# cherise215/Cooperative_Training_and_Latent_Space_Data_Augmentation

Hardware: AMD Instinct MI355X
Metric: cooperative-training slices/sec (256x256, bs16 per GPU) (higher is better)
Workload: dtype f32 (bf16x3 split)

## Files before the change

### cooperative_training_and_latent_space_data_augmentation_amd/_ffi.py

```python
from __future__ import annotations

import ctypes as C
import os

import numpy as np

_HERE = os.path.dirname(os.path.abspath(__file__))
LIB_PATH = os.path.join(_HERE, "csrc", "libctl_hip.so")
ABI_VERSION = 11
RED_BLOCKS = 512

IN_PLAIN, IN_UP2, IN_ZINS2, IN_C4 = 0, 1, 2, 3
ACT_NONE, ACT_LEAKY, ACT_SIGMOID = 0, 1, 2
EPI_BIAS, EPI_ACCUM, EPI_RES, EPI_STATS, EPI_BNBWD, EPI_TAILBWD = 1, 2, 4, 8, 16, 32
(OP_CONV, OP_WGRAD, OP_WGRAD_REDUCE, OP_PACK, OP_BN_FINALIZE, OP_BN_EVAL, OP_BN_ACT, OP_BWD_REDUCE, OP_BN_BWD_FINALIZE,
 OP_BWD_APPLY, OP_CHAN_SUM_FINALIZE, OP_SUMPOOL2, OP_SIGMOID_BWD, OP_ZERO, OP_COPY, OP_PACK_BATCH, OP_WGRAD_REDUCE_BATCH, OP_DROPOUT2D, OP_BN_REPLAY,
 OP_WGRAD_GROUP) = range(1, 21)
WGRAD_GROUP_MAX = 8
OP_MAX_T = 14

CONV_DTYPE = np.dtype([
    ("n", "<i4"), ("hin", "<i4"), ("win", "<i4"), ("cin", "<i4"), ("hout", "<i4"), ("wout", "<i4"), ("cout", "<i4"),
    ("ks", "<i4"), ("stride", "<i4"), ("pad", "<i4"), ("in_mode", "<i4"), ("pro_affine", "<i4"), ("pro_slope", "<f4"),
    ("epi_flags", "<i4"), ("epi_act", "<i4"), ("epi_slope", "<f4"), ("out_h", "<i4"), ("out_w", "<i4"),
    ("out_sy", "<i4"), ("out_sx", "<i4"), ("nsub", "<i4"), ("out_sub", "<i4"), ("groups", "<i4"), ("dt", "<i4")])
DT_BF16, DT_X16, DT_Y16, DT_RES16, DT_X3 = 1, 2, 4, 8, 16
PACK_X3 = 16
LOSS_WCE, LOSS_FOCAL, LOSS_DICE, LOSS_FG_DICE = 0, 1, 2, 3
OP_DTYPE = np.dtype([("kind", "<i4"), ("i", "<i4", (27,)), ("f", "<f4", (4,)), ("slot", "<i4", (OP_MAX_T,)),
                     ("off", "<i8", (OP_MAX_T,)), ("l", "<i8", (4,))], align=True)


class CtlError(RuntimeError):
    pass


class _Lib:
    def __init__(self):
        self._lib = None

    def load(self):
        if self._lib is not None:
            return self._lib
        if not os.path.exists(LIB_PATH):
            raise CtlError(f"HIP extension not built: {LIB_PATH} is missing. Run `python -c 'import __graft_entry__ as g; "
                           "g.build()'` (or `make -C <package>/csrc`). There is no fallback path.")
        import torch
        lib = C.CDLL(LIB_PATH)
        lib.ctl_last_error.restype = C.c_char_p
        lib.ctl_version.restype = C.c_int
        lib.ctl_launch_count.restype = C.c_ulonglong
        for name in ("ctl_conv_wpack_floats", "ctl_conv_stats_floats", "ctl_wgrad_partial_floats",
                     "ctl_wgrad_bias_partial_floats", "ctl_latent_score_ws_floats", "ctl_latent_mask_apply_ws_floats",
                     "ctl_rescale_intensity_ws_floats", "ctl_sizeof_op", "ctl_sizeof_conv", "ctl_latent_mask_fused_ws_floats", "ctl_conv_wpack_floats_x3",
                     "ctl_surface_stats_ws_bytes", "ctl_surface_map_ws_bytes", "ctl_cc_ws_bytes", "ctl_aug_ws_bytes", "ctl_aug_warp_ws_bytes",
                     "ctl_surface_quantiles_ws_bytes",
                     "ctl_aug_spline_ws_bytes", "ctl_aug_warp_cubic_ws_bytes", "ctl_aug_bias_ws_bytes", "ctl_order_stats_ws_bytes", "ctl_corrupt_spike_ws_bytes",
                     "ctl_seg_loss_ws_doubles"):
            getattr(lib, name).restype = C.c_size_t
        p, i32, i64, f32, u64 = C.c_void_p, C.c_int32, C.c_int64, C.c_float, C.c_uint64
        sig = {
            "ctl_conv_wpack_floats": [i32, i32, i32],
            "ctl_conv_stats_floats": [p], "ctl_conv_stats_blocks": [p],
            "ctl_wgrad_splits": [p], "ctl_wgrad_partial_floats": [p], "ctl_wgrad_bias_partial_floats": [p],
            "ctl_pack_weights": [p, p, i32, i32, i32, i64, i64, i64, i64, i32, p],
            "ctl_conv_forward": [p] * 12, "ctl_conv_forward_ex": [p] * 16, "ctl_conv_pool_ok": [p],
            "ctl_conv_wgrad": [p] * 8, "ctl_conv_wgrad_ex": [p] * 10,
            "ctl_wgrad_group_class": [p, i32], "ctl_wgrad_group_plan": [p, i32, p], "ctl_conv_wgrad_group": [i32] + [p] * 11,
            "ctl_wgrad_reduce": [p, p, p, p, i64, i64, i64, i64, p, i32, p],
            "ctl_confusion_hist": [p, p, i64, i32, p, p],
            "ctl_rescale_intensity": [p, p, p, i32, i64, f32, f32, f32, p],
            "ctl_noise_clamp": [p, p, u64, f32, f32, f32, p, i64, p],
            "ctl_rescale_intensity_ws_floats": [i32],
            "ctl_crop_or_pad": [p, p, i32, i32, i32, i32, i32, i32, p],
            "ctl_bn_finalize": [p, i32, i32, i64, p, p, f32, f32, i32, p, p, p, p, p, p, p, i32, p],
            "ctl_bn_finalize_ex": [p, i32, i32, i64, p, p, f32, f32, i32, p, p, p, p, p, p, p, p, i32, p],
            "ctl_bn_replay_running": [p, p, p, p, i32, f32, p],
            "ctl_bn_eval_coeffs": [i32, p, p, p, p, f32, p, p, i32, p],
            "ctl_bn_act": [p, p, p, f32, p, i64, i32, i32, p],
            "ctl_bwd_reduce": [i32, p, p, p, p, p, f32, i64, i32, p, i32, p], "ctl_red_blocks": [],
            "ctl_bn_bwd_finalize": [p, i32, i64, p, p, p, p, p, p, i32, i32, i32, p],
            "ctl_bn_bwd_finalize_ex": [p, i32, i64, p, p, p, p, p, p, i32, i32, i32, C.c_uint32, p],
            "ctl_bwd_apply": [i32, p, p, p, p, p, f32, p, i64, i32, p, p, i32, p],
            "ctl_chan_sum_finalize": [p, i32, p, i32, p],
            "ctl_sumpool2": [p, p, i32, i32, i32, i32, i32, p],
            "ctl_sigmoid_bwd": [p, p, p, i64, p],
            "ctl_softmax_t_fwd": [p, f32, p, i64, i32, p],
            "ctl_softmax_t_bwd": [p, p, f32, p, i64, i32, p],
            "ctl_onehot": [p, p, i64, i32, p],
            "ctl_ce2d_fwd": [p, p, i64, i32, p, p, p],
            "ctl_ce2d_bwd": [p, p, p, i64, i32, p, p],
            "ctl_mse_fwd": [p, p, i64, f32, p, p, p],
            "ctl_mse_bwd": [p, p, p, i64, f32, p, p],
            "ctl_argmax_c": [p, p, i64, i32, p],
            "ctl_latent_score_ws_floats": [i32, i32, i32, i32],
            "ctl_latent_score": [i32, p, p, p, i32, i32, i32, p],
            "ctl_latent_mask_apply": [i32, p, p, p, i32, p, p, p, p, i32, i32, i32, p],
            "ctl_latent_mask_apply_ws_floats": [i32, i32, i32, i32],
            "ctl_latent_mask_fused_ws_floats": [i32, i32, i32, i32],
            "ctl_latent_mask_fused": [i32, p, p, p, i32, p, p, p, p, p, i32, i32, i32, p],
            "ctl_dropout2d": [p, p, u64, f32, p, p, i32, i32, i32, p],
            "ctl_uniform": [p, i64, u64, p],
            "ctl_step_tick": [p, p],
            "ctl_spin": [i32, p],
            "ctl_dropout2d_ex": [p, p, u64, p, f32, p, p, p, i32, i32, i32, p],
            "ctl_dropout2d_dt": [p, p, u64, p, f32, p, p, i32, i32, i32, C.c_uint32, p],
            "ctl_uniform_dev": [p, i64, u64, p, p],
            "ctl_adam_dev": [p, p, p, p, i64, f32, f32, f32, f32, p, f32, p],
            "ctl_adam": [p, p, p, p, i64, f32, f32, f32, f32, i32, f32, p],
            "ctl_accumulate": [p, p, i32, i64, p],
            "ctl_plan_run": [p, i32, p, i32, p],
            "ctl_prof_start": [C.c_char_p], "ctl_prof_start_sampled": [C.c_char_p, i32], "ctl_prof_stop": [p, C.c_size_t],
            "ctl_pack_weights_batched": [p, p, p, i32, i64, p], "ctl_wgrad_reduce_batched": [p, p, p, i32, i64, p],
            "ctl_pack_weights_bf16_batched": [p, p, p, i32, i64, p],
            "ctl_pack_weights_x3_batched": [p, p, p, i32, i64, p], "ctl_conv_wpack_floats_x3": [i32, i32, i32],
            "ctl_bwd_reduce_rows": [i32, i64, i32],
            "ctl_bn_act_dt": [p, p, p, f32, p, i64, i32, i32, C.c_uint32, p],
            "ctl_bwd_reduce_dt": [i32, p, p, p, p, p, f32, i64, i32, p, i32, C.c_uint32, p, p],
            "ctl_bwd_apply_dt": [i32, p, p, p, p, p, f32, p, i64, i32, p, p, i32, C.c_uint32, p],
            "ctl_sumpool2_dt": [p, p, i32, i32, i32, i32, i32, C.c_uint32, p],
            "ctl_surface_stats_rows": [i32, i32, i32, i32], "ctl_surface_stats_ws_bytes": [i32] * 6,
            "ctl_surface_stats": [p, p, i32, i32, i32, i32, i32, i32, i32, p, p, p, C.c_size_t, p],
            "ctl_surface_map_ws_bytes": [i32] * 4,
            "ctl_surface_quantiles_ws_bytes": [i32] * 7,
            "ctl_surface_quantiles": [p, p, i32, i32, i32, i32, i32, i32, i32, p, p, i32, p, p, p, C.c_size_t, p],
            "ctl_surface_map": [p, i32, i32, i32, i32, i32, p, p, p, p, C.c_size_t, p],
            "ctl_cc_ws_bytes": [i32] * 5, "ctl_cc_label": [p, i32, i32, i32, i32, i32, i32, p, p],
            "ctl_cc_keep_largest": [p, i32, i32, i32, i32, i32, i32, p, p, p, C.c_size_t, p],
            "ctl_aug_ws_bytes": [i32] * 3, "ctl_aug_warp_ws_bytes": [i32] * 5, "ctl_aug_field": [p, p, p, p, i32, i32, i32, p, p, C.c_size_t, p],
            "ctl_aug_warp": [p, p, p, p, p, i32, i32, i32, i32, i32, p, p, p, C.c_size_t, p],
            "ctl_aug_spline_ws_bytes": [i32] * 4, "ctl_aug_warp_cubic_ws_bytes": [i32] * 6,
            "ctl_aug_spline_coeffs": [p, p, p, i32, i32, i32, i32, p, p, C.c_size_t, p],
            "ctl_aug_warp_cubic": [p, p, p, p, p, i32, i32, i32, i32, i32, i32, p, p, p, C.c_size_t, p],
            "ctl_aug_bias_ws_bytes": [i32] * 3, "ctl_aug_bias": [p, p, p, p, i32, i32, i32, p, p, C.c_size_t, p],
            "ctl_aug_coarse_field": [p, i32, i32, i32, p, p],
            "ctl_order_stats_ws_bytes": [i32, i32], "ctl_order_stats": [p, i32, i64, p, i32, p, p, C.c_size_t, p],
            "ctl_percentile_apply": [p, p, i32, i64, C.c_double, C.c_double, i32, f32, f32, p, p, p],
            "ctl_resample_inplane": [p, p, i32, i32, i32, i32, i32, i32, C.c_double, C.c_double, p, p, p],
            "ctl_restore_scores": [p, i32, i32, i32, i32, i32, i32, i32, i32, i32, i32, C.c_double, C.c_double, i32, p, p, p],
            "ctl_restore_labels": [p, i32, i32, i32, i32, i32, i32, i32, i32, i32, C.c_double, C.c_double, p, p],
            "ctl_corrupt_bias": [p, p, i32, i32, i32, p, p], "ctl_corrupt_spike_ws_bytes": [i32] * 4,
            "ctl_corrupt_spike": [p, i32, i32, i32, p, p, i32, C.c_double, p, p, C.c_size_t, p],
            "ctl_corrupt_rigid3d": [p, i32, i32, i32, p, i32, p, p], "ctl_axis_operator": [p, p, i32, i32, i32, i32, i32, p, p, p],
            "ctl_slice_foreground": [p, p, i32, i64, p, p],
            "ctl_batch_gather": [p, p, p, i32, i64, p, i32, p, i32, i32, p, p, i32, i32, p, p, p],
            "ctl_seg_loss_blocks": [i32, i64], "ctl_seg_loss_ws_doubles": [i32, i32, i64, i32],
            "ctl_seg_loss_fwd": [i32, p, p, p, f32, i32, i64, i32, p, p, p],
            "ctl_seg_loss_bwd": [i32, p, p, p, f32, p, p, i32, i64, i32, p, p],
        }
        for name, args in sig.items():
            getattr(lib, name).argtypes = args
        if lib.ctl_version() != ABI_VERSION or lib.ctl_sizeof_op() != OP_DTYPE.itemsize or lib.ctl_sizeof_conv() != CONV_DTYPE.itemsize:
            raise CtlError(f"ABI mismatch: library version {lib.ctl_version()} vs binding {ABI_VERSION}, sizeof(ctl_op)={lib.ctl_sizeof_op()} "
                           f"vs {OP_DTYPE.itemsize}, sizeof(ctl_conv)={lib.ctl_sizeof_conv()} vs {CONV_DTYPE.itemsize}")
        if lib.ctl_red_blocks() != RED_BLOCKS:
            raise CtlError(f"ABI mismatch: the library was built with CTL_RED_BLOCKS={lib.ctl_red_blocks()}, this binding sizes scratch for {RED_BLOCKS}")
        self._lib = lib
        return lib

    def __getattr__(self, name):
        return getattr(self.load(), name)


lib = _Lib()

EXPORTED = ["ctl_version", "ctl_last_error", "ctl_conv_wpack_floats", "ctl_conv_stats_floats", "ctl_conv_stats_blocks",
            "ctl_pack_weights", "ctl_conv_forward", "ctl_conv_forward_ex", "ctl_conv_pool_ok", "ctl_wgrad_splits", "ctl_wgrad_partial_floats",
            "ctl_wgrad_bias_partial_floats", "ctl_conv_wgrad", "ctl_conv_wgrad_ex", "ctl_wgrad_reduce", "ctl_bn_finalize", "ctl_bn_finalize_ex", "ctl_bn_replay_running", "ctl_bn_eval_coeffs",
            "ctl_bn_act", "ctl_bwd_reduce", "ctl_bn_bwd_finalize", "ctl_bn_bwd_finalize_ex", "ctl_bwd_apply", "ctl_chan_sum_finalize", "ctl_sumpool2",
            "ctl_sigmoid_bwd", "ctl_softmax_t_fwd", "ctl_softmax_t_bwd", "ctl_onehot", "ctl_ce2d_fwd", "ctl_ce2d_bwd",
            "ctl_mse_fwd", "ctl_mse_bwd", "ctl_argmax_c", "ctl_latent_score_ws_floats", "ctl_latent_score",
            "ctl_latent_mask_apply", "ctl_latent_mask_apply_ws_floats", "ctl_dropout2d", "ctl_uniform", "ctl_adam", "ctl_plan_run", "ctl_sizeof_op",
            "ctl_sizeof_conv", "ctl_prof_start", "ctl_prof_start_sampled", "ctl_prof_stop", "ctl_pack_weights_batched",
            "ctl_wgrad_reduce_batched", "ctl_confusion_hist", "ctl_rescale_intensity_ws_floats", "ctl_rescale_intensity",
            "ctl_noise_clamp", "ctl_crop_or_pad", "ctl_step_tick", "ctl_spin", "ctl_dropout2d_ex", "ctl_dropout2d_dt", "ctl_uniform_dev", "ctl_adam_dev",
            "ctl_latent_mask_fused_ws_floats", "ctl_latent_mask_fused", "ctl_accumulate", "ctl_pack_weights_bf16_batched",
            "ctl_bn_act_dt", "ctl_bwd_reduce_dt", "ctl_bwd_apply_dt", "ctl_sumpool2_dt", "ctl_bwd_reduce_rows", "ctl_red_blocks",
            "ctl_launch_count", "ctl_conv_wpack_floats_x3", "ctl_pack_weights_x3_batched", "ctl_wgrad_group_class", "ctl_wgrad_group_plan",
            "ctl_conv_wgrad_group", "ctl_surface_stats_rows", "ctl_surface_stats_ws_bytes", "ctl_surface_stats", "ctl_surface_map_ws_bytes",
            "ctl_surface_map", "ctl_cc_ws_bytes", "ctl_cc_label", "ctl_cc_keep_largest", "ctl_aug_ws_bytes", "ctl_aug_warp_ws_bytes", "ctl_aug_field",
            "ctl_aug_warp", "ctl_aug_spline_ws_bytes", "ctl_aug_warp_cubic_ws_bytes", "ctl_aug_spline_coeffs", "ctl_aug_warp_cubic",
            "ctl_aug_bias_ws_bytes", "ctl_aug_bias", "ctl_aug_coarse_field", "ctl_order_stats_ws_bytes", "ctl_order_stats",
            "ctl_percentile_apply", "ctl_resample_inplane", "ctl_corrupt_bias", "ctl_corrupt_spike_ws_bytes", "ctl_corrupt_spike",
            "ctl_corrupt_rigid3d", "ctl_axis_operator", "ctl_slice_foreground", "ctl_batch_gather", "ctl_surface_quantiles_ws_bytes",
            "ctl_surface_quantiles", "ctl_restore_scores", "ctl_restore_labels", "ctl_seg_loss_blocks", "ctl_seg_loss_ws_doubles",
            "ctl_seg_loss_fwd", "ctl_seg_loss_bwd"]


def prof_start(kernel_filter: str = "", every: int = 1) -> None:
    check(lib.ctl_prof_start_sampled(kernel_filter.encode(), int(every)), "ctl_prof_start_sampled")


def prof_stop() -> dict:
    buf = C.create_string_buffer(1 << 18)
    check(lib.ctl_prof_stop(buf, len(buf)), "ctl_prof_stop")
    out = {}
    for line in buf.value.decode().splitlines():
        parts = line.split()
        out[parts[0]] = {k: float(v) for k, v in (kv.split("=") for kv in parts[1:])}
    return out


def check(rc: int, what: str = "") -> None:
    if rc != 0:
        msg = lib.ctl_last_error()
        raise CtlError(f"{what} failed (rc={rc}): {msg.decode() if msg else ''}")


def conv_desc(**kw) -> np.ndarray:
    d = np.zeros((), dtype=CONV_DTYPE)
    d["pad"] = 1 if kw.get("ks", 3) in (3, 4) else 0
    d["stride"] = 1
    d["nsub"] = 1
    d["groups"] = 1
    d["out_sy"] = d["out_sx"] = 1
    for k, v in kw.items():
        d[k] = v
    if "out_h" not in kw:
        d["out_h"] = d["hout"]
    if "out_w" not in kw:
        d["out_w"] = d["wout"]
    return d


def desc_ptr(d: np.ndarray) -> int:
    return d.ctypes.data
```

### cooperative_training_and_latent_space_data_augmentation_amd/csrc/ctl_common.h

```cpp
#pragma once
#include <hip/hip_runtime.h>
#include <stdint.h>
#include <stdio.h>
#include "ctl_hip.h"

void ctl_set_error(const char* fmt, ...);

#define CTL_FAIL(code, ...)            \
    do {                               \
        ctl_set_error(__VA_ARGS__);    \
        return (code);                 \
    } while (0)

#define CTL_REQUIRE(cond, ...)                        \
    do {                                              \
        if (!(cond)) CTL_FAIL(CTL_EINVAL, __VA_ARGS__); \
    } while (0)

void ctl_count_launches(int n);
#define CTL_LAUNCH_CHECK(name)                                                         \
    do {                                                                               \
        ctl_count_launches(1);                                                         \
        hipError_t e__ = hipGetLastError();                                            \
        if (e__ != hipSuccess) CTL_FAIL(CTL_ELAUNCH, "%s: %s", name, hipGetErrorString(e__)); \
    } while (0)

__host__ __device__ static inline int ctl_cdiv(int a, int b) { return (a + b - 1) / b; }
__host__ __device__ static inline int64_t ctl_cdiv64(int64_t a, int64_t b) { return (a + b - 1) / b; }

typedef float f32x4 __attribute__((ext_vector_type(4)));

__device__ __forceinline__ float ctl_leaky(float v, float slope) { return v > 0.f ? v : v * slope; }
__device__ __forceinline__ float ctl_leaky_grad(float out, float slope) { return out > 0.f ? 1.f : slope; }

__device__ __forceinline__ void ctl_barrier_lds_reads_done() { asm volatile("s_barrier" ::: "memory"); }
__device__ __forceinline__ void ctl_barrier_lds_writes_done() { asm volatile("s_waitcnt lgkmcnt(0)\n\ts_barrier" ::: "memory"); }

#ifdef CTL_TUNING
#include <stdlib.h>
static inline int ctl_tune_int(const char* name, int dflt) { const char* e = getenv(name); return e ? atoi(e) : dflt; }
static inline const char* ctl_tune_str(const char* name) { return getenv(name); }
#else
static inline constexpr int ctl_tune_int(const char*, int dflt) { return dflt; }
static inline constexpr const char* ctl_tune_str(const char*) { return nullptr; }
#endif

typedef unsigned int u32x2e __attribute__((ext_vector_type(2)));
typedef __bf16 bf16x2e __attribute__((ext_vector_type(2)));
typedef float f32x2e __attribute__((ext_vector_type(2)));
__device__ __forceinline__ f32x4 ldq(const void* __restrict__ p, int64_t i, bool b16) {
    if (b16) {
        const u32x2e u = reinterpret_cast<const u32x2e*>(p)[i];
        return f32x4{__builtin_bit_cast(float, u.x << 16), __builtin_bit_cast(float, u.x & 0xffff0000u),
                     __builtin_bit_cast(float, u.y << 16), __builtin_bit_cast(float, u.y & 0xffff0000u)};
    }
    return reinterpret_cast<const f32x4*>(p)[i];
}
#ifndef CTL_ELEM_NT
#define CTL_ELEM_NT 0
#endif
__device__ __forceinline__ void stq(void* __restrict__ p, int64_t i, f32x4 v, bool b16) {
    if (b16) {
        const u32x2e pk = u32x2e{__builtin_bit_cast(unsigned, __builtin_convertvector(f32x2e{v.x, v.y}, bf16x2e)),
                                 __builtin_bit_cast(unsigned, __builtin_convertvector(f32x2e{v.z, v.w}, bf16x2e))};
        if (CTL_ELEM_NT) __builtin_nontemporal_store(pk, reinterpret_cast<u32x2e*>(p) + i); else reinterpret_cast<u32x2e*>(p)[i] = pk;
    } else {
        if (CTL_ELEM_NT) __builtin_nontemporal_store(v, reinterpret_cast<f32x4*>(p) + i); else reinterpret_cast<f32x4*>(p)[i] = v;
    }
}

__device__ __forceinline__ double wave_sum_double(double v) {
    for (int o = 32; o > 0; o >>= 1) v += __shfl_xor(v, o);
    return v;
}

struct ctl_bn_chan { float gamma, beta, rm, rv; };
__device__ __forceinline__ ctl_bn_chan ctl_bn_chan_load(int ch, const float* __restrict__ gamma, const float* __restrict__ beta,
                                                        int update_running, const float* __restrict__ running_mean,
                                                        const float* __restrict__ running_var) {
    ctl_bn_chan p;
    p.gamma = gamma[ch]; p.beta = beta[ch];
    p.rm = update_running ? running_mean[ch] : 0.f;
    p.rv = update_running ? running_var[ch] : 0.f;
    return p;
}
__device__ __forceinline__ void ctl_bn_coefs(double s1, double s2, double count, int c, int g, int ch, ctl_bn_chan& p, float eps,
                                             float momentum, int update_running, float* __restrict__ running_mean,
                                             float* __restrict__ running_var, float* __restrict__ scale, float* __restrict__ shift,
                                             float* __restrict__ save_mean, float* __restrict__ save_invstd,
                                             float* __restrict__ save_uvar = nullptr) {
    const double mean = s1 / count;
    double var = s2 / count - mean * mean;
    if (var < 0.0) var = 0.0;
    const float invstd = (float)(1.0 / sqrt(var + (double)eps));
    const float sc = p.gamma * invstd;
    scale[g * c + ch] = sc;
    shift[g * c + ch] = p.beta - (float)mean * sc;
    if (save_mean) save_mean[g * c + ch] = (float)mean;
    if (save_invstd) save_invstd[g * c + ch] = invstd;
    if (update_running) {
        const double unbiased = count > 1.0 ? var * count / (count - 1.0) : var;
        if (save_uvar) save_uvar[g * c + ch] = (float)unbiased;
        p.rm = (1.f - momentum) * p.rm + momentum * (float)mean;
        p.rv = (1.f - momentum) * p.rv + momentum * (float)unbiased;
        running_mean[ch] = p.rm;
        running_var[ch] = p.rv;
    }
}
struct ctl_conv_cfg {
    int mt, tw, nt;
    int th;
    int tiles_h, tiles_w;
    int g;
    int cot;
    int pc;
};
int ctl_conv_pick_cfg(const ctl_conv* d, ctl_conv_cfg* c, int for_wgrad);
int ctl_conv_grid_x(int ntiles, int other, int occ);
static inline int ctl_num_cus() { static const int n = ctl_tune_int("CTL_NUM_CUS", 256); return n; }

int ctl_conv_forward_bf16(const ctl_conv* d, const void* x, const void* x2, const void* wpack, const float* bias, const float* pro_scale,
                          const float* pro_shift, const void* res, const float* res_scale, const float* res_shift, const void* res2, void* y,
                          float* stats_partial, void* pool, void* xout, ctl_stream stream);
int ctl_conv_bf16_stats_blocks(const ctl_conv* d);
int ctl_wgrad_bf16_splits(const ctl_conv* d);
int ctl_conv_wgrad_bf16(const ctl_conv* d, const void* x, const float* pro_scale, const float* pro_shift, const void* dy, const void* dy2,
                        const float* dy_coef, float* w_partial, float* b_partial, ctl_stream stream);

int ctl_wgrad_bf16_group_class(const ctl_conv* d, int has_dy2);
int ctl_wgrad_bf16_group_plan(const ctl_conv* descs, int n, int32_t* splits);
int ctl_conv_wgrad_bf16_group(int n, const ctl_conv* descs, const int32_t* splits, const void* const* x, const float* const* pro_scale,
                              const float* const* pro_shift, const void* const* dy, const void* const* dy2, const float* const* dy_coef,
                              float* const* w_partial, float* const* b_partial, ctl_stream stream);

int ctl_conv_x3_ok(const ctl_conv* d);
int ctl_conv_x3_stats_blocks(const ctl_conv* d);
int ctl_conv_forward_x3(const ctl_conv* d, const float* x, const float* wpack, const float* bias, const float* pro_scale, const float* pro_shift,
                        const float* res, const float* res_scale, const float* res_shift, const float* res2, const float* x2, float* y,
                        float* stats_partial, float* pool, float* xout, ctl_stream stream);

int ctl_wgrad_x3_ok(const ctl_conv* d);
int ctl_wgrad_x3_splits(const ctl_conv* d);
int ctl_conv_wgrad_x3(const ctl_conv* d, const float* x, const float* pro_scale, const float* pro_shift, const float* dy, const float* dy2,
                      const float* dy_coef, float* w_partial, float* b_partial, ctl_stream stream);

int ctl_prof_begin(const char* kind, const ctl_conv* d, const ctl_conv_cfg* c, int nt, hipStream_t stream, bool dy2 = false);
void ctl_prof_end(int token, hipStream_t stream);
int ctl_prof_begin_raw(const char* id, double flops, double bytes, hipStream_t stream);
```

### cooperative_training_and_latent_space_data_augmentation_amd/csrc/ctl_conv.hip

```cpp
#include <stdlib.h>

#include <type_traits>

#include "ctl_common.h"

#include "ctl_conv_common.h"

#ifdef CTL_TIMING
#define CTL_TM_WAVES 65536
__device__ unsigned long long ctl_tm[CTL_TM_WAVES][10];
#define TM_DECL unsigned long long tm_prev = __builtin_amdgcn_s_memtime(), tm_acc[10] = {0, 0, 0, 0, 0, 0, 0, 0, 0, 0}; \
                const unsigned long long tm_t0 = tm_prev, tm_r0 = __builtin_amdgcn_s_memrealtime();
#define TM(i) { const unsigned long long tm_now = __builtin_amdgcn_s_memtime(); tm_acc[i] += tm_now - tm_prev; tm_prev = tm_now; }
#define TM_COUNT(i) { tm_acc[i] += 1; }
#define TM_FLUSH { const unsigned w_ = ((blockIdx.x + gridDim.x * (blockIdx.y + gridDim.y * blockIdx.z)) * 4 + (threadIdx.x >> 6)) % CTL_TM_WAVES; \
                   tm_acc[8] = __builtin_amdgcn_s_memtime() - tm_t0; tm_acc[9] = __builtin_amdgcn_s_memrealtime() - tm_r0; \
                   if ((threadIdx.x & 63) == 0) { _Pragma("unroll") for (int i_ = 0; i_ < 10; ++i_) ctl_tm[w_][i_] += tm_acc[i_]; } }
extern "C" int ctl_debug_timing(unsigned long long* out8) {
    static unsigned long long host[CTL_TM_WAVES][10];
    if (hipMemcpyFromSymbol(host, HIP_SYMBOL(ctl_tm), sizeof(host)) != hipSuccess) return -1;
    for (int i = 0; i < 12; ++i) out8[i] = 0;
    for (int w = 0; w < CTL_TM_WAVES; ++w) {
        for (int i = 0; i < 10; ++i) out8[i] += host[w][i];
        if (host[w][8] > out8[10]) out8[10] = host[w][8];
        if (host[w][8]) out8[11] += 1;
    }
    for (int w = 0; w < CTL_TM_WAVES; ++w) for (int i = 0; i < 10; ++i) host[w][i] = 0;
    return hipMemcpyToSymbol(HIP_SYMBOL(ctl_tm), host, sizeof(host)) == hipSuccess ? 0 : -1;
}
#else
#define TM_DECL
#define TM(i)
#define TM_COUNT(i)
#define TM_FLUSH
#endif
#include "ctl_conv_igemm.h"


#ifndef CTL_WGRAD_PIPE_ASM_MFMA
#define CTL_WGRAD_PIPE_ASM_MFMA 0
#endif
#ifndef CTL_WGRAD_PIPE_ABLATE
#define CTL_WGRAD_PIPE_ABLATE 0
#endif
#ifndef CTL_WGRAD_PIPE_LAG
#define CTL_WGRAD_PIPE_LAG 2
#endif
template <int K, int N, class F>
__device__ __forceinline__ void ctl_unroll(F&& f) {
    if constexpr (K < N) {
        f(std::integral_constant<int, K>{});
        ctl_unroll<K + 1, N>(f);
    }
}

template <int KS, int S, int MODE, int MT, int TW, int NTW, bool DY2 = false, bool PIPE = false>
__global__ __launch_bounds__(256) void conv_wgrad_kernel(const ctl_conv d, const float* __restrict__ x,
                                                          const float* __restrict__ pro_scale,
                                                          const float* __restrict__ pro_shift,
                                                          const float* __restrict__ dy, float* __restrict__ w_partial,
                                                          float* __restrict__ b_partial, int tiles_h, int tiles_w,
                                                          int ntiles, int cin_p, int cout_p, const float* __restrict__ dy2,
                                                          const float* __restrict__ dy_coef) {
    using G = Geom<KS, S, MT, TW>;
    constexpr int TAPS = KS * KS;
    constexpr int DYT_FLOATS = NTW * G::TP * 16;
    constexpr int RED_FLOATS = 4 * NTW * 256;
    constexpr int BUF_FLOATS = G::XT_FLOATS + DYT_FLOATS;
    constexpr int IMG_FLOATS = (PIPE ? 2 : 1) * BUF_FLOATS;
    constexpr int LDS_FLOATS = (IMG_FLOATS > RED_FLOATS) ? IMG_FLOATS : RED_FLOATS;
    static_assert(!PIPE || (KS == 3 && S == 1 && MODE != CTL_IN_C4), "pipelined weight gradient: 3x3 stride-1 layers");
    __shared__ __attribute__((aligned(16))) float lds[LDS_FLOATS + (DY2 ? 5 : 2) * CTL_PRO_MAX];
    float* xt = lds;
    float* dyt = lds + G::XT_FLOATS;
    float* cf_scale = lds + LDS_FLOATS;
    float* cf_shift = cf_scale + CTL_PRO_MAX;
    float* cd = cf_shift + CTL_PRO_MAX;

    const int tid = threadIdx.x;
    const int lane = tid & 63;
    const int wave = __builtin_amdgcn_readfirstlane(tid >> 6);
    const int p = lane & 15, q = lane >> 4;
    const int g = blockIdx.y;
    const int cot0 = blockIdx.z * NTW;
    const int group_n = d.n / (d.groups > 1 ? d.groups : 1);

    constexpr bool C4 = (MODE == CTL_IN_C4);
    static_assert(!C4 || (KS == 3 && S == 1), "row-packed taps: 3x3 stride-1 only");
    constexpr int NACC = C4 ? 3 : TAPS;
    f32x4 acc[NACC][NTW];
#pragma unroll
    for (int a = 0; a < NACC; ++a)
#pragma unroll
        for (int t = 0; t < NTW; ++t) acc[a][t] = f32x4{0.f, 0.f, 0.f, 0.f};
    int c4off[3];
#pragma unroll
    for (int j = 0; j < 3; ++j) {
        const int tp = (4 * j + (p >> 2) < 9) ? 4 * j + (p >> 2) : 8;
        c4off[j] = ((tp / 3) * G::IWP + tp % 3) * 4 + (p & 3);
    }
    float bsum[NTW];
#pragma unroll
    for (int t = 0; t < NTW; ++t) bsum[t] = 0.f;

    constexpr int DU = G::TP * NTW * 4, ND = DU / 256;
    const __amdgpu_buffer_rsrc_t rx = ctl_rsrc(x, (int64_t)d.n * d.hin * d.win * d.cin * 4);
    const __amdgpu_buffer_rsrc_t rdy = ctl_rsrc(dy, (int64_t)d.n * d.hout * d.wout * d.cout * 4);
    const __amdgpu_buffer_rsrc_t rdy2 = DY2 ? ctl_rsrc(dy2, (int64_t)d.n * d.hout * d.wout * d.cout * 4) : rdy;
    XStage<KS, S, MODE, MT, TW> xs;
    xs.init(d);
    f32x4 dv[ND];
    f32x4 dv2[DY2 ? ND : 1];
    unsigned dmask = 0;
    bool dwhole = false;
    int dco = 0;
    int drel[ND], drc[ND], dlds[ND];
#pragma unroll
    for (int i = 0; i < ND; ++i) {
        const int u = tid + i * 256;
        const int pix = u / (NTW * 4);
        const int q4 = u - pix * (NTW * 4);
        const int t = q4 >> 2, cq = q4 & 3;
        const int pr = pix / TW, pc = pix % TW;
        const int co = (cot0 + t) * 16 + cq * 4;
        drc[i] = (co < d.cout) ? (pr | (pc << 16)) : 0x7fff7fff;
        drel[i] = (co < d.cout) ? ((pr * d.wout + pc) * d.cout + co) * 4 : CTL_OOB;
        dlds[i] = (t * G::TP + pix) * 16 + cq * 4;
        if (i == 0) dco = co < d.cout ? co : 0;
    }
    auto dyload = [&](int n, int ho0, int wo0) {
        const int tb = ((n * d.hout + ho0) * d.wout + wo0) * d.cout * 4;
        dwhole = ho0 + G::TH <= d.hout && wo0 + TW <= d.wout && d.cout >= 4;
        if (dwhole) {
#pragma unroll
            for (int i = 0; i < ND; ++i) dv[i] = ctl_bload4s(rdy, drel[i], tb);
            if constexpr (DY2) {
#pragma unroll
                for (int i = 0; i < ND; ++i) dv2[i] = ctl_bload4s(rdy2, drel[i], tb);
            }
            return;
        }
        dmask = 0;
#pragma unroll
        for (int i = 0; i < ND; ++i) {
            const bool ok = (unsigned)(ho0 + (drc[i] & 0xffff)) < (unsigned)d.hout && (unsigned)(wo0 + (drc[i] >> 16)) < (unsigned)d.wout;
            const int vo = ok ? (tb + drel[i]) : CTL_OOB;
            if constexpr (DY2) {
                dv[i] = ctl_bload4(rdy, vo); dv2[i] = ctl_bload4(rdy2, vo);
                dmask |= (ok && drel[i] != CTL_OOB) ? (1u << i) : 0u;
                continue;
            }
            if (d.cout >= 4) dv[i] = ctl_bload4(rdy, vo);
            else dv[i] = f32x4{ctl_bload1(rdy, vo), 0.f, 0.f, 0.f};
        }
    };
    auto dystore = [&](int goff) {
        if constexpr (DY2) {
            const float* cc = cd + goff + dco;
            const f32x4 ca = *reinterpret_cast<const f32x4*>(cc), cb = *reinterpret_cast<const f32x4*>(cc + CTL_PRO_MAX);
            const f32x4 c3 = *reinterpret_cast<const f32x4*>(cc + 2 * CTL_PRO_MAX);
            const f32x4 zero = {0.f, 0.f, 0.f, 0.f};
#pragma unroll
            for (int i = 0; i < ND; ++i) {
                const f32x4 r = ca * dv[i] + cb * dv2[i] + c3;
                *reinterpret_cast<f32x4*>(dyt + dlds[i]) = (dwhole || ((dmask >> i) & 1u)) ? r : zero;
            }
            return;
        }
#pragma unroll
        for (int i = 0; i < ND; ++i) *reinterpret_cast<f32x4*>(dyt + dlds[i]) = dv[i];
    };
    TileWalk cur;
    cur.init(blockIdx.x, gridDim.x, tiles_h, tiles_w);
    TM_DECL
    if constexpr (PIPE) {
        using XS = XStage<KS, S, MODE, MT, TW>;
        constexpr int NU = XS::NU, NITEM = NU + ND, NSLOT = MT * 4;
        constexpr bool PLAIN = CTL_MODE_IS_PLAIN(MODE);
        static_assert(TW == 16, "pipelined weight gradient: 16-pixel-wide tiles");
        const float *xl = x, *dyl = dy, *dy2l = DY2 ? dy2 : dy;
        asm volatile("" : "+s"(xl), "+s"(dyl), "+s"(dy2l));
        const __amdgpu_buffer_rsrc_t rx = ctl_rsrc(xl, (int64_t)d.n * d.hin * d.win * d.cin * 4);
        const __amdgpu_buffer_rsrc_t rdy = ctl_rsrc(dyl, (int64_t)d.n * d.hout * d.wout * d.cout * 4);
        const __amdgpu_buffer_rsrc_t rdy2 = ctl_rsrc(dy2l, (int64_t)d.n * d.hout * d.wout * d.cout * 4);
        const int ngrp = d.groups > 1 ? d.groups : 1;
        if (d.pro_affine)
            for (int i = tid; i < ngrp * d.cin; i += 256) { cf_scale[i] = pro_scale[i]; cf_shift[i] = pro_shift[i]; }
        if constexpr (DY2) {
            for (int i = tid; i < ngrp * d.cout; i += 256) {
                const int gi = i / d.cout, ch = i - gi * d.cout;
                cd[i] = dy_coef[(gi * 3 + 0) * d.cout + ch]; cd[CTL_PRO_MAX + i] = dy_coef[(gi * 3 + 1) * d.cout + ch];
                cd[2 * CTL_PRO_MAX + i] = dy_coef[(gi * 3 + 2) * d.cout + ch];
            }
        }
        const bool pro = d.pro_affine != 0;
        const float slope = d.pro_slope;
        const unsigned hv = PLAIN ? d.hin : 2 * d.hin, wv = PLAIN ? d.win : 2 * d.win;
        const bool chan_ok = g * 16 + (tid & 3) * 4 < d.cin;
        const bool chan_all = g * 16 + 16 <= d.cin;
        const int xcb = chan_ok ? g * 16 + (tid & 3) * 4 : 0;
        int L_tb = 0, L_vh0 = 0, L_vw0 = 0, L_dtb = 0, L_ho0 = 0, L_wo0 = 0, L_n = 0, R_n = 0;
        bool L_live = false, L_xall = false, L_dall = false, R_xall = false, R_dall = false;
        int L_oh = 0, L_ow = 0;
        auto L_set_a = [&](bool live) {
            const int ho0 = cur.th * G::TH, wo0 = cur.tw * TW;
            L_live = live; L_n = live ? cur.n : 0; L_ho0 = ho0; L_wo0 = wo0;
            L_vh0 = ho0 - G::PAD; L_vw0 = wo0 - G::PAD;
            L_oh = PLAIN ? L_vh0 : ((ho0 >> 1) - XS::PADH); L_ow = PLAIN ? L_vw0 : ((wo0 >> 1) - XS::PADH);
        };
        auto L_set_b = [&]() {
            L_tb = (((cur.n * d.hin + L_oh) * d.win + L_ow) * d.cin + g * 16) * 4;
            L_dtb = ((cur.n * d.hout + L_ho0) * d.wout + L_wo0) * d.cout * 4;
        };
        auto L_set_c = [&]() {
            L_xall = L_live && chan_all && L_vh0 >= 0 && L_vw0 >= 0 && L_vh0 + G::IH <= (int)hv && L_vw0 + G::IW <= (int)wv;
            L_dall = L_live && L_ho0 + G::TH <= d.hout && L_wo0 + TW <= d.wout;
        };
        auto L_set = [&](bool live) { L_set_a(live); L_set_b(); L_set_c(); };
        auto x_addr = [&](auto I) -> int {
            constexpr int i = decltype(I)::value;
            int vo = L_tb + xs.rel[i];
            if (__builtin_expect(!L_xall, 0)) {
                const int vh = L_vh0 + (xs.rc[i] & 0xffff), vw = L_vw0 + (xs.rc[i] >> 16);
                const bool ok = (L_live & chan_ok) & ((unsigned)vh < hv) & ((unsigned)vw < wv);
                vo = ok ? vo : CTL_OOB;
                xs.vmask = (xs.vmask & ~(1u << i)) | (ok ? (1u << i) : 0u);
            }
            return vo;
        };
        auto x_value = [&](auto I, f32x4 sc, f32x4 sh) -> f32x4 {
            constexpr int i = decltype(I)::value;
            f32x4 t = xs.v[i];
            if (pro) {
                t = ctl_leaky01(t * sc + sh, slope);
                if (__builtin_expect(!R_xall, 0)) {
                    const f32x4 zero = {0.f, 0.f, 0.f, 0.f};
                    t = ((xs.vmask >> i) & 1u) ? t : zero;
                }
            }
            return t;
        };
        auto dy_addr = [&](auto I) -> int {
            constexpr int i = decltype(I)::value;
            int vo = L_dtb + drel[i];
            if (__builtin_expect(!L_dall, 0)) {
                const bool ok = L_live & ((unsigned)(L_ho0 + (drc[i] & 0xffff)) < (unsigned)d.hout) & ((unsigned)(L_wo0 + (drc[i] >> 16)) < (unsigned)d.wout);
                vo = ok ? vo : CTL_OOB;
                if constexpr (DY2) dmask = (dmask & ~(1u << i)) | ((ok & (drel[i] != CTL_OOB)) ? (1u << i) : 0u);
            }
            return vo;
        };
        auto dy_value = [&](auto I, f32x4 ca, f32x4 cb, f32x4 c3) -> f32x4 {
            constexpr int i = decltype(I)::value;
            f32x4 r = dv[i];
            if constexpr (DY2) {
                r = ca * dv[i] + cb * dv2[i] + c3;
                if (__builtin_expect(!(R_dall && d.cout % 16 == 0), 0)) {
                    const f32x4 zero = {0.f, 0.f, 0.f, 0.f};
                    r = ((dmask >> i) & 1u) ? r : zero;
                }
            }
            return r;
        };
        auto u_value = [&](auto K, f32x4 sc, f32x4 sh, f32x4 ca, f32x4 cb, f32x4 c3) -> f32x4 {
            constexpr int k = decltype(K)::value;
            if constexpr (k < NU) return x_value(std::integral_constant<int, k>{}, sc, sh);
            else return dy_value(std::integral_constant<int, k - NU>{}, ca, cb, c3);
        };
        auto u_write = [&](auto K, float* img_w, f32x4 v) {
            constexpr int k = decltype(K)::value;
            if constexpr (k < NU) *reinterpret_cast<f32x4*>(img_w + xs.lds[k]) = v;
            else *reinterpret_cast<f32x4*>(img_w + G::XT_FLOATS + dlds[k - NU]) = v;
        };
        auto u_addr = [&](auto K) -> int {
            constexpr int k = decltype(K)::value;
            if constexpr (k < NU) return x_addr(std::integral_constant<int, k>{});
            else return dy_addr(std::integral_constant<int, k - NU>{});
        };
        auto u_load = [&](auto K, int vo) {
            constexpr int k = decltype(K)::value;
            if constexpr (k < NU) xs.v[k] = ctl_bload4(rx, vo);
            else {
                dv[k - NU] = ctl_bload4(rdy, vo);
                if constexpr (DY2) dv2[k - NU] = ctl_bload4(rdy2, vo);
            }
        };
        f32x4 sc = {1.f, 1.f, 1.f, 1.f}, sh = {0.f, 0.f, 0.f, 0.f}, ca = sh, cb = sh, c3 = sh;
        auto coefs = [&](int n) {
            const int gi = ngrp > 1 ? n / group_n : 0;
            if (pro) {
                sc = *reinterpret_cast<const f32x4*>(cf_scale + gi * d.cin + xcb); sh = *reinterpret_cast<const f32x4*>(cf_shift + gi * d.cin + xcb);
            }
            if constexpr (DY2) {
                const float* cc = cd + gi * d.cout + dco;
                ca = *reinterpret_cast<const f32x4*>(cc); cb = *reinterpret_cast<const f32x4*>(cc + CTL_PRO_MAX);
                c3 = *reinterpret_cast<const f32x4*>(cc + 2 * CTL_PRO_MAX);
            }
        };
        auto all_units = [&](auto&& f) { ctl_unroll<0, NITEM>(f); };
        L_set((int)blockIdx.x < ntiles);
        all_units([&](auto K) { u_load(K, u_addr(K)); });
        __syncthreads();
        R_xall = L_xall; R_dall = L_dall;
        coefs(L_n);
        all_units([&](auto K) { u_write(K, lds, u_value(K, sc, sh, ca, cb, c3)); });
// ... 191 lines not shown
        for (int tp = 0; tp < TPR; ++tp) {
            const int tap = tap0 + tp;
            if (tap < NACC) {
#pragma unroll
                for (int t = 0; t < NTW; ++t) {
                    float* r0 = red + tp * TAP_FLOATS + ((wave * NTW + t) * 4) * 64 + lane;
                    r0[0] = acc[tap][t].x; r0[64] = acc[tap][t].y; r0[128] = acc[tap][t].z; r0[192] = acc[tap][t].w;
                }
            }
        }
        ctl_barrier_lds_writes_done();
#pragma unroll
        for (int tp = 0; tp < TPR; ++tp) {
            const int tap = tap0 + tp;
            if (tap < NACC) {
#pragma unroll
                for (int e0 = 0; e0 < NTW * 256; e0 += 256) {
                    const int e = e0 + tid;
                    const int t = e >> 8, r = (e >> 6) & 3, l = e & 63;
                    float v = 0.f;
#pragma unroll
                    for (int w = 0; w < 4; ++w) v += red[tp * TAP_FLOATS + ((w * NTW + t) * 4 + r) * 64 + l];
                    const int co = (cot0 + t) * 16 + (l & 15);
                    if (C4) {
                        const int wtap = 4 * tap + (l >> 4);
                        if (wtap < TAPS && co < cout_p) w_partial[split_base + ((int64_t)wtap * cin_p + r) * cout_p + co] = v;
                    } else {
                        const int ci = g * 16 + (l >> 4) * 4 + r;
                        if (co < cout_p) w_partial[split_base + ((int64_t)tap * cin_p + ci) * cout_p + co] = v;
                    }
                }
            }
        }
    }
    if (g == 0 && b_partial != nullptr) {
        ctl_barrier_lds_reads_done();
#pragma unroll
        for (int t = 0; t < NTW; ++t) {
            float v = bsum[t];
            v += __shfl_xor(v, 16);
            v += __shfl_xor(v, 32);
            if (q == 0) red[(wave * NTW + t) * 16 + p] = v;
        }
        ctl_barrier_lds_writes_done();
        if (tid < NTW * 16) {
            float v = 0.f;
#pragma unroll
            for (int w = 0; w < 4; ++w) v += red[w * NTW * 16 + tid];
            const int co = cot0 * 16 + tid;
            if (co < cout_p) b_partial[(int64_t)blockIdx.x * cout_p + co] = v;
        }
    }
#ifdef CTL_TIMING_WGRAD
    tm_acc[5] += __builtin_amdgcn_s_memtime() - tm_loop_end;
    TM_FLUSH
#endif
}

__global__ __launch_bounds__(256) void wgrad_reduce_kernel(const float* __restrict__ w_partial,
                                                            const float* __restrict__ b_partial, int splits, int taps,
                                                            int ks, int cin, int cout, int cin_p, int cout_p,
                                                            float* __restrict__ dw, int64_t s_co, int64_t s_ci,
                                                            int64_t s_kh, int64_t s_kw, float* __restrict__ dbias,
                                                            int accumulate) {
    __shared__ float sm[8][32];
    const int e = threadIdx.x & 31, sl = threadIdx.x >> 5;
    const int64_t total = (int64_t)taps * cin * cout;
    const int64_t idx = (int64_t)blockIdx.x * 32 + e;
    const bool is_w = idx < total;
    const bool is_b = !is_w && dbias != nullptr && idx < total + cout;
    float v = 0.f;
    int co = 0, ci = 0, tap = 0;
    if (is_w) {
        co = idx % cout;
        ci = (idx / cout) % cin;
        tap = idx / ((int64_t)cout * cin);
        const int64_t stride = (int64_t)taps * cin_p * cout_p;
        const float* src = w_partial + ((int64_t)tap * cin_p + ci) * cout_p + co;
        for (int s = sl; s < splits; s += 8) v += src[s * stride];
    } else if (is_b) {
        co = idx - total;
        for (int s = sl; s < splits; s += 8) v += b_partial[(int64_t)s * cout_p + co];
    }
    sm[sl][e] = v;
    __syncthreads();
    if (sl == 0 && (is_w || is_b)) {
        float t = 0.f;
#pragma unroll
        for (int k = 0; k < 8; ++k) t += sm[k][e];
        float* dst = is_w ? dw + co * s_co + ci * s_ci + (tap / ks) * s_kh + (tap % ks) * s_kw : dbias + co;
        *dst = accumulate ? (*dst + t) : t;
    }
}

__global__ void pack_weights_kernel(const float* __restrict__ src, float* __restrict__ dst, int cout, int cin, int ks,
                                    int g_chunks, int64_t total, int64_t s_co, int64_t s_ci, int64_t s_kh,
                                    int64_t s_kw, int flip) {
    const int64_t idx = (int64_t)blockIdx.x * blockDim.x + threadIdx.x;
    if (idx >= total) return;
    const int j = idx & 3, lane = (idx >> 2) & 63;
    int64_t rest = idx >> 8;
    const int g = rest % g_chunks;
    rest /= g_chunks;
    const int taps = ks * ks;
    const int tap = rest % taps;
    const int cot = rest / taps;
    const int co = cot * 16 + (lane & 15);
    const int ci = g * 16 + (lane >> 4) * 4 + j;
    int kh = tap / ks, kw = tap % ks;
    if (flip) { kh = ks - 1 - kh; kw = ks - 1 - kw; }
    float v = 0.f;
    if (co < cout && ci < cin) v = src[co * s_co + ci * s_ci + kh * s_kh + kw * s_kw];
    dst[idx] = v;
}

__global__ void pack_weights_batched_kernel(const float* __restrict__ params, float* __restrict__ wpack,
                                            const int64_t* __restrict__ table) {
    const int64_t* r = table + (int64_t)blockIdx.y * 12;
    const int64_t total = r[10];
    const int64_t idx = (int64_t)blockIdx.x * blockDim.x + threadIdx.x;
    if (idx >= total || (r[11] & CTL_PACK_X3)) return;
    const float* src = params + r[0];
    float* dst = wpack + r[1];
    const int cout = (int)r[2], cin = (int)r[3], ks = (int)r[4], flip = (int)r[5];
    const int g_chunks = (cin + 15) / 16;
    const int j = idx & 3, lane = (idx >> 2) & 63;
    int64_t rest = idx >> 8;
    const int g = rest % g_chunks;
    rest /= g_chunks;
    const int taps = ks * ks;
    const int tap = rest % taps;
    const int cot = rest / taps;
    const int co = cot * 16 + (lane & 15);
    const int ci = g * 16 + (lane >> 4) * 4 + j;
    int kh = tap / ks, kw = tap % ks;
    float v = 0.f;
    if (r[11] == 4) {
        const int c = j, quad = (int)((idx >> 8) % 3), cot4 = (int)((idx >> 8) / 3);
        const int co4 = cot4 * 16 + (lane & 15), tp = 4 * quad + (lane >> 4);
        if (co4 < cout && c < cin && tp < 9) v = src[co4 * r[6] + c * r[7] + (tp / 3) * r[8] + (tp % 3) * r[9]];
        dst[idx] = v;
        return;
    }
    if (r[11] == 1) {
        if (co < cout && ci < cin) {
            for (int a = 0; a < 2; ++a) {
                const int sh = a + 2 - kh;
                if (sh < 0 || sh > 2) continue;
                for (int b = 0; b < 2; ++b) {
                    const int sw = b + 2 - kw;
                    if (sw < 0 || sw > 2) continue;
                    v += src[co * r[6] + ci * r[7] + sh * r[8] + sw * r[9]];
                }
            }
        }
    } else if (r[11] == 2) {
        if (co < cout && ci < cin) {
            const int a = flip >> 1, b = flip & 1;
            const int h0 = (kh == 0) ? 0 : (a ? 2 : 1), h1 = (kh == 0) ? (a ? 1 : 0) : 2;
            const int w0 = (kw == 0) ? 0 : (b ? 2 : 1), w1 = (kw == 0) ? (b ? 1 : 0) : 2;
            for (int sh = h0; sh <= h1; ++sh)
                for (int sw = w0; sw <= w1; ++sw) v += src[co * r[6] + ci * r[7] + sh * r[8] + sw * r[9]];
        }
    } else if (r[11] == 3) {
        if (co < cout && ci < cin) {
            const int a = flip >> 1, b = flip & 1;
            const int sh = a ? (kh == 0 ? 2 : 0) : (kh == 0 ? 1 : -1);
            const int sw = b ? (kw == 0 ? 2 : 0) : (kw == 0 ? 1 : -1);
            if (sh >= 0 && sw >= 0) v = src[co * r[6] + ci * r[7] + sh * r[8] + sw * r[9]];
        }
    } else {
        if (flip) { kh = ks - 1 - kh; kw = ks - 1 - kw; }
        if (co < cout && ci < cin) v = src[co * r[6] + ci * r[7] + kh * r[8] + kw * r[9]];
    }
    dst[idx] = v;
}

__global__ __launch_bounds__(256) void wgrad_reduce_batched_kernel(const float* __restrict__ scratch, float* __restrict__ grad,
                                                                    const int64_t* __restrict__ table) {
    __shared__ float sm[32][65];
    const int64_t* r = table + (int64_t)blockIdx.y * 16;
    const int splits = (int)r[4], taps = (int)(r[5] & 0xff), ks = (int)(r[5] >> 8), cin = (int)r[6], cout = (int)r[7];
    const int cin_p = (int)r[8], cout_p = (int)r[9];
    const int64_t total = (int64_t)taps * cin * cout;
    const bool has_b = r[1] >= 0 && r[3] >= 0;
    const bool wide = splits <= 64;
    const int EW = wide ? 64 : 8, SLN = wide ? 4 : 32;
    if ((int64_t)blockIdx.x * EW >= total + (has_b ? cout : 0)) return;
    const int e = wide ? (threadIdx.x & 63) : (threadIdx.x & 7), sl = wide ? (threadIdx.x >> 6) : (threadIdx.x >> 3);
    const int64_t idx = (int64_t)blockIdx.x * EW + e;
    const bool is_w = idx < total, is_b = !is_w && has_b && idx < total + cout;
    float v = 0.f;
    int co = 0, ci = 0, tap = 0;
    if (is_w) {
        co = idx % cout;
        ci = (idx / cout) % cin;
        tap = idx / ((int64_t)cout * cin);
        const int64_t stride = (int64_t)taps * cin_p * cout_p;
        const float* src = scratch + r[0] + ((int64_t)tap * cin_p + ci) * cout_p + co;
        for (int s0 = sl; s0 < splits; s0 += 8 * SLN) {
            float t8[8];
#pragma unroll
            for (int u = 0; u < 8; ++u) { const int s = s0 + u * SLN; t8[u] = s < splits ? src[s * stride] : 0.f; }
#pragma unroll
            for (int u = 0; u < 8; ++u) v += t8[u];
        }
    } else if (is_b) {
        co = idx - total;
        const float* src = scratch + r[1] + co;
        for (int s = sl; s < splits; s += SLN) v += src[(int64_t)s * cout_p];
    }
    sm[sl][e] = v;
    __syncthreads();
    if (sl == 0 && (is_w || is_b)) {
        float t = 0.f;
        for (int k = 0; k < SLN; ++k) t += sm[k][e];
        float* dst = is_w ? grad + r[2] + co * r[10] + ci * r[11] + (tap / ks) * r[12] + (tap % ks) * r[13] : grad + r[3] + co;
        *dst = r[14] ? (*dst + t) : t;
    }
}

extern "C" int ctl_pack_weights_batched(const float* params, float* wpack, const int64_t* table, int32_t n_rec,
                                        int64_t max_total, ctl_stream stream) {
    CTL_REQUIRE(params && wpack && table && n_rec > 0 && max_total > 0, "pack_weights_batched: bad arguments");
    pack_weights_batched_kernel<<<dim3((unsigned)ctl_cdiv64(max_total, 256), (unsigned)n_rec), dim3(256), 0, (hipStream_t)stream>>>(
        params, wpack, table);
    CTL_LAUNCH_CHECK("pack_weights_batched");
    return CTL_OK;
}
extern "C" int ctl_wgrad_reduce_batched(const float* scratch, float* grad, const int64_t* table, int32_t n_rec,
                                        int64_t max_elems, ctl_stream stream) {
    CTL_REQUIRE(scratch && grad && table && n_rec > 0 && max_elems > 0, "wgrad_reduce_batched: bad arguments");
    wgrad_reduce_batched_kernel<<<dim3((unsigned)max_elems, (unsigned)n_rec), dim3(256), 0, (hipStream_t)stream>>>(
        scratch, grad, table);
    CTL_LAUNCH_CHECK("wgrad_reduce_batched");
    return CTL_OK;
}

extern "C" size_t ctl_conv_wpack_floats(int32_t cin, int32_t cout, int32_t ks) {
    return (size_t)ctl_cdiv(cout, 16) * ks * ks * ctl_cdiv(cin, 16) * 256;
}

static bool conv_combo_ok(const ctl_conv* d) {
    const int k = d->ks, s = d->stride, m = d->in_mode, pd = d->pad;
    if (k == 3 && s == 1 && pd == 1 && m != CTL_IN_C4) return true;
    if (k == 3 && s == 1 && pd == 1 && m == CTL_IN_C4 && d->cin <= 4 && d->nsub == 1) return true;
    if (k == 3 && s == 2 && pd == 1 && m == CTL_IN_PLAIN) return true;
    if (k == 1 && s == 1 && pd == 0 && m != CTL_IN_ZINS2) return true;
    if (k == 2 && s == 2 && pd == 0 && m == CTL_IN_PLAIN) return true;
    if (k == 4 && s == 2 && pd == 1 && m == CTL_IN_PLAIN) return true;
    if (k == 2 && s == 1 && (pd == 0 || pd == 2) && m == CTL_IN_PLAIN && d->nsub == 4) return true;
    return false;
}

int ctl_conv_pick_cfg(const ctl_conv* d, ctl_conv_cfg* c, int for_wgrad) {
    CTL_REQUIRE(conv_combo_ok(d), "conv: unsupported ks/stride/pad/in_mode %d/%d/%d/%d", d->ks, d->stride, d->pad,
                d->in_mode);
    CTL_REQUIRE(d->cin == 1 || d->cin % 4 == 0, "conv: cin must be 1 or a multiple of 4 (got %d)", d->cin);
    CTL_REQUIRE(d->cout == 1 || d->cout % 4 == 0, "conv: cout must be 1 or a multiple of 4 (got %d)", d->cout);
    CTL_REQUIRE(d->cin < 16 ? (d->cin == 1 || d->cin == 4 || d->cin == 8 || d->cin == 12) : d->cin % 16 == 0,
                "conv: cin >= 16 must be a multiple of 16 (got %d)", d->cin);
    CTL_REQUIRE(d->nsub == 1 || d->nsub == 4, "conv: nsub must be 1 or 4");
    c->cot = ctl_cdiv(d->cout, 16);
    c->g = ctl_cdiv(d->cin, 16);
    c->nt = (c->cot % 2 == 0) ? 2 : 1;
    auto blocks = [&](int mt, int tw) {
        const int th = 4 * mt * 16 / tw;
        return (int64_t)d->n * ctl_cdiv(d->hout, th) * ctl_cdiv(d->wout, tw) * (c->cot / c->nt) * d->nsub;
    };
    int mt, tw;
    if (for_wgrad) {
        if (d->hout >= 8) { mt = 2; tw = 16; }
        else { mt = 1; tw = 16; }
    } else if (d->stride == 2) {
        if (blocks(2, 16) >= 384) { mt = 2; tw = 16; } else { mt = 1; tw = 16; }
        if (d->ks == 4 && c->nt == 2) { mt = 1; tw = 16; }
    } else if (d->wout >= 32 && blocks(4, 32) >= 512 && !(c->nt == 2 && blocks(4, 32) > 768)) {
        mt = 4; tw = 32;
    } else if (blocks(2, 16) >= 384) {
        mt = 2; tw = 16;
    } else {
        mt = 1; tw = 16;
    }
    {
        static int fm = 0, ft = 0, fn = 0;
        static const bool forced = [] {
            const char* f = ctl_tune_str("CTL_FORCE_CFG");
            return f && sscanf(f, "%d,%d,%d", &fm, &ft, &fn) == 3;
        }();
        if (forced) {
            const bool tile_ok = (fm == 4 && ft == 32 && d->stride == 1 && !for_wgrad) || (fm == 2 && ft == 16) || (fm == 1 && ft == 16);
            if (tile_ok) { mt = fm; tw = ft; }
            if ((fn == 1 || fn == 2) && c->cot % fn == 0) c->nt = fn;
            if (d->ks == 4 && c->nt == 2) { mt = 1; tw = 16; }
        }
    }
    c->pc = 0;
    c->mt = mt; c->tw = tw; c->th = 4 * mt * 16 / tw;
    c->tiles_h = ctl_cdiv(d->hout, c->th);
    c->tiles_w = ctl_cdiv(d->wout, c->tw);
    return CTL_OK;
}

int ctl_conv_grid_x(int ntiles, int other, int occ) {
    static int per_cu = -1;
    if (per_cu < 0) {
        per_cu = ctl_tune_int("CTL_PERSIST", 4);
        if (per_cu < 1) per_cu = 1;
    }
    const int resident = occ < per_cu ? occ : per_cu;
    int cap = (ctl_num_cus() * resident) / other;
    if (other > 1 && cap >= 8) cap -= cap % 8;
    if (cap < 1) cap = 1;
    return ntiles < cap ? ntiles : cap;
}

extern "C" int ctl_pack_weights(const float* src, float* dst, int32_t cout, int32_t cin, int32_t ks, int64_t s_co,
                                int64_t s_ci, int64_t s_kh, int64_t s_kw, int32_t flip, ctl_stream stream) {
    CTL_REQUIRE(src && dst && cout > 0 && cin > 0 && ks >= 1 && ks <= 4, "pack_weights: bad arguments");
    const int64_t total = (int64_t)ctl_conv_wpack_floats(cin, cout, ks);
    pack_weights_kernel<<<dim3((unsigned)ctl_cdiv64(total, 256)), dim3(256), 0, (hipStream_t)stream>>>(
        src, dst, cout, cin, ks, ctl_cdiv(cin, 16), total, s_co, s_ci, s_kh, s_kw, flip);
    CTL_LAUNCH_CHECK("pack_weights");
    return CTL_OK;
}

struct conv_call {
    const ctl_conv* d; ctl_conv_cfg c;
    const float *x, *wpack, *bias, *pro_scale, *pro_shift, *res, *res_scale, *res_shift, *res2, *x2;
    float *y, *stats_partial, *pool, *xout;
    hipStream_t stream;
    bool query;
    int grid_x;
};

template <int KS, int S, int MODE, int MT, int TW, int NT, int EPI, bool X2 = false>
static void conv_go(conv_call& a) {
    if constexpr (!X2 && ((KS == 3 && S == 1 && MODE == CTL_IN_PLAIN) || (KS == 4 && S == 2)) && EPI != 2) {
        if (a.d->pro_affine == 2) { conv_go<KS, S, MODE, MT, TW, NT, EPI, true>(a); return; }
    }
    static int occ = 0;
    if (!occ) {
        int n = 0;
        if (hipOccupancyMaxActiveBlocksPerMultiprocessor(&n, conv_igemm_kernel<KS, S, MODE, MT, TW, NT, EPI, X2>, 256, 0) != hipSuccess || n < 1) {
            (void)hipGetLastError();
            n = 2;
        }
        occ = n;
    }
    const ctl_conv* d = a.d;
    const int ntiles = d->n * a.c.tiles_h * a.c.tiles_w;
    a.grid_x = ctl_conv_grid_x(ntiles, (a.c.cot / NT) * d->nsub, occ);
    if (a.query) return;
    const dim3 grid((unsigned)a.grid_x, (unsigned)(a.c.cot / NT), (unsigned)d->nsub);
    conv_igemm_kernel<KS, S, MODE, MT, TW, NT, EPI, X2><<<grid, dim3(256), 0, a.stream>>>(
        *d, a.x, a.wpack, a.bias, a.pro_scale, a.pro_shift, a.res, a.res_scale, a.res_shift, a.y, a.stats_partial, a.c.tiles_h,
        a.c.tiles_w, a.c.g, (int64_t)ctl_conv_wpack_floats(d->cin, d->cout, d->ks), ntiles, a.res2, a.x2, a.pool, a.xout);
}
template <int KS, int S, int MODE>
constexpr bool conv_tail_ok() { return (KS == 1 && MODE == CTL_IN_PLAIN) || KS == 2 || (KS == 3 && S == 1 && MODE == CTL_IN_ZINS2); }
template <int KS, int S, int MODE, int MT, int TW>
static void conv_go_nt(conv_call& a) {
    const bool epi = (a.d->epi_flags & (CTL_EPI_RES | CTL_EPI_ACCUM | CTL_EPI_BNBWD)) != 0;
    if constexpr (conv_tail_ok<KS, S, MODE>()) {
        if (a.d->epi_flags & CTL_EPI_TAILBWD) {
            if (a.c.nt == 2) conv_go<KS, S, MODE, MT, TW, 2, 2>(a); else conv_go<KS, S, MODE, MT, TW, 1, 2>(a);
            return;
        }
    }
    if constexpr (KS == 3 && S == 1 && MODE == CTL_IN_PLAIN) {
        if ((a.d->epi_flags & (CTL_EPI_RES | CTL_EPI_ACCUM | CTL_EPI_BNBWD)) == CTL_EPI_BNBWD && a.d->cout % 16 == 0 && a.d->epi_act == CTL_ACT_NONE) {
            if (a.c.nt == 2) conv_go<KS, S, MODE, MT, TW, 2, 3>(a); else conv_go<KS, S, MODE, MT, TW, 1, 3>(a);
            return;
        }
    }
    if (a.c.nt == 2) { if (epi) conv_go<KS, S, MODE, MT, TW, 2, 1>(a); else conv_go<KS, S, MODE, MT, TW, 2, 0>(a); }
    else { if (epi) conv_go<KS, S, MODE, MT, TW, 1, 1>(a); else conv_go<KS, S, MODE, MT, TW, 1, 0>(a); }
}
template <int KS, int S, int MODE>
static void conv_go_tile(conv_call& a) {
    if (S == 1 && a.c.mt == 4 && a.c.tw == 32) conv_go_nt<KS, S, MODE, (S == 1 ? 4 : 2), (S == 1 ? 32 : 16)>(a);
    else if (a.c.mt == 2) conv_go_nt<KS, S, MODE, 2, 16>(a);
    else conv_go_nt<KS, S, MODE, 1, 16>(a);
}
static int conv_dispatch(conv_call& a) {
    const int k = a.d->ks, s = a.d->stride, m = a.d->in_mode;
    if (k == 3 && s == 1 && m == CTL_IN_PLAIN) conv_go_tile<3, 1, CTL_IN_PLAIN>(a);
    else if (k == 3 && s == 1 && m == CTL_IN_UP2) conv_go_tile<3, 1, CTL_IN_UP2>(a);
    else if (k == 3 && s == 1 && m == CTL_IN_ZINS2) conv_go_tile<3, 1, CTL_IN_ZINS2>(a);
    else if (k == 3 && s == 1 && m == CTL_IN_C4) conv_go_tile<3, 1, CTL_IN_C4>(a);
    else if (k == 3 && s == 2) conv_go_tile<3, 2, CTL_IN_PLAIN>(a);
    else if (k == 1 && m == CTL_IN_PLAIN) conv_go_tile<1, 1, CTL_IN_PLAIN>(a);
    else if (k == 1 && m == CTL_IN_UP2) conv_go_tile<1, 1, CTL_IN_UP2>(a);
    else if (k == 2 && s == 2) conv_go_tile<2, 2, CTL_IN_PLAIN>(a);
    else if (k == 2 && s == 1) conv_go_tile<2, 1, CTL_IN_PLAIN>(a);
    else if (k == 4 && s == 2) {
        const bool epi = (a.d->epi_flags & (CTL_EPI_RES | CTL_EPI_ACCUM | CTL_EPI_BNBWD)) != 0;
        if (a.c.mt == 2 && a.c.nt == 1) { if (epi) conv_go<4, 2, CTL_IN_PLAIN, 2, 16, 1, 1>(a); else conv_go<4, 2, CTL_IN_PLAIN, 2, 16, 1, 0>(a); }
        else if (a.c.nt == 2) { if (epi) conv_go<4, 2, CTL_IN_PLAIN, 1, 16, 2, 1>(a); else conv_go<4, 2, CTL_IN_PLAIN, 1, 16, 2, 0>(a); }
        else { if (epi) conv_go<4, 2, CTL_IN_PLAIN, 1, 16, 1, 1>(a); else conv_go<4, 2, CTL_IN_PLAIN, 1, 16, 1, 0>(a); }
    }
    else CTL_FAIL(CTL_EUNSUPPORTED, "conv_forward: no kernel for this combination");
    return CTL_OK;
}

extern "C" int ctl_conv_stats_blocks(const ctl_conv* d) {
    if (d->dt & CTL_DT_BF16) return ctl_conv_bf16_stats_blocks(d);
    if (d->dt & CTL_DT_X3) return ctl_conv_x3_stats_blocks(d);
    conv_call a = {};
    a.d = d;
    if (ctl_conv_pick_cfg(d, &a.c, 0) != CTL_OK) return -1;
    a.query = true;
    if (conv_dispatch(a) != CTL_OK) return -1;
    return a.grid_x * d->nsub;
}
extern "C" size_t ctl_conv_stats_floats(const ctl_conv* d) {
    const int b = ctl_conv_stats_blocks(d);
    return b < 0 ? 0 : (size_t)(d->groups > 1 ? d->groups : 1) * b * 2 * d->cout;
}

extern "C" int ctl_conv_forward(const ctl_conv* d, const float* x, const float* wpack, const float* bias,
                                const float* pro_scale, const float* pro_shift, const float* res,
                                const float* res_scale, const float* res_shift, float* y, float* stats_partial,
                                ctl_stream stream) {
    return ctl_conv_forward_ex(d, x, wpack, bias, pro_scale, pro_shift, res, res_scale, res_shift, nullptr, nullptr, y, stats_partial, nullptr, nullptr, stream);
}
extern "C" int ctl_conv_pool_ok(const ctl_conv* d) {
    ctl_conv_cfg c;
    if (!d) return 0;
    if (!(d->epi_flags & CTL_EPI_TAILBWD) || d->ks != 1 || d->stride != 1 || d->in_mode != CTL_IN_PLAIN || d->nsub != 1 || (d->out_h & 1) || (d->out_w & 1) ||
        d->out_h != d->hout || d->out_w != d->wout || d->cout % 16 != 0)
        return 0;
    if (ctl_conv_pick_cfg(d, &c, 0) != CTL_OK) return 0;
    return (c.mt == 4 && c.tw == 32) || (c.mt == 2 && c.tw == 16);
}
extern "C" int ctl_conv_forward_ex(const ctl_conv* d, const float* x, const float* wpack, const float* bias,
                                   const float* pro_scale, const float* pro_shift, const float* res,
                                   const float* res_scale, const float* res_shift, const float* res2, const float* x2, float* y,
                                   float* stats_partial, float* pool, float* xout, ctl_stream stream) {
    CTL_REQUIRE(d && x && wpack && y, "conv_forward: null argument");
    CTL_REQUIRE(!xout || d->pro_affine == 2, "conv_forward: `xout` (the virtual input written out) goes with the BatchNorm-backward prologue (pro_affine 2)");
    CTL_REQUIRE(!pool || ctl_conv_pool_ok(d), "conv_forward: `pool` needs a CTL_EPI_TAILBWD 1x1 conv with even output sizes whose tile configuration gives every wave a row pair (ctl_conv_pool_ok)");
    CTL_REQUIRE((d->dt & CTL_DT_BF16) || !(d->dt & (CTL_DT_X16 | CTL_DT_Y16 | CTL_DT_RES16)), "conv_forward: bf16-stored tensors need CTL_DT_BF16");
    conv_call a = {};
    a.d = d;
    int rc = ctl_conv_pick_cfg(d, &a.c, 0);
    if (rc != CTL_OK) return rc;
    CTL_REQUIRE(!(d->epi_flags & CTL_EPI_BIAS) || bias, "conv_forward: CTL_EPI_BIAS without bias");
    CTL_REQUIRE(!(d->epi_flags & CTL_EPI_RES) || (res && res_scale && res_shift), "conv_forward: CTL_EPI_RES without res");
    CTL_REQUIRE(!(d->epi_flags & CTL_EPI_STATS) || stats_partial, "conv_forward: CTL_EPI_STATS without a partial buffer");
    CTL_REQUIRE(!(d->epi_flags & CTL_EPI_BNBWD) || ((d->epi_flags & CTL_EPI_STATS) && res && res_scale && res_shift &&
                                                    !(d->epi_flags & (CTL_EPI_RES | CTL_EPI_ACCUM | CTL_EPI_BIAS)) && d->epi_act == CTL_ACT_NONE),
                "conv_forward: CTL_EPI_BNBWD needs CTL_EPI_STATS + res (= u) + res_scale/res_shift (BatchNorm coefficients) and nothing else");
    if (d->epi_flags & CTL_EPI_TAILBWD) {
        const int k = d->ks, s = d->stride, m = d->in_mode;
        CTL_REQUIRE((d->epi_flags & CTL_EPI_STATS) && res && res2 && !(d->epi_flags & (CTL_EPI_RES | CTL_EPI_BNBWD | CTL_EPI_BIAS)) &&
                    d->epi_act == CTL_ACT_NONE && d->cout % 16 == 0,
                    "conv_forward: CTL_EPI_TAILBWD needs CTL_EPI_STATS + res (= the block output) + res2 (= the BatchNorm input), cout %% 16 == 0, nothing else but CTL_EPI_ACCUM (got cout %d)", d->cout);
        CTL_REQUIRE((k == 1 && m == CTL_IN_PLAIN) || k == 2 || (k == 3 && s == 1 && m == CTL_IN_ZINS2),
                    "conv_forward: CTL_EPI_TAILBWD is built for the launches that write a block's output gradient (1x1, 2x2, zero-insert 3x3)");
        CTL_REQUIRE(d->epi_slope >= 0.f && d->epi_slope <= 1.f, "conv_forward: LeakyReLU slope must be in [0, 1]");
    }
    CTL_REQUIRE(d->pro_affine >= 0 && d->pro_affine <= 2, "conv_forward: pro_affine must be 0, 1 or 2");
    CTL_REQUIRE(d->pro_affine != 1 || (pro_scale && pro_shift), "conv_forward: prologue without scale/shift");
    CTL_REQUIRE(d->pro_affine != 2 || (x2 && pro_scale && d->cin % 16 == 0 && d->in_mode == CTL_IN_PLAIN &&
                                       ((d->ks == 3 && d->stride == 1) || (d->ks == 4 && d->stride == 2)) && !(d->epi_flags & CTL_EPI_TAILBWD)),
                "conv_forward: the BatchNorm-backward prologue (pro_affine 2) needs x2 + coefficients, cin %% 16 == 0 and a plain 3x3 stride-1 or 4x4 stride-2 conv (got cin %d)", d->cin);
    CTL_REQUIRE(!d->pro_affine || (d->groups > 1 ? d->groups : 1) * d->cin <= CTL_PRO_MAX, "conv_forward: groups * cin = %d prologue coefficients exceed %d", (d->groups > 1 ? d->groups : 1) * d->cin, CTL_PRO_MAX);
    CTL_REQUIRE(d->pro_affine != 1 || (d->pro_slope >= 0.f && d->pro_slope <= 1.f), "conv_forward: prologue slope must be in [0, 1]");
    CTL_REQUIRE(d->epi_act != CTL_ACT_LEAKY || (d->epi_slope >= 0.f && d->epi_slope <= 1.f), "conv_forward: LeakyReLU slope must be in [0, 1]");
    CTL_REQUIRE(d->n > 0 && d->hout > 0 && d->wout > 0, "conv_forward: empty problem");
    CTL_REQUIRE(d->groups >= 0 && (d->groups <= 1 || d->n % d->groups == 0), "conv_forward: n=%d is not divisible into %d groups", d->n, d->groups);
    CTL_REQUIRE((int64_t)d->n * d->hin * d->win * d->cin * 4 < (1ll << 31) &&
                (int64_t)d->n * d->out_h * d->out_w * d->cout * 4 < (1ll << 31),
                "conv_forward: tensors must stay below 2 GiB (32-bit buffer offsets)");
    if (d->dt & CTL_DT_X3)
        return ctl_conv_forward_x3(d, x, wpack, bias, pro_scale, pro_shift, res, res_scale, res_shift, res2, x2, y, stats_partial, pool, xout, stream);
    if (d->dt & CTL_DT_BF16) {
        const int ptok16 = ctl_prof_begin("conv_igemm_bf16", d, &a.c, a.c.nt, (hipStream_t)stream);
        rc = ctl_conv_forward_bf16(d, x, x2, wpack, bias, pro_scale, pro_shift, res, res_scale, res_shift, res2, y, stats_partial, pool, xout, stream);
        ctl_prof_end(ptok16, (hipStream_t)stream);
        return rc;
    }
    a.x = x; a.wpack = wpack; a.bias = bias; a.pro_scale = pro_scale; a.pro_shift = pro_shift; a.res = res;
    a.res_scale = res_scale; a.res_shift = res_shift; a.res2 = res2; a.x2 = x2; a.y = y; a.stats_partial = stats_partial; a.pool = pool; a.xout = xout;
    a.stream = (hipStream_t)stream;
    const int ptok = ctl_prof_begin("conv_igemm", d, &a.c, a.c.nt, a.stream);
    rc = conv_dispatch(a);
    if (rc != CTL_OK) return rc;
    ctl_prof_end(ptok, a.stream);
    CTL_LAUNCH_CHECK("conv_forward");
    return CTL_OK;
}

#ifndef CTL_WGRAD_PIPE
#define CTL_WGRAD_PIPE 1
#endif
struct wgrad_cfg { ctl_conv_cfg c; int ntw, splits, ntiles, cin_p, cout_p; };

struct wgrad_call {
    const ctl_conv* d; wgrad_cfg* w;
    const float *x, *pro_scale, *pro_shift, *dy, *dy2, *dy_coef;
    float *w_partial, *b_partial;
    hipStream_t stream;
    bool query;
};

template <int KS, int S, int MODE, int MT, int TW, int NTW>
static void wgrad_go(wgrad_call& a) {
    static int occ = 0;
    if (!occ) {
        int n = 0;
        if (hipOccupancyMaxActiveBlocksPerMultiprocessor(&n, conv_wgrad_kernel<KS, S, MODE, MT, TW, NTW>, 256, 0) != hipSuccess || n < 1) {
            (void)hipGetLastError();
            n = 2;
        }
        occ = n;
    }
    wgrad_cfg& w = *a.w;
    static int per_cu = -1;
    if (per_cu < 0) {
        per_cu = ctl_tune_int("CTL_WGRAD_PERSIST", 1);
        if (per_cu < 1) per_cu = 1;
    }
    const int par = w.c.g * (w.c.cot / NTW);
    static const int slots = ctl_tune_int("CTL_WGRAD_SLOTS", 0);
    static const int narrow_cu = ctl_tune_int("CTL_WGRAD_NARROW_PERSIST", 2);
    const int cu_blocks = (KS == 1 || MODE == CTL_IN_C4) ? narrow_cu : per_cu;
    int splits = (slots > 0 ? slots : ctl_num_cus() * (occ < cu_blocks ? occ : cu_blocks)) / par;
    if (splits > 512) splits = 512;
    if (splits > w.ntiles) splits = w.ntiles;
    if (splits < 1) splits = 1;
    w.splits = splits;
    if (a.query) return;
    const dim3 grid((unsigned)splits, (unsigned)w.c.g, (unsigned)(w.c.cot / NTW));
    if constexpr (KS == 3 && S == 1 && MODE != CTL_IN_C4) {
        static const int pipe = ctl_tune_int("CTL_WGRAD_PIPE", CTL_WGRAD_PIPE);
        const bool pipe_on = pipe >= 2 || (pipe == 1 && a.dy2 && w.ntiles >= 8 * splits);
        if (pipe_on && a.d->cin % 4 == 0 && a.d->cout % 4 == 0 && a.d->cin <= CTL_PRO_MAX) {
            if (a.dy2)
                conv_wgrad_kernel<KS, S, MODE, MT, TW, NTW, true, true><<<grid, dim3(256), 0, a.stream>>>(
                    *a.d, a.x, a.pro_scale, a.pro_shift, a.dy, a.w_partial, a.b_partial, w.c.tiles_h, w.c.tiles_w, w.ntiles, w.cin_p, w.cout_p, a.dy2, a.dy_coef);
            else
                conv_wgrad_kernel<KS, S, MODE, MT, TW, NTW, false, true><<<grid, dim3(256), 0, a.stream>>>(
                    *a.d, a.x, a.pro_scale, a.pro_shift, a.dy, a.w_partial, a.b_partial, w.c.tiles_h, w.c.tiles_w, w.ntiles, w.cin_p, w.cout_p, nullptr, nullptr);
            return;
        }
    }
    if constexpr (KS == 3 && S == 1) {
        if (a.dy2) {
            conv_wgrad_kernel<KS, S, MODE, MT, TW, NTW, true><<<grid, dim3(256), 0, a.stream>>>(
                *a.d, a.x, a.pro_scale, a.pro_shift, a.dy, a.w_partial, a.b_partial, w.c.tiles_h, w.c.tiles_w, w.ntiles, w.cin_p, w.cout_p, a.dy2, a.dy_coef);
            return;
        }
    }
    conv_wgrad_kernel<KS, S, MODE, MT, TW, NTW><<<grid, dim3(256), 0, a.stream>>>(
        *a.d, a.x, a.pro_scale, a.pro_shift, a.dy, a.w_partial, a.b_partial, w.c.tiles_h, w.c.tiles_w, w.ntiles, w.cin_p, w.cout_p, nullptr, nullptr);
}
template <int KS, int S, int MODE>
static void wgrad_go_tile(wgrad_call& a) {
    const wgrad_cfg& w = *a.w;
    if (w.c.mt == 2) { if (w.ntw == 2) wgrad_go<KS, S, MODE, 2, 16, 2>(a); else wgrad_go<KS, S, MODE, 2, 16, 1>(a); }
    else { if (w.ntw == 2) wgrad_go<KS, S, MODE, 1, 16, 2>(a); else wgrad_go<KS, S, MODE, 1, 16, 1>(a); }
}
static int wgrad_dispatch(wgrad_call& a) {
    const int k = a.d->ks, s = a.d->stride, m = a.d->in_mode;
    if (k == 3 && s == 1 && m == CTL_IN_PLAIN) wgrad_go_tile<3, 1, CTL_IN_PLAIN>(a);
    else if (k == 3 && s == 1 && m == CTL_IN_UP2) wgrad_go_tile<3, 1, CTL_IN_UP2>(a);
    else if (k == 3 && s == 1 && m == CTL_IN_C4) wgrad_go_tile<3, 1, CTL_IN_C4>(a);
    else if (k == 3 && s == 2) wgrad_go_tile<3, 2, CTL_IN_PLAIN>(a);
    else if (k == 1 && m == CTL_IN_PLAIN) wgrad_go_tile<1, 1, CTL_IN_PLAIN>(a);
    else if (k == 1 && m == CTL_IN_UP2) wgrad_go_tile<1, 1, CTL_IN_UP2>(a);
    else if (k == 2 && s == 2) wgrad_go_tile<2, 2, CTL_IN_PLAIN>(a);
    else CTL_FAIL(CTL_EUNSUPPORTED, "conv_wgrad: no kernel for this combination");
    return CTL_OK;
}

static int wgrad_pick(const ctl_conv* d, wgrad_cfg* w) {
    CTL_REQUIRE(d->nsub == 1, "wgrad: nsub must be 1");
    CTL_REQUIRE(d->in_mode != CTL_IN_ZINS2, "wgrad: zero-insert input is not a forward mode");
    int rc = ctl_conv_pick_cfg(d, &w->c, 1);
    if (rc != CTL_OK) return rc;
    w->ntw = (w->c.cot >= 2 && w->c.cot % 2 == 0) ? 2 : 1;
    w->ntiles = d->n * w->c.tiles_h * w->c.tiles_w;
    w->cin_p = w->c.g * 16;
    w->cout_p = w->c.cot * 16;
    if (d->dt & CTL_DT_BF16) {
        w->splits = ctl_wgrad_bf16_splits(d);
        return w->splits > 0 ? CTL_OK : CTL_EUNSUPPORTED;
    }
    if (d->dt & CTL_DT_X3) {
        w->splits = ctl_wgrad_x3_splits(d);
        return w->splits > 0 ? CTL_OK : CTL_EUNSUPPORTED;
    }
    wgrad_call a = {};
    a.d = d; a.w = w; a.query = true;
    return wgrad_dispatch(a);
}

extern "C" int ctl_wgrad_splits(const ctl_conv* d) {
    wgrad_cfg w;
    return wgrad_pick(d, &w) == CTL_OK ? w.splits : -1;
}
extern "C" size_t ctl_wgrad_partial_floats(const ctl_conv* d) {
    wgrad_cfg w;
    if (wgrad_pick(d, &w) != CTL_OK) return 0;
    return (size_t)w.splits * d->ks * d->ks * w.cin_p * w.cout_p;
}
extern "C" size_t ctl_wgrad_bias_partial_floats(const ctl_conv* d) {
    wgrad_cfg w;
    if (wgrad_pick(d, &w) != CTL_OK) return 0;
    return (size_t)w.splits * w.cout_p;
}

extern "C" int ctl_conv_wgrad(const ctl_conv* d, const float* x, const float* pro_scale, const float* pro_shift,
                              const float* dy, float* w_partial, float* b_partial, ctl_stream stream) {
    return ctl_conv_wgrad_ex(d, x, pro_scale, pro_shift, dy, nullptr, nullptr, w_partial, b_partial, stream);
}
extern "C" int ctl_conv_wgrad_ex(const ctl_conv* d, const float* x, const float* pro_scale, const float* pro_shift,
                                 const float* dy, const float* dy2, const float* dy_coef, float* w_partial, float* b_partial,
                                 ctl_stream stream) {
    CTL_REQUIRE(d && x && dy && w_partial, "conv_wgrad: null argument");
    CTL_REQUIRE(d->pro_affine == 0 || d->pro_affine == 1, "conv_wgrad: pro_affine must be 0 or 1");
    CTL_REQUIRE(!dy2 || (dy_coef && d->ks == 3 && d->stride == 1 && d->cout % 16 == 0 &&
                         (d->groups > 1 ? d->groups : 1) * d->cout <= CTL_PRO_MAX),
                "conv_wgrad: the two-tensor output gradient needs coefficients, a 3x3 stride-1 conv, cout %% 16 == 0 and groups * cout <= %d (got cout %d)", CTL_PRO_MAX, d->cout);
    CTL_REQUIRE(!d->pro_affine || (pro_scale && pro_shift), "conv_wgrad: prologue without scale/shift");
    CTL_REQUIRE(!d->pro_affine || (d->groups > 1 ? d->groups : 1) * d->cin <= CTL_PRO_MAX, "conv_wgrad: groups * cin = %d prologue coefficients exceed %d", (d->groups > 1 ? d->groups : 1) * d->cin, CTL_PRO_MAX);
    CTL_REQUIRE(!d->pro_affine || (d->pro_slope >= 0.f && d->pro_slope <= 1.f), "conv_wgrad: prologue slope must be in [0, 1]");
    CTL_REQUIRE((int64_t)d->n * d->hin * d->win * d->cin * 4 < (1ll << 31) &&
                (int64_t)d->n * d->hout * d->wout * d->cout * 4 < (1ll << 31),
                "conv_wgrad: tensors must stay below 2 GiB (32-bit buffer offsets)");
    wgrad_cfg w;
    int rc = wgrad_pick(d, &w);
    if (rc != CTL_OK) return rc;
    if (d->dt & CTL_DT_X3) return ctl_conv_wgrad_x3(d, x, pro_scale, pro_shift, dy, dy2, dy_coef, w_partial, b_partial, stream);
    if (d->dt & CTL_DT_BF16) {
        const int ptok16 = ctl_prof_begin("conv_wgrad_bf16", d, &w.c, w.ntw, (hipStream_t)stream, dy2 != nullptr);
        rc = ctl_conv_wgrad_bf16(d, x, pro_scale, pro_shift, dy, dy2, dy_coef, w_partial, b_partial, stream);
        ctl_prof_end(ptok16, (hipStream_t)stream);
        return rc;
    }
    wgrad_call a = {};
    a.d = d; a.w = &w; a.x = x; a.pro_scale = pro_scale; a.pro_shift = pro_shift; a.dy = dy; a.dy2 = dy2; a.dy_coef = dy_coef; a.w_partial = w_partial;
    a.b_partial = b_partial; a.stream = (hipStream_t)stream;
    const int ptok = ctl_prof_begin("conv_wgrad", d, &w.c, w.ntw, a.stream, dy2 != nullptr);
    rc = wgrad_dispatch(a);
    if (rc != CTL_OK) return rc;
    ctl_prof_end(ptok, a.stream);
    CTL_LAUNCH_CHECK("conv_wgrad");
    return CTL_OK;
}

extern "C" int ctl_wgrad_reduce(const ctl_conv* d, const float* w_partial, const float* b_partial, float* dw,
                                int64_t s_co, int64_t s_ci, int64_t s_kh, int64_t s_kw, float* dbias,
                                int32_t accumulate, ctl_stream stream) {
    CTL_REQUIRE(d && w_partial && dw, "wgrad_reduce: null argument");
    CTL_REQUIRE(!dbias || b_partial, "wgrad_reduce: dbias without b_partial");
    wgrad_cfg w;
    int rc = wgrad_pick(d, &w);
    if (rc != CTL_OK) return rc;
    const int taps = d->ks * d->ks;
    const int64_t total = (int64_t)taps * d->cin * d->cout + (dbias ? d->cout : 0);
    wgrad_reduce_kernel<<<dim3((unsigned)ctl_cdiv64(total, 32)), dim3(256), 0, (hipStream_t)stream>>>(
        w_partial, b_partial, w.splits, taps, d->ks, d->cin, d->cout, w.cin_p, w.cout_p, dw, s_co, s_ci, s_kh, s_kw,
        dbias, accumulate);
    CTL_LAUNCH_CHECK("wgrad_reduce");
    return CTL_OK;
}
```

### cooperative_training_and_latent_space_data_augmentation_amd/csrc/ctl_conv_igemm.h

```cpp
#pragma once
#include <stdlib.h>

#include <type_traits>

#include "ctl_common.h"

#include "ctl_conv_common.h"
#include "ctl_conv_x3_stage.h"

#ifndef TM_DECL
#define TM_DECL
#define TM(i)
#define TM_COUNT(i)
#define TM_FLUSH
#endif

#define CTL_MODE_IS_PLAIN(M) ((M) == CTL_IN_PLAIN || (M) == CTL_IN_C4)

template <int KS, int S, int MODE, int MT, int TW, bool X2 = false>
struct XStage {
    using G = Geom<KS, S, MT, TW>;
    static constexpr bool C4M = (MODE == CTL_IN_C4);
    static constexpr int UNITS = G::IH * G::IW * (C4M ? 1 : 4);
    static constexpr int NU = (UNITS + 255) / 256;
    static constexpr int PADH = (G::PAD + 1) >> 1;
    int rel[NU];
    int rc[NU];
    int lds[NU];
    f32x4 v[NU];
    f32x4 v2[X2 ? NU : 1];
    unsigned vmask;
    int pad_h, pad_w;
    bool all_in;
    int tb_last;

    __device__ __forceinline__ void init(const ctl_conv& d) {
        const int tid = threadIdx.x, cq = C4M ? 0 : (tid & 3);
#pragma unroll
        for (int i = 0; i < NU; ++i) {
            const int u = tid + i * 256;
            const int pix = C4M ? u : (u >> 2);
            const int r = pix / G::IW;
            const int c = pix - r * G::IW;
            const bool in = u < UNITS;
            const int rr = CTL_MODE_IS_PLAIN(MODE) ? r : (((r - G::PAD) >> 1) + PADH);
            const int cc = CTL_MODE_IS_PLAIN(MODE) ? c : (((c - G::PAD) >> 1) + PADH);
            rel[i] = in ? ((rr * d.win + cc) * d.cin + cq * 4) * 4 : CTL_OOB;
            rc[i] = in ? (r | (c << 16)) : 0x7fff7fff;
            lds[i] = in ? (C4M ? (r * G::IWP + c) * 4 : ((r * G::IWP + G::ldscol(c)) * 16 + cq * 4)) : G::XT_IMAGE;
        }
        vmask = 0;
        all_in = false;
        pad_h = pad_w = G::PAD;
    }

    __device__ __forceinline__ void load(__amdgpu_buffer_rsrc_t rx, const ctl_conv& d, int n, int ho0, int wo0, int g) { load(rx, rx, d, n, ho0, wo0, g); }
    __device__ __forceinline__ void load(__amdgpu_buffer_rsrc_t rx, __amdgpu_buffer_rsrc_t rx2, const ctl_conv& d, int n, int ho0, int wo0, int g) {
        const int vh0 = ho0 * S - pad_h, vw0 = wo0 * S - pad_w;
        const unsigned hv = CTL_MODE_IS_PLAIN(MODE) ? d.hin : 2 * d.hin;
        const unsigned wv = CTL_MODE_IS_PLAIN(MODE) ? d.win : 2 * d.win;
        const int oh = CTL_MODE_IS_PLAIN(MODE) ? vh0 : ((ho0 >> 1) - PADH);
        const int ow = CTL_MODE_IS_PLAIN(MODE) ? vw0 : ((wo0 >> 1) - PADH);
        const int tb = (((n * d.hin + oh) * d.win + ow) * d.cin + g * 16) * 4;
        tb_last = tb;
#ifdef CTL_NO_INTERIOR
        all_in = false;
#else
        all_in = MODE != CTL_IN_ZINS2 && vh0 >= 0 && vw0 >= 0 && vh0 + G::IH <= (int)hv && vw0 + G::IW <= (int)wv &&
                 g * 16 + 16 <= d.cin;
#endif
        if (all_in) {
#pragma unroll
            for (int i = 0; i < NU; ++i) v[i] = ctl_bload4s(rx, rel[i], tb);
            if constexpr (X2) {
#pragma unroll
                for (int i = 0; i < NU; ++i) v2[i] = ctl_bload4s(rx2, rel[i], tb);
            }
            return;
        }
        const bool chan_ok = C4M || g * 16 + (threadIdx.x & 3) * 4 < d.cin;
        unsigned m = 0;
        int vo[NU];
#pragma unroll
        for (int i = 0; i < NU; ++i) {
            const int vh = vh0 + (rc[i] & 0xffff), vw = vw0 + (rc[i] >> 16);
            bool ok = chan_ok && (unsigned)vh < hv && (unsigned)vw < wv;
            if (MODE == CTL_IN_ZINS2) ok = ok && (((vh | vw) & 1) == 0);
            vo[i] = ok ? (tb + rel[i]) : CTL_OOB;
            m |= ok ? (1u << i) : 0u;
        }
        vmask = m;
        if constexpr (X2) {
#pragma unroll
            for (int i = 0; i < NU; ++i) { v[i] = ctl_bload4(rx, vo[i]); v2[i] = ctl_bload4(rx2, vo[i]); }
        } else if (d.cin >= 4) {
#pragma unroll
            for (int i = 0; i < NU; ++i) v[i] = ctl_bload4(rx, vo[i]);
        } else {
#pragma unroll
            for (int i = 0; i < NU; ++i) v[i] = f32x4{ctl_bload1(rx, vo[i]), 0.f, 0.f, 0.f};
        }
    }

    __device__ __forceinline__ void store(float* __restrict__ xt, const ctl_conv& d, int g,
                                          const float* pro_scale, const float* pro_shift, int goff, const float* pro_c = nullptr) {
        store(xt, d, g, pro_scale, pro_shift, goff, pro_c, ctl_rsrc((const void*)nullptr, 0), false);
    }
    __device__ __forceinline__ void store(float* __restrict__ xt, const ctl_conv& d, int g,
                                          const float* pro_scale, const float* pro_shift, int goff, const float* pro_c,
                                          __amdgpu_buffer_rsrc_t rxout, bool xout_on) {
        if constexpr (X2) {
            const int cb = g * 16 + (threadIdx.x & 3) * 4;
            const f32x4 ca = *reinterpret_cast<const f32x4*>(pro_scale + goff + cb), cbb = *reinterpret_cast<const f32x4*>(pro_shift + goff + cb);
            const f32x4 cc = *reinterpret_cast<const f32x4*>(pro_c + goff + cb);
            const f32x4 zero = {0.f, 0.f, 0.f, 0.f};
#pragma unroll
            for (int i = 0; i < NU; ++i) {
                const bool in = all_in || ((vmask >> i) & 1u);
                const f32x4 r = in ? (ca * v[i] + cbb * v2[i] + cc) : zero;
                *reinterpret_cast<f32x4*>(xt + lds[i]) = r;
                if (xout_on) {
                    const unsigned tr = (unsigned)((rc[i] & 0xffff) - pad_h), tc = (unsigned)((rc[i] >> 16) - pad_w);
                    const bool own = in && tr < (unsigned)(G::TH * S) && tc < (unsigned)(TW * S);
                    ctl_bstore4(rxout, own ? (tb_last + rel[i]) : CTL_OOB, r);
                }
            }
            return;
        }
        if (!d.pro_affine) {
#pragma unroll
            for (int i = 0; i < NU; ++i) *reinterpret_cast<f32x4*>(xt + lds[i]) = v[i];
            return;
        }
        const int cb = C4M ? 0 : g * 16 + (threadIdx.x & 3) * 4;
        f32x4 sc = {1.f, 1.f, 1.f, 1.f}, sh = {0.f, 0.f, 0.f, 0.f};
        if (cb < d.cin) {
            if (d.cin >= 4) {
                sc = *reinterpret_cast<const f32x4*>(pro_scale + goff + cb);
                sh = *reinterpret_cast<const f32x4*>(pro_shift + goff + cb);
            } else {
                sc.x = pro_scale[goff];
                sh.x = pro_shift[goff];
            }
        }
        const float slope = d.pro_slope;
        if (all_in) {
#pragma unroll
            for (int i = 0; i < NU; ++i) *reinterpret_cast<f32x4*>(xt + lds[i]) = ctl_leaky01(v[i] * sc + sh, slope);
            return;
        }
        const f32x4 zero = {0.f, 0.f, 0.f, 0.f};
#pragma unroll
        for (int i = 0; i < NU; ++i) {
            const f32x4 t = ctl_leaky01(v[i] * sc + sh, slope);
            *reinterpret_cast<f32x4*>(xt + lds[i]) = ((vmask >> i) & 1u) ? t : zero;
        }
    }
};


#ifndef CTL_LB_MID
#define CTL_LB_MID 3
#endif
#ifndef CTL_LB_SMALL
#define CTL_LB_SMALL 3
#endif
#ifndef CTL_PC_SETS
#define CTL_PC_SETS 3
#endif
#ifndef CTL_PC_SETS_X2
#define CTL_PC_SETS_X2 2
#endif
template <int KS, int S, int MODE, int MT, int TW, int NT, int EPI, bool X2 = false, bool X3 = false, bool PC = false>
#ifndef CTL_LB_X2EPI
#define CTL_LB_X2EPI 2
#endif
#ifndef CTL_LB_X2
#define CTL_LB_X2 2
#endif
#ifndef CTL_LB_SMALL_X2EPI
#define CTL_LB_SMALL_X2EPI CTL_LB_SMALL
#endif
#ifndef CTL_LB_X3
#define CTL_LB_X3(MT, NT, X2) (((NT) == 1 && (MT) >= 2 && !(X2)) ? 3 : 2)
#endif
__global__ __launch_bounds__(PC ? 512 : 256, PC ? 2 : X3 ? CTL_LB_X3(MT, NT, X2) : (MT * NT >= 8 || KS == 4) ? 2 : ((MT * NT >= 4) ? (X2 ? (EPI ? CTL_LB_X2EPI : CTL_LB_X2) : CTL_LB_MID)
                                                                                    : ((X2 && EPI) ? CTL_LB_SMALL_X2EPI : CTL_LB_SMALL))) void conv_igemm_kernel(const ctl_conv d, const float* __restrict__ x,
                                                          const float* __restrict__ wpack,
                                                          const float* __restrict__ bias,
                                                          const float* __restrict__ pro_scale,
                                                          const float* __restrict__ pro_shift,
                                                          const float* __restrict__ res,
                                                          const float* __restrict__ res_scale,
                                                          const float* __restrict__ res_shift, float* __restrict__ y,
                                                          float* __restrict__ stats_partial, int tiles_h, int tiles_w,
                                                          int G_chunks, int64_t wpack_sub_stride, int ntiles,
                                                          const float* __restrict__ res2, const float* __restrict__ x2,
                                                          float* __restrict__ pool, float* __restrict__ xout) {
    using G = Geom<KS, S, MT, TW>;
    constexpr int TAPS = KS * KS;
    constexpr bool C4 = (MODE == CTL_IN_C4);
    static_assert(!C4 || (KS == 3 && S == 1), "K-packed taps: 3x3 stride-1 only");
    static_assert(!X3 || !C4, "X3: whole 16-channel chunks");
    static_assert(!PC || X3, "the producer / consumer form exists for the X3 launches");
    constexpr int NIMG = PC ? 2 : 1;
    using XS3 = XStage3<KS, S, C4 ? CTL_IN_PLAIN : MODE, MT, TW, X2>;
    constexpr int NFRAG = X3 ? (TAPS + 1) / 2 : (C4 ? 3 : TAPS);
    constexpr int WSPL = X3 ? 3 : 1;
    constexpr int RED_FLOATS = 4 * NT * 16 * 2;
    constexpr int WT_FLOATS = NFRAG * NT * WSPL * 256;
    constexpr int XT_ALLOC = X3 ? XS3::XT_BYTES / 4 : G::XT_FLOATS;
    static_assert((NIMG * (XT_ALLOC + WT_FLOATS) + RED_FLOATS + (X2 ? 3 : 2) * CTL_PRO_MAX) * 4 <= 160 * 1024, "LDS budget of one CU");
    __shared__ __attribute__((aligned(16))) float xt[NIMG * (XT_ALLOC + WT_FLOATS) + RED_FLOATS + (X2 ? 3 : 2) * CTL_PRO_MAX];
    float* wt = xt + NIMG * XT_ALLOC;
    float* sred = wt + NIMG * WT_FLOATS;
    float* cf_scale = sred + RED_FLOATS;
    float* cf_shift = cf_scale + CTL_PRO_MAX;
    float* cf_c = cf_shift + (X2 ? CTL_PRO_MAX : 0);
    constexpr int WU = NFRAG * NT * WSPL * 64, NW = (WU + 255) / 256;

    const int tid = threadIdx.x;
    const int lane = tid & 63;
    const int wave_all = __builtin_amdgcn_readfirstlane(tid >> 6);
    const int wave = PC ? (wave_all & 3) : wave_all;
    const bool consumer = PC && wave_all >= 4;
    const int p = lane & 15, q = lane >> 4;
    const int P = gridDim.x < 8 ? (int)gridDim.x : 8;
    const int xcd = blockIdx.x % P, jblk = blockIdx.x / P;
    const int nb = ((int)gridDim.x - xcd + P - 1) / P;
    const int t_lo = (int)(((int64_t)ntiles * xcd) / P), t_hi = (int)(((int64_t)ntiles * (xcd + 1)) / P);
    const int bid0 = t_lo + jblk;
    const int z = blockIdx.z;
    const int cot0 = blockIdx.y * NT;
    const float* wp = wpack + (int64_t)z * wpack_sub_stride;
    const int my_tiles = (bid0 < t_hi) ? (t_hi - bid0 + nb - 1) / nb : 0;
    const int total_it = my_tiles * G_chunks;
    const int flags = d.epi_flags;
    const int ngroups = d.groups > 1 ? d.groups : 1;
    const int group_n = d.n / ngroups;
    const int oy0 = (z >> 1) * d.out_sub, ox0 = (z & 1) * d.out_sub;
    const __amdgpu_buffer_rsrc_t rx = ctl_rsrc(x, (int64_t)d.n * d.hin * d.win * d.cin * 4);
    const __amdgpu_buffer_rsrc_t rx2 = X2 ? ctl_rsrc(x2, (int64_t)d.n * d.hin * d.win * d.cin * 4) : rx;
    const bool xout_on = X2 && xout != nullptr && blockIdx.y == 0 && blockIdx.z == 0;
    const __amdgpu_buffer_rsrc_t rxout = xout_on ? ctl_rsrc(xout, (int64_t)d.n * d.hin * d.win * d.cin * 4) : rx;
    const int64_t ybytes = (int64_t)d.n * d.out_h * d.out_w * d.cout * 4;
    const __amdgpu_buffer_rsrc_t ry = ctl_rsrc(y, ybytes);
    const __amdgpu_buffer_rsrc_t rres = ctl_rsrc(EPI ? (const void*)res : (const void*)y, ybytes);
    constexpr bool TAIL = (EPI == 2);
    const __amdgpu_buffer_rsrc_t rres2 = ctl_rsrc(TAIL ? (const void*)res2 : (const void*)y, ybytes);
    constexpr bool CAN_POOL = TAIL && KS == 1 && S == 1 && MODE == CTL_IN_PLAIN && (MT / (TW / 16)) == 2;
    const __amdgpu_buffer_rsrc_t rpool = ctl_rsrc(CAN_POOL && pool ? (const void*)pool : (const void*)y, CAN_POOL && pool ? ybytes / 4 : ybytes);

    f32x4 ssum[NT], ssq[NT];
#pragma unroll
    for (int t = 0; t < NT; ++t) ssum[t] = ssq[t] = f32x4{0.f, 0.f, 0.f, 0.f};

    constexpr int TWT = TW / 16;
    static_assert(MT % TWT == 0, "a wave's M-tiles must cover whole tile rows");
    const int wrow = wave * (MT / TWT);
    int yrel[MT];
#pragma unroll
    for (int m = 0; m < MT; ++m)
        yrel[m] = (((wrow + m / TWT) * d.out_sy * d.out_w + ((m % TWT) * 16 + p) * d.out_sx) * d.cout + q * 4) * 4;
    const float* xrd = xt + ((wrow * S) * G::IWP + p) * 16 + q * 4;
    const float* wrd = wt + lane * 4;
    const float* xrd4[3];
#pragma unroll
    for (int j = 0; j < 3; ++j) {
        const int tp = (4 * j + q < 9) ? 4 * j + q : 8;
        xrd4[j] = xt + ((wrow + tp / 3) * G::IWP + p + tp % 3) * 4;
    }
    int xoff3[X3 ? NFRAG : 1];
    if constexpr (X3) {
#pragma unroll
        for (int f = 0; f < NFRAG; ++f) {
            int tap = 2 * f + (q >> 1);
            tap = tap < TAPS ? tap : TAPS - 1;
            const int kh = tap / KS, kw = tap % KS;
            const int kcol = (S == 2) ? ((kw & 1) * G::IWH + (kw >> 1)) : kw;
            xoff3[f] = (((wrow * S + kh) * G::IWP + p + kcol) * 16) + (q & 1) * XS3::PLANE;
        }
    }
    const unsigned char* xt8 = reinterpret_cast<const unsigned char*>(xt);
    const unsigned char* wrd8 = reinterpret_cast<const unsigned char*>(wt) + lane * 16;

    std::conditional_t<X3, XS3, XStage<KS, S, MODE, MT, TW, X2>> xs;
    xs.init(d);
    if (KS == 2 && S == 1) {
        xs.pad_h = d.pad == 2 ? 1 - (z >> 1) : 0;
        xs.pad_w = d.pad == 2 ? 1 - (z & 1) : 0;
    }
    const __amdgpu_buffer_rsrc_t rw = ctl_rsrc(wp, (int64_t)ctl_cdiv(d.cout, 16) * NFRAG * G_chunks * WSPL * 1024);
    f32x4 wv[NW];
    int wrel[NW];
#pragma unroll
    for (int i = 0; i < NW; ++i) {
        const int u = tid + i * 256;
        const int tt = u >> 6, l = u & 63;
        const int sp = X3 ? tt % WSPL : 0, tq = tt / WSPL;
        const int tap = tq / NT, t = tq - tap * NT;
        wrel[i] = (u < WU) ? (((((cot0 + t) * NFRAG + tap) * G_chunks) * WSPL + sp) * 64 + l) * 16 : CTL_OOB;
    }
    auto wload = [&](int g) {
#pragma unroll
        for (int i = 0; i < NW; ++i) wv[i] = ctl_bload4s(rw, wrel[i], g * WSPL * 1024);
    };
    auto wstore = [&](int img = 0) {
#pragma unroll
        for (int i = 0; i < NW; ++i) {
            const int u = tid + i * 256;
            if (u < WU) *reinterpret_cast<f32x4*>(wt + img * WT_FLOATS + u * 4) = wv[i];
        }
    };

    TileWalk cur, nxt;
    cur.init(bid0, nb, tiles_h, tiles_w);
    nxt = cur;
    TM_DECL
    if (!PC && total_it > 0) {
        xs.load(rx, rx2, d, cur.n, cur.th * G::TH, cur.tw * TW, 0);
        wload(0);
    }
    f32x4 bias4[NT];
    float bv[NT][4];
    {
        const bool has_bias = (flags & CTL_EPI_BIAS) != 0;
        const float* bp = has_bias ? bias : wpack;
#pragma unroll
        for (int t = 0; t < NT; ++t) {
            const int co0 = (cot0 + t) * 16 + q * 4;
#pragma unroll
            for (int k = 0; k < 4; ++k) bv[t][k] = bp[has_bias ? (co0 + k < d.cout ? co0 + k : d.cout - 1) : k];
        }
    }
    {
        const int ncf = ngroups * d.cin;
        const bool pro_on = X2 || d.pro_affine != 0;
        const bool con = pro_on && tid < ncf;
        const int ci = con ? tid : 0;
        float c0, c1, c2 = 0.f;
        if constexpr (X2) {
            const int gi = ci / d.cin, ch = ci - gi * d.cin;
            c0 = pro_scale[(gi * 3 + 0) * d.cin + ch]; c1 = pro_scale[(gi * 3 + 1) * d.cin + ch]; c2 = pro_scale[(gi * 3 + 2) * d.cin + ch];
        } else {
            const float* ps = pro_on ? pro_scale : wpack;
            const float* ph = pro_on ? pro_shift : wpack;
            c0 = ps[ci]; c1 = ph[ci];
        }
        static_assert(NT == 1 || NT == 2, "bias hand-over written for one or two cout tiles per block");
        if constexpr (NT == 1)
            asm volatile("" : "+v"(c0), "+v"(c1), "+v"(c2), "+v"(bv[0][0]), "+v"(bv[0][1]), "+v"(bv[0][2]), "+v"(bv[0][3]));
        else
            asm volatile("" : "+v"(c0), "+v"(c1), "+v"(c2), "+v"(bv[0][0]), "+v"(bv[0][1]), "+v"(bv[0][2]), "+v"(bv[0][3]),
                              "+v"(bv[NT - 1][0]), "+v"(bv[NT - 1][1]), "+v"(bv[NT - 1][2]), "+v"(bv[NT - 1][3]));
        const bool hb = (flags & CTL_EPI_BIAS) != 0;
#pragma unroll
        for (int t = 0; t < NT; ++t) {
            const int co0 = (cot0 + t) * 16 + q * 4;
            bias4[t] = f32x4{(hb && co0 + 0 < d.cout) ? bv[t][0] : 0.f, (hb && co0 + 1 < d.cout) ? bv[t][1] : 0.f,
                             (hb && co0 + 2 < d.cout) ? bv[t][2] : 0.f, (hb && co0 + 3 < d.cout) ? bv[t][3] : 0.f};
            asm volatile("" ::"v"(bias4[t]));
        }
        if (pro_on) {
            if (con) {
                cf_scale[tid] = c0; cf_shift[tid] = c1;
                if constexpr (X2) cf_c[tid] = c2;
            }
            __syncthreads();
        }
    }
    if constexpr (!PC) {
        if (total_it > 0) {
            xs.store(xt, d, 0, cf_scale, cf_shift, (cur.n / group_n) * d.cin, cf_c, rxout, xout_on);
            wstore();
        }
        __syncthreads();
    }

    constexpr bool WREG3 = X3 && !PC && MT == 1 && (NFRAG * NT * 3 <= 15);
    const bool wreg_on = WREG3 && G_chunks == 1;
    x3_bf16x8 wreg[WREG3 ? NFRAG : 1][WREG3 ? 3 : 1][WREG3 ? NT : 1];
    if constexpr (WREG3) {
        if (wreg_on) {
#pragma unroll
            for (int f = 0; f < NFRAG; ++f)
#pragma unroll
                for (int sp = 0; sp < 3; ++sp)
#pragma unroll
                    for (int t = 0; t < NT; ++t) wreg[f][sp][t] = *reinterpret_cast<const x3_bf16x8*>(wrd8 + ((f * NT + t) * 3 + sp) * 1024);
        }
    }

    const int srows = gridDim.x * gridDim.z * (PC ? 4 : 1), srow = (z * gridDim.x + blockIdx.x) * (PC ? 4 : 1) + (PC ? wave : 0);
    auto flush_stats = [&](int grp) {
#pragma unroll
        for (int t = 0; t < NT; ++t) {
            float a[8] = {ssum[t].x, ssum[t].y, ssum[t].z, ssum[t].w, ssq[t].x, ssq[t].y, ssq[t].z, ssq[t].w};
#pragma unroll
            for (int i = 0; i < 8; ++i) {
                float v = a[i];
                v += __shfl_xor(v, 1); v += __shfl_xor(v, 2); v += __shfl_xor(v, 4); v += __shfl_xor(v, 8);
                a[i] = v;
            }
            if constexpr (PC) {
                if (p == 0) {
#pragma unroll
                    for (int r = 0; r < 4; ++r) {
                        const int co = (cot0 + t) * 16 + q * 4 + r;
                        if (co < d.cout) {
                            stats_partial[(((int64_t)grp * srows + srow) * 2 + 0) * d.cout + co] = a[r];
                            stats_partial[(((int64_t)grp * srows + srow) * 2 + 1) * d.cout + co] = a[4 + r];
                        }
                    }
                }
                ssum[t] = ssq[t] = f32x4{0.f, 0.f, 0.f, 0.f};
                continue;
            }
            if (p == 0) {
#pragma unroll
                for (int r = 0; r < 4; ++r) {
                    sred[((wave * NT + t) * 16 + q * 4 + r) * 2 + 0] = a[r];
                    sred[((wave * NT + t) * 16 + q * 4 + r) * 2 + 1] = a[4 + r];
                }
            }
            ssum[t] = ssq[t] = f32x4{0.f, 0.f, 0.f, 0.f};
        }
        if constexpr (PC) return;
        __syncthreads();
        if (tid < NT * 16 * 2) {
            const int stat = tid / (NT * 16), cl = tid % (NT * 16);
            float v = 0.f;
#pragma unroll
            for (int w = 0; w < 4; ++w) v += sred[((w * NT * 16) + cl) * 2 + stat];
            const int co = cot0 * 16 + cl;
            if (co < d.cout) stats_partial[(((int64_t)grp * srows + srow) * 2 + stat) * d.cout + co] = v;
        }
        __syncthreads();
    };
    int cur_grp = (my_tiles > 0) ? cur.n / group_n : 0;
    if constexpr (PC) {
        if ((flags & CTL_EPI_STATS) && ngroups > 1 && consumer && p == 0) {
            for (int gi = 0; gi < ngroups; ++gi)
#pragma unroll
                for (int t = 0; t < NT; ++t)
#pragma unroll
                    for (int r = 0; r < 4; ++r) {
                        const int co = (cot0 + t) * 16 + q * 4 + r;
                        if (co < d.cout) {
                            stats_partial[(((int64_t)gi * srows + srow) * 2 + 0) * d.cout + co] = 0.f;
                            stats_partial[(((int64_t)gi * srows + srow) * 2 + 1) * d.cout + co] = 0.f;
                        }
                    }
        }
    } else if ((flags & CTL_EPI_STATS) && ngroups > 1 && tid < NT * 16 * 2) {
        const int stat = tid / (NT * 16), co = cot0 * 16 + tid % (NT * 16);
        if (co < d.cout)
            for (int gi = 0; gi < ngroups; ++gi) stats_partial[(((int64_t)gi * srows + srow) * 2 + stat) * d.cout + co] = 0.f;
    }

    TM(7)
    f32x4 acc[MT][NT];
#ifndef CTL_X3_ABLATE
#define CTL_X3_ABLATE 0
#endif

    auto mfma_phase3 = [&](auto wreg_tag, const unsigned char* xb, const unsigned char* wb) {
        constexpr bool WR = decltype(wreg_tag)::value;
#ifndef CTL_X3_MS
#define CTL_X3_MS(MT, NT, X2) ((CTL_LB_X3(MT, NT, X2) == 3 || (MT) < 2) ? 1 : 2)
#endif
        constexpr int MS = PC ? (MT >= 2 ? 2 : 1) : CTL_X3_MS(MT, NT, X2);
        constexpr int NSTEP = NFRAG * (MT / MS);
        x3_bf16x8 xf[2][MS][3], wf[2][WR ? 1 : 3][WR ? 1 : NT];
        auto xread = [&](int st, int b) {
            const int f = st / (MT / MS), m0 = (st % (MT / MS)) * MS;
#pragma unroll
            for (int mi = 0; mi < MS; ++mi)
#pragma unroll
                for (int sp = 0; sp < 3; ++sp)
                    xf[b][mi][sp] = *reinterpret_cast<const x3_bf16x8*>(xb + xoff3[f] + ((((m0 + mi) / TWT) * S) * G::IWP + ((m0 + mi) % TWT) * 16) * 16 + 2 * sp * XS3::PLANE);
        };
        auto wread = [&](int f, int b) {
            if constexpr (!WR) {
#pragma unroll
                for (int sp = 0; sp < 3; ++sp)
#pragma unroll
                    for (int t = 0; t < NT; ++t) wf[b][sp][t] = *reinterpret_cast<const x3_bf16x8*>(wb + ((f * NT + t) * 3 + sp) * 1024);
            }
        };
        xread(0, 0);
        wread(0, 0);
#pragma unroll
        for (int st = 0; st < NSTEP; ++st) {
            const int f = st / (MT / MS), m0 = (st % (MT / MS)) * MS, b = st & 1;
            if (st + 1 < NSTEP) {
                xread(st + 1, b ^ 1);
                if ((st + 1) % (MT / MS) == 0) wread(f + 1, (f + 1) & 1);
            }
#pragma unroll
            for (int mi = 0; mi < MS; ++mi) asm volatile("" : "+v"(xf[b][mi][0]), "+v"(xf[b][mi][1]), "+v"(xf[b][mi][2]) : : "memory");
#pragma unroll
            for (int t = 0; t < NT; ++t) {
                x3_bf16x8 ah, am, al;
                if constexpr (WR) { ah = wreg[WREG3 ? f : 0][0][WREG3 ? t : 0]; am = wreg[WREG3 ? f : 0][WREG3 ? 1 : 0][WREG3 ? t : 0]; al = wreg[WREG3 ? f : 0][WREG3 ? 2 : 0][WREG3 ? t : 0]; }
                else { ah = wf[f & 1][0][t]; am = wf[f & 1][WR ? 0 : 1][t]; al = wf[f & 1][WR ? 0 : 2][t]; }
#define CTL_X3_MFMA(A, SP) _Pragma("unroll") for (int mi = 0; mi < MS; ++mi) \
                    acc[m0 + mi][t] = __builtin_amdgcn_mfma_f32_16x16x32_bf16(A, xf[b][mi][SP], acc[m0 + mi][t], 0, 0, 0);
                CTL_X3_MFMA(al, 0)
                CTL_X3_MFMA(ah, 2)
                CTL_X3_MFMA(am, 1)
                CTL_X3_MFMA(am, 0)
                CTL_X3_MFMA(ah, 1)
                CTL_X3_MFMA(ah, 0)
#undef CTL_X3_MFMA
            }
        }
    };

    constexpr bool BNB = (EPI == 3), HAS_OV = (EPI == 1 || EPI == 2);
    f32x4 rv[EPI ? MT : 1][EPI ? NT : 1], ov[HAS_OV ? MT : 1][HAS_OV ? NT : 1], r2[TAIL ? MT : 1][TAIL ? NT : 1];
    f32x4 e_rs[EPI ? NT : 1] = {}, e_rh[EPI ? NT : 1] = {};
    auto tile_full = [&](int ho0, int wo0) {
#ifdef CTL_NO_FULL_EPI
        return false;
#else
        return ho0 + G::TH <= d.hout && wo0 + TW <= d.wout && (cot0 + NT) * 16 <= d.cout;
#endif
    };
    auto tile_ybase = [&](int n, int ho0, int wo0) {
        return (((n * d.out_h + ho0 * d.out_sy + oy0) * d.out_w + wo0 * d.out_sx + ox0) * d.cout + cot0 * 16) * 4;
    };
    auto epi_load = [&](auto full_tag, int n, int ho0, int wo0) {
        constexpr bool FULL = decltype(full_tag)::value;
        if constexpr (EPI != 0) {
            const int grp = n / group_n;
            const int ybase = tile_ybase(n, ho0, wo0);
#pragma unroll
            for (int t = 0; t < NT; ++t) {
                const bool cok = FULL || (cot0 + t) * 16 + q * 4 < d.cout;
#pragma unroll
                for (int m = 0; m < MT; ++m) {
                    const bool pvm = FULL || ((ho0 + wrow + m / TWT < d.hout) && (wo0 + (m % TWT) * 16 + p < d.wout));
                    const int vo = FULL ? (yrel[m] + t * 64) : ((pvm && cok) ? (ybase + yrel[m] + t * 64) : CTL_OOB);
                    const int so = FULL ? ybase : 0;
                    rv[m][t] = f32x4{0.f, 0.f, 0.f, 0.f};
                    if constexpr (HAS_OV) ov[m][t] = f32x4{0.f, 0.f, 0.f, 0.f};
                    if constexpr (BNB) {
                        rv[m][t] = ctl_bload4s(rres, vo, so);
                    } else if constexpr (TAIL) {
                        rv[m][t] = ctl_bload4s(rres, vo, so);
                        r2[m][t] = ctl_bload4s(rres2, vo, so);
                        if (flags & CTL_EPI_ACCUM) ov[m][t] = ctl_bload4s(ry, vo, so);
                    } else if (d.cout >= 4) {
                        if (flags & (CTL_EPI_RES | CTL_EPI_BNBWD)) rv[m][t] = ctl_bload4s(rres, vo, so);
                        if (flags & CTL_EPI_ACCUM) ov[m][t] = ctl_bload4s(ry, vo, so);
                    } else {
                        if (flags & (CTL_EPI_RES | CTL_EPI_BNBWD)) rv[m][t].x = ctl_bload1(rres, vo);
                        if (flags & CTL_EPI_ACCUM) ov[m][t].x = ctl_bload1(ry, vo);
                    }
                }
                const int co0 = (cot0 + t) * 16 + q * 4;
                const int cc = cok ? co0 : 0;
                f32x4 rs = {0.f, 0.f, 0.f, 0.f}, rh = {0.f, 0.f, 0.f, 0.f};
                if (!TAIL && (BNB || (flags & (CTL_EPI_RES | CTL_EPI_BNBWD)))) {
                    if (d.cout >= 4) {
                        rs = *reinterpret_cast<const f32x4*>(res_scale + grp * d.cout + cc);
                        rh = *reinterpret_cast<const f32x4*>(res_shift + grp * d.cout + cc);
                    } else { rs.x = res_scale[grp]; rh.x = res_shift[grp]; }
                }
                e_rs[t] = rs; e_rh[t] = rh;
            }
        }
    };
    auto epi_finish = [&](auto full_tag, int n, int ho0, int wo0) {
        constexpr bool FULL = decltype(full_tag)::value;
        const int ybase = tile_ybase(n, ho0, wo0);
#ifndef CTL_NO_FAST_EPI
        if constexpr (!EPI && FULL) {
            if (d.epi_act == CTL_ACT_NONE) {
                if (flags & CTL_EPI_STATS) {
                    asm volatile("" ::: "memory");
#pragma unroll
                    for (int t = 0; t < NT; ++t)
#pragma unroll
                        for (int m = 0; m < MT; ++m) { ssum[t] += acc[m][t]; ssq[t] += acc[m][t] * acc[m][t]; }
                }
#pragma unroll
                for (int t = 0; t < NT; ++t)
#pragma unroll
                    for (int m = 0; m < MT; ++m) ctl_bstore4(ry, ybase + yrel[m] + t * 64, acc[m][t]);
                return;
            }
        }
#endif
        bool pv[MT];
#pragma unroll
        for (int m = 0; m < MT; ++m)
            pv[m] = FULL || ((ho0 + wrow + m / TWT < d.hout) && (wo0 + (m % TWT) * 16 + p < d.wout));
#pragma unroll
        for (int t = 0; t < NT; ++t) {
            const int co0 = (cot0 + t) * 16 + q * 4;
            const bool cok = FULL || co0 < d.cout;
            const f32x4 rs = e_rs[EPI ? t : 0], rh = e_rh[EPI ? t : 0];
#pragma unroll
            for (int m = 0; m < MT; ++m) {
                f32x4 v = acc[m][t];
                if constexpr (TAIL) {
                    v += ov[m][t];
                    const f32x4 o = rv[m][t];
                    const float sl = d.epi_slope;
                    v.x *= o.x > 0.f ? 1.f : sl; v.y *= o.y > 0.f ? 1.f : sl;
                    v.z *= o.z > 0.f ? 1.f : sl; v.w *= o.w > 0.f ? 1.f : sl;
                    if (FULL || pv[m]) { ssum[t] += v; ssq[t] += v * r2[m][t]; }
                    if (FULL) ctl_bstore4(ry, ybase + yrel[m] + t * 64, v);
                    else ctl_bstore4(ry, (pv[m] && cok) ? (ybase + yrel[m] + t * 64) : CTL_OOB, v);
                    if constexpr (CAN_POOL) {
                        if (pool) {
                            f32x4 hs;
                            hs.x = v.x + __shfl_xor(v.x, 1); hs.y = v.y + __shfl_xor(v.y, 1);
                            hs.z = v.z + __shfl_xor(v.z, 1); hs.w = v.w + __shfl_xor(v.w, 1);
                            if (m < TWT) ov[m][t] = hs;
                            else {
                                const f32x4 top = ov[m - TWT][t];
                                const f32x4 pl = {top.x + hs.x, top.y + hs.y, top.z + hs.z, top.w + hs.w};
                                const int lo = ((((n * (d.out_h >> 1) + ((ho0 + wrow) >> 1)) * (d.out_w >> 1) + ((wo0 + (m % TWT) * 16 + p) >> 1)) * d.cout) + co0) * 4;
                                ctl_bstore4(rpool, ((p & 1) == 0 && (FULL || (pv[m] && cok))) ? lo : CTL_OOB, pl);
                            }
                        }
                    }
                    continue;
                }
                if (BNB || (EPI == 1 && (flags & CTL_EPI_BNBWD))) {
                    const f32x4 u = rv[m][t], sa = u * rs + rh;
                    const float sl = d.epi_slope;
                    v.x *= sa.x > 0.f ? 1.f : sl; v.y *= sa.y > 0.f ? 1.f : sl;
                    v.z *= sa.z > 0.f ? 1.f : sl; v.w *= sa.w > 0.f ? 1.f : sl;
                    if (FULL || pv[m]) { ssum[t] += v; ssq[t] += v * u; }
                } else {
                    if (EPI) v += rv[m][t] * rs + rh;
                    if (flags & CTL_EPI_STATS) {
                        if (FULL) { ssum[t] += v; ssq[t] += v * v; }
                        else if (pv[m]) { ssum[t] += v; ssq[t] += v * v; }
                    }
                }
                if (d.epi_act == CTL_ACT_LEAKY) {
                    v = ctl_leaky01(v, d.epi_slope);
                } else if (d.epi_act == CTL_ACT_SIGMOID) {
                    v.x = 1.f / (1.f + expf(-v.x)); v.y = 1.f / (1.f + expf(-v.y));
                    v.z = 1.f / (1.f + expf(-v.z)); v.w = 1.f / (1.f + expf(-v.w));
                }
                if constexpr (HAS_OV) v += ov[m][t];
                if (FULL) {
                    ctl_bstore4(ry, ybase + yrel[m] + t * 64, v);
                } else {
                    const int vo = (pv[m] && cok) ? (ybase + yrel[m] + t * 64) : CTL_OOB;
                    if (d.cout >= 4) ctl_bstore4(ry, vo, v);
                    else ctl_bstore1(ry, vo, v.x);
                }
            }
        }
    };

    if constexpr (PC) {
        const bool wdouble = G_chunks > 1;
        if (!consumer) {
            constexpr int R = X2 ? CTL_PC_SETS_X2 : CTL_PC_SETS;
            typename XS3::Pay P[R];
            int s_n[R], s_g[R];
            TileWalk lw = cur;
            int lg = 0, lit = 0;
            auto load_step = [&](typename XS3::Pay& pay, int& sn, int& sg) {
                xs.template load<true>(pay, rx, rx2, d, lw.n, lw.th * G::TH, lw.tw * TW, lg, lit < total_it);
                sn = lw.n; sg = lg;
                ++lit;
                if (++lg == G_chunks) { lg = 0; lw.next(); }
            };
#pragma unroll
            for (int r = 0; r < R - 1; ++r) load_step(P[r], s_n[r], s_g[r]);
            wload(0);
            load_step(P[R - 1], s_n[R - 1], s_g[R - 1]);
            auto run = [&](auto wd_tag) {
                constexpr bool WD = decltype(wd_tag)::value;
                int wg = 0;
                auto step = [&](int it, typename XS3::Pay& pay, int& sn, int& sg, bool more) {
                    const int img = it & 1;
#ifdef CTL_TIMING_X3_VMCNT
                    asm volatile("s_waitcnt vmcnt(%0)" :: "n"((R - 1) * XS3::NU * (X2 ? 4 : 2)) : "memory");
                    TM(9)
#endif
                    xs.template store<true>(pay, xt + img * XT_ALLOC, d, sg, cf_scale, cf_shift, (sn / group_n) * d.cin, cf_c, rxout, xout_on);
                    if constexpr (WD) wstore(img);
                    else if (it == 0) wstore(0);
                    TM(3)
                    if (more) {
                        if constexpr (WD) { wg = (wg + 1 == G_chunks) ? 0 : wg + 1; wload(wg); }
                        load_step(pay, sn, sg);
                    }
                    TM(0)
                    ctl_barrier_lds_writes_done();
                    TM(4)
                };
                const int full = (total_it / R) * R;
                for (int it0 = 0; it0 < full; it0 += R) {
#pragma unroll
                    for (int r = 0; r < R; ++r) step(it0 + r, P[r], s_n[r], s_g[r], true);
                }
#pragma unroll
                for (int r = 0; r < R - 1; ++r)
                    if (full + r < total_it) {
                        step(full + r, P[r], s_n[r], s_g[r], false);
                        if constexpr (WD) { if (full + r + 1 < total_it) { wg = (wg + 1 == G_chunks) ? 0 : wg + 1; wload(wg); } }
                    }
            };
            if (wdouble) run(std::true_type{}); else run(std::false_type{});
            TM_FLUSH
            return;
        }
#ifndef CTL_PC_PRIO
#define CTL_PC_PRIO 2
#endif
        __builtin_amdgcn_s_setprio(CTL_PC_PRIO);
        TileWalk cw = cur;
        int g = 0;
        for (int it = 0; it < total_it; ++it) {
            const int n = cw.n, ho0 = cw.th * G::TH, wo0 = cw.tw * TW;
            const bool last = (g == G_chunks - 1);
            const bool full = tile_full(ho0, wo0);
            if (last) {
                const int grp = n / group_n;
                if ((flags & CTL_EPI_STATS) && grp != cur_grp) { flush_stats(cur_grp); cur_grp = grp; }
                if (full) epi_load(std::true_type{}, n, ho0, wo0); else epi_load(std::false_type{}, n, ho0, wo0);
            }
            TM(7)
            ctl_barrier_lds_reads_done();
            TM(2)
            TM_COUNT(6)
            if (g == 0) {
#pragma unroll
                for (int m = 0; m < MT; ++m)
#pragma unroll
                    for (int t = 0; t < NT; ++t) acc[m][t] = bias4[t];
            }
            const int img = it & 1;
            mfma_phase3(std::false_type{}, xt8 + img * (XT_ALLOC * 4), wrd8 + (wdouble ? img : 0) * (WT_FLOATS * 4));
            TM(1)
            if (last) {
                if (full) epi_finish(std::true_type{}, n, ho0, wo0); else epi_finish(std::false_type{}, n, ho0, wo0);
            }
            TM(5)
            if (++g == G_chunks) { g = 0; cw.next(); }
        }
        if (flags & CTL_EPI_STATS) flush_stats(cur_grp);
        TM_FLUSH
        return;
    } else {
    for (int it = 0, g = 0; it < total_it; ++it) {
        TM_COUNT(6)
        const int n = cur.n, ho0 = cur.th * G::TH, wo0 = cur.tw * TW;
        const bool has_next = it + 1 < total_it;
        const int g2 = (g + 1 == G_chunks) ? 0 : g + 1;
        const bool new_w = has_next && G_chunks > 1;
        if (g2 == 0) nxt.next();
        if (has_next && !(X3 && (CTL_X3_ABLATE & 2))) {
            xs.load(rx, rx2, d, nxt.n, nxt.th * G::TH, nxt.tw * TW, g2);
            if (new_w) wload(g2);
        }
        TM(0)
        if (g == 0) {
#pragma unroll
            for (int m = 0; m < MT; ++m)
#pragma unroll
                for (int t = 0; t < NT; ++t) acc[m][t] = bias4[t];
        }
        if constexpr (X3 && (CTL_X3_ABLATE & 4)) {
        } else if constexpr (X3) {
            if constexpr (WREG3) {
                if (wreg_on) mfma_phase3(std::true_type{}, xt8, wrd8);
                else mfma_phase3(std::false_type{}, xt8, wrd8);
            } else {
                mfma_phase3(std::false_type{}, xt8, wrd8);
            }
        } else
        {
            f32x4 wf[2][NT], xf[2][MT];
            auto lds_operands = [&](int tap, int b) {
                const int kh = tap / KS, kw = tap % KS;
                const int kcol = (S == 2) ? ((kw & 1) * G::IWH + (kw >> 1)) : kw;
#pragma unroll
                for (int t = 0; t < NT; ++t) wf[b][t] = *reinterpret_cast<const f32x4*>(wrd + (tap * NT + t) * 256);
#pragma unroll
                for (int m = 0; m < MT; ++m) {
                    if (C4) xf[b][m] = *reinterpret_cast<const f32x4*>(xrd4[tap] + ((m / TWT) * G::IWP + (m % TWT) * 16) * 4);
                    else xf[b][m] = *reinterpret_cast<const f32x4*>(xrd + (((m / TWT) * S + kh) * G::IWP + (m % TWT) * 16 + kcol) * 16);
                }
            };
            lds_operands(0, 0);
#pragma unroll
            for (int tap = 0; tap < NFRAG; ++tap) {
                const int b = tap & 1;
                if (tap + 1 < NFRAG) lds_operands(tap + 1, b ^ 1);
#ifdef CTL_PIN_READ_AHEAD
                __builtin_amdgcn_sched_barrier(0);
#endif
#pragma unroll
                for (int m = 0; m < MT; ++m) {
#pragma unroll
                    for (int t = 0; t < NT; ++t) {
                        acc[m][t] = __builtin_amdgcn_mfma_f32_16x16x4f32(wf[b][t].x, xf[b][m].x, acc[m][t], 0, 0, 0);
                        acc[m][t] = __builtin_amdgcn_mfma_f32_16x16x4f32(wf[b][t].y, xf[b][m].y, acc[m][t], 0, 0, 0);
                        acc[m][t] = __builtin_amdgcn_mfma_f32_16x16x4f32(wf[b][t].z, xf[b][m].z, acc[m][t], 0, 0, 0);
                        acc[m][t] = __builtin_amdgcn_mfma_f32_16x16x4f32(wf[b][t].w, xf[b][m].w, acc[m][t], 0, 0, 0);
                    }
                }
#ifdef CTL_PIN_READ_AHEAD
                __builtin_amdgcn_sched_barrier(0);
#endif
            }
        }

        TM(1)
        ctl_barrier_lds_reads_done();
        TM(2)
#ifdef CTL_TIMING_X3_VMCNT
        asm volatile("s_waitcnt vmcnt(0)" ::: "memory");
        TM(9)
#endif
        if (has_next) {
            xs.store(xt, d, g2, cf_scale, cf_shift, (nxt.n / group_n) * d.cin, cf_c, rxout, xout_on);
            if (new_w) wstore();
        }
        TM(3)
        ctl_barrier_lds_writes_done();
        TM(4)

        if (g == G_chunks - 1 && !(X3 && (CTL_X3_ABLATE & 8))) {
            const int grp = n / group_n;
            if ((flags & CTL_EPI_STATS) && grp != cur_grp) {
                flush_stats(cur_grp);
                cur_grp = grp;
            }
            if (tile_full(ho0, wo0)) { epi_load(std::true_type{}, n, ho0, wo0); epi_finish(std::true_type{}, n, ho0, wo0); }
            else { epi_load(std::false_type{}, n, ho0, wo0); epi_finish(std::false_type{}, n, ho0, wo0); }
        }
        TM(5)
        if (g2 == 0) cur = nxt;
        g = g2;
    }
    }
#ifndef CTL_TIMING_WGRAD
#ifdef CTL_TIMING_DOMINANT_ONLY
    if (KS == 3 && S == 1 && MODE == 0 && MT == 4 && TW == 32 && NT == 1 && EPI == 0)
#endif
    TM_FLUSH
#endif

    if (flags & CTL_EPI_STATS) flush_stats(cur_grp);
}
```

### cooperative_training_and_latent_space_data_augmentation_amd/csrc/ctl_conv_x3.hip

```cpp
#include "ctl_common.h"
#ifdef CTL_TIMING_X3
#define CTL_TM_WAVES 65536
__device__ unsigned long long ctl_tm3[CTL_TM_WAVES][10];
#define TM_DECL unsigned long long tm_prev = __builtin_amdgcn_s_memtime(), tm_acc[10] = {0, 0, 0, 0, 0, 0, 0, 0, 0, 0}; \
                const unsigned long long tm_t0 = tm_prev, tm_r0 = __builtin_amdgcn_s_memrealtime();
#define TM(i) { const unsigned long long tm_now = __builtin_amdgcn_s_memtime(); tm_acc[i] += tm_now - tm_prev; tm_prev = tm_now; }
#define TM_COUNT(i) { tm_acc[i] += 1; }
#ifdef CTL_TIMING_X3_VMCNT
#define CTL_TM3_REAL
#else
#define CTL_TM3_REAL tm_acc[9] = __builtin_amdgcn_s_memrealtime() - tm_r0;
#endif
#define TM_FLUSH { const unsigned w_ = ((blockIdx.x + gridDim.x * (blockIdx.y + gridDim.y * blockIdx.z)) * 8 + (threadIdx.x >> 6)) % CTL_TM_WAVES; \
                   tm_acc[8] = __builtin_amdgcn_s_memtime() - tm_t0; CTL_TM3_REAL \
                   if ((threadIdx.x & 63) == 0) { _Pragma("unroll") for (int i_ = 0; i_ < 10; ++i_) ctl_tm3[w_][i_] += tm_acc[i_]; } }
extern "C" int ctl_debug_timing_x3(unsigned long long* out12) {
    static unsigned long long host[CTL_TM_WAVES][10];
    if (hipMemcpyFromSymbol(host, HIP_SYMBOL(ctl_tm3), sizeof(host)) != hipSuccess) return -1;
    for (int i = 0; i < 12; ++i) out12[i] = 0;
    for (int w = 0; w < CTL_TM_WAVES; ++w) {
        for (int i = 0; i < 10; ++i) out12[i] += host[w][i];
        if (host[w][8] > out12[10]) out12[10] = host[w][8];
        if (host[w][8]) out12[11] += 1;
    }
    for (int w = 0; w < CTL_TM_WAVES; ++w) for (int i = 0; i < 10; ++i) host[w][i] = 0;
    return hipMemcpyToSymbol(HIP_SYMBOL(ctl_tm3), host, sizeof(host)) == hipSuccess ? 0 : -1;
}
#endif
#include "ctl_conv_igemm.h"

__device__ static float x3_pack_value(const float* __restrict__ src, const int64_t* __restrict__ r, int mode, int co, int ci, int kh, int kw) {
    const int cout = (int)r[2], cin = (int)r[3], ks = (int)r[4], flip = (int)r[5];
    if (co >= cout || ci >= cin) return 0.f;
    float v = 0.f;
    if (mode == 1) {
        for (int a = 0; a < 2; ++a) {
            const int sh = a + 2 - kh;
            if (sh < 0 || sh > 2) continue;
            for (int b = 0; b < 2; ++b) {
                const int sw = b + 2 - kw;
                if (sw < 0 || sw > 2) continue;
                v += src[co * r[6] + ci * r[7] + sh * r[8] + sw * r[9]];
            }
        }
    } else if (mode == 2) {
        const int a = flip >> 1, b = flip & 1;
        const int h0 = (kh == 0) ? 0 : (a ? 2 : 1), h1 = (kh == 0) ? (a ? 1 : 0) : 2;
        const int w0 = (kw == 0) ? 0 : (b ? 2 : 1), w1 = (kw == 0) ? (b ? 1 : 0) : 2;
        for (int sh = h0; sh <= h1; ++sh)
            for (int sw = w0; sw <= w1; ++sw) v += src[co * r[6] + ci * r[7] + sh * r[8] + sw * r[9]];
    } else if (mode == 3) {
        const int a = flip >> 1, b = flip & 1;
        const int sh = a ? (kh == 0 ? 2 : 0) : (kh == 0 ? 1 : -1);
        const int sw = b ? (kw == 0 ? 2 : 0) : (kw == 0 ? 1 : -1);
        if (sh >= 0 && sw >= 0) v = src[co * r[6] + ci * r[7] + sh * r[8] + sw * r[9]];
    } else {
        if (flip) { kh = ks - 1 - kh; kw = ks - 1 - kw; }
        v = src[co * r[6] + ci * r[7] + kh * r[8] + kw * r[9]];
    }
    return v;
}
__global__ void pack_weights_x3_batched_kernel(const float* __restrict__ params, float* __restrict__ wpack, const int64_t* __restrict__ table) {
    const int64_t* r = table + (int64_t)blockIdx.y * 12;
    if (!(r[11] & CTL_PACK_X3)) return;
    const int mode = (int)(r[11] & ~(int64_t)CTL_PACK_X3);
    const int cout = (int)r[2], cin = (int)r[3], ks = (int)r[4];
    const int g_chunks = (cin + 15) / 16, taps = ks * ks, nfrag = (taps + 1) / 2;
    const int64_t total = (int64_t)((cout + 15) / 16) * nfrag * g_chunks * 64 * 4;
    const int64_t idx = (int64_t)blockIdx.x * blockDim.x + threadIdx.x;
    if (idx >= total) return;
    const float* src = params + r[0];
    unsigned* dst = reinterpret_cast<unsigned*>(wpack + r[1]);
    const int jp = idx & 3, lane = (idx >> 2) & 63;
    int64_t rest = idx >> 8;
    const int g = rest % g_chunks;
    rest /= g_chunks;
    const int f = rest % nfrag;
    const int cot = rest / nfrag;
    const int co = cot * 16 + (lane & 15), q = lane >> 4;
    const int tap = 2 * f + (q >> 1);
    float a = 0.f, b = 0.f;
    if (tap < taps) {
        const int ci = g * 16 + (q & 1) * 8 + jp * 2;
        a = x3_pack_value(src, r, mode, co, ci, tap / ks, tap % ks);
        b = x3_pack_value(src, r, mode, co, ci + 1, tap / ks, tap % ks);
    }
    const int64_t base = ((((int64_t)cot * nfrag + f) * g_chunks + g) * 3) * 256 + lane * 4 + jp;
#pragma unroll
    for (int sp = 0; sp < 3; ++sp) dst[base + sp * 256] = x3_pack2(x3_part(a, sp), x3_part(b, sp));
}
extern "C" size_t ctl_conv_wpack_floats_x3(int32_t cin, int32_t cout, int32_t ks) {
    return (size_t)ctl_cdiv(cout, 16) * ((ks * ks + 1) / 2) * ctl_cdiv(cin, 16) * 3 * 256;
}
extern "C" int ctl_pack_weights_x3_batched(const float* params, float* wpack, const int64_t* table, int32_t n_rec, int64_t max_total, ctl_stream stream) {
    CTL_REQUIRE(params && wpack && table && n_rec > 0 && max_total > 0, "pack_weights_x3_batched: bad arguments");
    pack_weights_x3_batched_kernel<<<dim3((unsigned)ctl_cdiv64(max_total, 3 * 256) + 1, (unsigned)n_rec), dim3(256), 0, (hipStream_t)stream>>>(params, wpack, table);
    CTL_LAUNCH_CHECK("pack_weights_x3_batched");
    return CTL_OK;
}

struct conv3_call {
    const ctl_conv* d; ctl_conv_cfg c;
    const float *x, *wpack, *bias, *pro_scale, *pro_shift, *res, *res_scale, *res_shift, *res2, *x2;
    float *y, *stats_partial, *pool, *xout;
    hipStream_t stream;
    bool query;
    int grid_x;
    int stat_rows_per_block;
};

#ifndef CTL_X3_PC_DEFAULT
#define CTL_X3_PC_DEFAULT 1
#endif
#ifndef CTL_X3_PC_MIN_STEPS
#define CTL_X3_PC_MIN_STEPS 4
#endif
static bool conv3_pc_shape_ok(const ctl_conv* d) {
    const int f = d->epi_flags & (CTL_EPI_RES | CTL_EPI_ACCUM | CTL_EPI_BNBWD | CTL_EPI_TAILBWD);
    const bool epi_ok = f == 0 || (f == CTL_EPI_BNBWD && d->cout % 16 == 0 && d->epi_act == CTL_ACT_NONE);
    return d->ks == 3 && d->stride == 1 && d->in_mode == CTL_IN_PLAIN && d->nsub == 1 && epi_ok;
}
template <int KS, int S, int MODE, int MT, int TW, int NT, int EPI, bool X2>
constexpr bool conv3_pc_ok() { return S == 1 && KS == 3 && MODE == CTL_IN_PLAIN && (EPI == 0 || EPI == 3); }
template <int KS, int S, int MODE, int MT, int TW, int NT, int EPI, bool X2>
static bool conv3_go_pc(conv3_call& a) {
    if constexpr (conv3_pc_ok<KS, S, MODE, MT, TW, NT, EPI, X2>()) {
        if (!a.c.pc) return false;
        const ctl_conv* d = a.d;
        const int ntiles = d->n * a.c.tiles_h * a.c.tiles_w;
        const int grid_x = ctl_conv_grid_x(ntiles, (a.c.cot / NT) * d->nsub, 1);
        a.grid_x = grid_x;
        a.stat_rows_per_block = 4;
        if (a.query) return true;
        const dim3 grid((unsigned)grid_x, (unsigned)(a.c.cot / NT), (unsigned)d->nsub);
        conv_igemm_kernel<KS, S, MODE, MT, TW, NT, EPI, X2, true, true><<<grid, dim3(512), 0, a.stream>>>(
            *d, a.x, a.wpack, a.bias, a.pro_scale, a.pro_shift, a.res, a.res_scale, a.res_shift, a.y, a.stats_partial, a.c.tiles_h,
            a.c.tiles_w, a.c.g, (int64_t)ctl_conv_wpack_floats_x3(d->cin, d->cout, d->ks), ntiles, a.res2, a.x2, a.pool, a.xout);
        return true;
    }
    return false;
}
template <int KS, int S, int MODE, int MT, int TW, int NT, int EPI, bool X2 = false>
static void conv3_go(conv3_call& a) {
    if constexpr (!X2 && ((KS == 3 && S == 1 && MODE == CTL_IN_PLAIN) || (KS == 4 && S == 2)) && EPI != 2) {
        if (a.d->pro_affine == 2) { conv3_go<KS, S, MODE, MT, TW, NT, EPI, true>(a); return; }
    }
    a.stat_rows_per_block = 1;
    if (conv3_go_pc<KS, S, MODE, MT, TW, NT, EPI, X2>(a)) return;
    static int occ = 0;
    if (!occ) {
        int n = 0;
        if (hipOccupancyMaxActiveBlocksPerMultiprocessor(&n, conv_igemm_kernel<KS, S, MODE, MT, TW, NT, EPI, X2, true>, 256, 0) != hipSuccess || n < 1) {
            (void)hipGetLastError();
            n = 2;
        }
        occ = n;
    }
    const ctl_conv* d = a.d;
    const int ntiles = d->n * a.c.tiles_h * a.c.tiles_w;
    a.grid_x = ctl_conv_grid_x(ntiles, (a.c.cot / NT) * d->nsub, occ);
    if (a.query) return;
    const dim3 grid((unsigned)a.grid_x, (unsigned)(a.c.cot / NT), (unsigned)d->nsub);
    conv_igemm_kernel<KS, S, MODE, MT, TW, NT, EPI, X2, true><<<grid, dim3(256), 0, a.stream>>>(
        *d, a.x, a.wpack, a.bias, a.pro_scale, a.pro_shift, a.res, a.res_scale, a.res_shift, a.y, a.stats_partial, a.c.tiles_h,
        a.c.tiles_w, a.c.g, (int64_t)ctl_conv_wpack_floats_x3(d->cin, d->cout, d->ks), ntiles, a.res2, a.x2, a.pool, a.xout);
}
template <int KS, int S, int MODE>
constexpr bool conv3_tail_ok() { return KS == 2 || (KS == 3 && S == 1 && MODE == CTL_IN_ZINS2); }
template <int KS, int S, int MODE, int MT, int TW>
static void conv3_go_nt(conv3_call& a) {
    constexpr bool NT2 = !(S == 2 && KS >= 3);
    const bool epi = (a.d->epi_flags & (CTL_EPI_RES | CTL_EPI_ACCUM | CTL_EPI_BNBWD)) != 0;
    const bool two = NT2 && a.c.nt == 2;
    auto go = [&](auto E) {
        constexpr int EPI = decltype(E)::value;
        if constexpr (NT2) { if (two) { conv3_go<KS, S, MODE, MT, TW, 2, EPI>(a); return; } }
        conv3_go<KS, S, MODE, MT, TW, 1, EPI>(a);
    };
    if constexpr (conv3_tail_ok<KS, S, MODE>()) {
        if (a.d->epi_flags & CTL_EPI_TAILBWD) { go(std::integral_constant<int, 2>{}); return; }
    }
    if constexpr (KS == 3 && S == 1 && MODE == CTL_IN_PLAIN) {
        if ((a.d->epi_flags & (CTL_EPI_RES | CTL_EPI_ACCUM | CTL_EPI_BNBWD)) == CTL_EPI_BNBWD && a.d->cout % 16 == 0 && a.d->epi_act == CTL_ACT_NONE) {
            go(std::integral_constant<int, 3>{});
            return;
        }
    }
    if (epi) go(std::integral_constant<int, 1>{}); else go(std::integral_constant<int, 0>{});
}
template <int KS, int S, int MODE>
static void conv3_go_tile(conv3_call& a) {
    if (S == 1 && a.c.mt == 4 && a.c.tw == 32) conv3_go_nt<KS, S, MODE, (S == 1 ? 4 : 2), (S == 1 ? 32 : 16)>(a);
    else if (a.c.mt == 2) conv3_go_nt<KS, S, MODE, 2, 16>(a);
    else conv3_go_nt<KS, S, MODE, 1, 16>(a);
}
static int conv3_dispatch(conv3_call& a) {
    const int k = a.d->ks, s = a.d->stride, m = a.d->in_mode;
    if (k == 3 && s == 1 && m == CTL_IN_PLAIN) conv3_go_tile<3, 1, CTL_IN_PLAIN>(a);
    else if (k == 3 && s == 1 && m == CTL_IN_UP2) conv3_go_tile<3, 1, CTL_IN_UP2>(a);
    else if (k == 3 && s == 1 && m == CTL_IN_ZINS2) conv3_go_tile<3, 1, CTL_IN_ZINS2>(a);
    else if (k == 3 && s == 2) conv3_go_tile<3, 2, CTL_IN_PLAIN>(a);
    else if (k == 2 && s == 2) conv3_go_tile<2, 2, CTL_IN_PLAIN>(a);
    else if (k == 2 && s == 1) conv3_go_tile<2, 1, CTL_IN_PLAIN>(a);
    else if (k == 4 && s == 2) conv3_go_nt<4, 2, CTL_IN_PLAIN, 1, 16>(a);
    else CTL_FAIL(CTL_EUNSUPPORTED, "conv_forward(x3): no kernel for ks/stride/in_mode %d/%d/%d", k, s, m);
    return CTL_OK;
}

static int conv3_pick_cfg(const ctl_conv* d, ctl_conv_cfg* c) {
    const int rc = ctl_conv_pick_cfg(d, c, 0);
    if (rc != CTL_OK) return rc;
    static const int pc_on = ctl_tune_int("CTL_X3_PC", CTL_X3_PC_DEFAULT), min_steps = ctl_tune_int("CTL_X3_PC_MIN_STEPS", CTL_X3_PC_MIN_STEPS);
    static const int pc_min_g = ctl_tune_int("CTL_X3_PC_MIN_G", 4);
    if (pc_on && conv3_pc_shape_ok(d) && c->g >= pc_min_g && c->nt == 2) {
        static const int tiles[3][2] = {{4, 32}, {2, 16}, {1, 16}};
        const int other = (c->cot / c->nt) * d->nsub;
        for (int i = 0; i < 3; ++i) {
            const int mt = tiles[i][0], tw = tiles[i][1], th = 4 * mt * 16 / tw;
            if (tw == 32 && d->wout < 32) continue;
            const int64_t ntiles = (int64_t)d->n * ctl_cdiv(d->hout, th) * ctl_cdiv(d->wout, tw);
            if (ntiles * other < ctl_num_cus() && i < 2) continue;
            const int grid_x = ctl_conv_grid_x((int)ntiles, other, 1);
            static const int gate = ctl_tune_int("CTL_X3_PC_GATE", 1);
            const bool shares_ok = !gate || ntiles <= grid_x || ntiles % grid_x == 0;
            if (shares_ok && ntiles * c->g >= (int64_t)min_steps * grid_x) {
                c->pc = 1; c->mt = mt; c->tw = tw; c->th = th;
                c->tiles_h = ctl_cdiv(d->hout, th); c->tiles_w = ctl_cdiv(d->wout, tw);
            }
            break;
        }
    }
    if (d->stride == 2 && d->ks >= 3) {
        c->nt = 1;
        if (d->ks == 4 && c->mt != 1) {
            c->mt = 1; c->tw = 16; c->th = 4;
            c->tiles_h = ctl_cdiv(d->hout, c->th);
            c->tiles_w = ctl_cdiv(d->wout, c->tw);
        }
    }
    return CTL_OK;
}

int ctl_conv_x3_ok(const ctl_conv* d) {
    return d->cin % 16 == 0 && (d->cout % 16 == 0 || (d->cout < 16 && d->cout % 4 == 0)) && d->ks >= 2 && d->in_mode != CTL_IN_C4 && !(d->dt & (CTL_DT_BF16 | CTL_DT_X16 | CTL_DT_Y16 | CTL_DT_RES16));
}
int ctl_conv_x3_stats_blocks(const ctl_conv* d) {
    conv3_call a = {};
    a.d = d;
    if (!ctl_conv_x3_ok(d) || conv3_pick_cfg(d, &a.c) != CTL_OK) return -1;
    a.query = true;
    if (conv3_dispatch(a) != CTL_OK) return -1;
    return a.grid_x * d->nsub * a.stat_rows_per_block;
}
int ctl_conv_forward_x3(const ctl_conv* d, const float* x, const float* wpack, const float* bias, const float* pro_scale, const float* pro_shift,
                        const float* res, const float* res_scale, const float* res_shift, const float* res2, const float* x2, float* y,
                        float* stats_partial, float* pool, float* xout, ctl_stream stream) {
    CTL_REQUIRE(ctl_conv_x3_ok(d), "conv_forward(x3): CTL_DT_X3 needs fp32-stored tensors, cin %% 16 == 0, cout %% 16 == 0 (or 4 / 8 / 12) and a 2x2 / 3x3 / 4x4 kernel "
                                   "(got cin %d, cout %d, ks %d, in_mode %d, dt %d)", d->cin, d->cout, d->ks, d->in_mode, d->dt);
    CTL_REQUIRE(!pool, "conv_forward(x3): `pool` belongs to the 1x1 hosts, which stay on the fp32 pipe");
    conv3_call a = {};
    a.d = d;
    int rc = conv3_pick_cfg(d, &a.c);
    if (rc != CTL_OK) return rc;
    a.x = x; a.wpack = wpack; a.bias = bias; a.pro_scale = pro_scale; a.pro_shift = pro_shift; a.res = res; a.res_scale = res_scale;
    a.res_shift = res_shift; a.res2 = res2; a.x2 = x2; a.y = y; a.stats_partial = stats_partial; a.pool = pool; a.xout = xout;
    a.stream = (hipStream_t)stream;
    a.query = true;
    rc = conv3_dispatch(a);
    if (rc != CTL_OK) return rc;
    a.query = false;
    const int ptok = ctl_prof_begin(a.stat_rows_per_block == 4 ? "conv_igemm_x3pc" : "conv_igemm_x3", d, &a.c, a.c.nt, a.stream);
    rc = conv3_dispatch(a);
    if (ptok >= 0) ctl_prof_end(ptok, a.stream);
    if (rc != CTL_OK) return rc;
    CTL_LAUNCH_CHECK("conv_forward(x3)");
    return CTL_OK;
}
```

### include/ctl_hip.h

```cpp
#ifndef CTL_HIP_H
#define CTL_HIP_H

#include <stddef.h>
#include <stdint.h>

#ifdef __cplusplus
extern "C" {
#endif

typedef void* ctl_stream;

enum ctl_status { CTL_OK = 0, CTL_EINVAL = -1, CTL_EUNSUPPORTED = -2, CTL_ELAUNCH = -3 };

#define CTL_ABI_VERSION 11
int         ctl_version(void);
const char* ctl_last_error(void);

enum { CTL_IN_PLAIN = 0, CTL_IN_UP2 = 1, CTL_IN_ZINS2 = 2, CTL_IN_C4 = 3  };
enum { CTL_ACT_NONE = 0, CTL_ACT_LEAKY = 1, CTL_ACT_SIGMOID = 2 };
enum { CTL_EPI_BIAS = 1, CTL_EPI_ACCUM = 2, CTL_EPI_RES = 4, CTL_EPI_STATS = 8, CTL_EPI_BNBWD = 16, CTL_EPI_TAILBWD = 32 };

typedef struct ctl_conv {
    int32_t n, hin, win, cin;
    int32_t hout, wout, cout;
    int32_t ks, stride, pad;
    int32_t in_mode;
    int32_t pro_affine;
    float   pro_slope;
    int32_t epi_flags;
    int32_t epi_act;
    float   epi_slope;
    int32_t out_h, out_w;
    int32_t out_sy, out_sx;
    int32_t nsub, out_sub;
    int32_t groups;
    int32_t dt;
} ctl_conv;
enum { CTL_DT_BF16 = 1, CTL_DT_X16 = 2, CTL_DT_Y16 = 4, CTL_DT_RES16 = 8, CTL_DT_X3 = 16 };
enum { CTL_PACK_X3 = 16 };

size_t ctl_conv_wpack_floats(int32_t cin, int32_t cout, int32_t ks);
size_t ctl_conv_stats_floats(const ctl_conv* d);
int    ctl_conv_stats_blocks(const ctl_conv* d);

int ctl_pack_weights(const float* src, float* dst, int32_t cout, int32_t cin, int32_t ks,
                     int64_t s_co, int64_t s_ci, int64_t s_kh, int64_t s_kw, int32_t flip, ctl_stream stream);

int ctl_conv_forward(const ctl_conv* d, const float* x, const float* wpack, const float* bias,
                     const float* pro_scale, const float* pro_shift,
                     const float* res, const float* res_scale, const float* res_shift,
                     float* y, float* stats_partial, ctl_stream stream);
int ctl_conv_forward_ex(const ctl_conv* d, const float* x, const float* wpack, const float* bias,
                        const float* pro_scale, const float* pro_shift,
                        const float* res, const float* res_scale, const float* res_shift, const float* res2, const float* x2,
                        float* y, float* stats_partial, float* pool, float* xout, ctl_stream stream);
int ctl_conv_pool_ok(const ctl_conv* d);

int    ctl_wgrad_splits(const ctl_conv* d);
size_t ctl_wgrad_partial_floats(const ctl_conv* d);
size_t ctl_wgrad_bias_partial_floats(const ctl_conv* d);
int ctl_conv_wgrad(const ctl_conv* d, const float* x, const float* pro_scale, const float* pro_shift,
                   const float* dy, float* w_partial, float* b_partial, ctl_stream stream);
int ctl_conv_wgrad_ex(const ctl_conv* d, const float* x, const float* pro_scale, const float* pro_shift,
                      const float* dy, const float* dy2, const float* dy_coef, float* w_partial, float* b_partial, ctl_stream stream);

int ctl_wgrad_group_class(const ctl_conv* d, int32_t has_dy2);
int ctl_wgrad_group_plan(const ctl_conv* descs, int32_t n, int32_t* splits);
int ctl_conv_wgrad_group(int32_t n, const ctl_conv* descs, const int32_t* splits, const float* const* x, const float* const* pro_scale,
                         const float* const* pro_shift, const float* const* dy, const float* const* dy2, const float* const* dy_coef,
                         float* const* w_partial, float* const* b_partial, ctl_stream stream);
int ctl_wgrad_reduce(const ctl_conv* d, const float* w_partial, const float* b_partial,
                     float* dw, int64_t s_co, int64_t s_ci, int64_t s_kh, int64_t s_kw,
                     float* dbias, int32_t accumulate, ctl_stream stream);

int ctl_pack_weights_batched(const float* params, float* wpack, const int64_t* table, int32_t n_rec, int64_t max_total,
                             ctl_stream stream);
int ctl_wgrad_reduce_batched(const float* scratch, float* grad, const int64_t* table, int32_t n_rec, int64_t max_blocks,
                             ctl_stream stream);
int ctl_pack_weights_bf16_batched(const float* params, float* wpack, const int64_t* table, int32_t n_rec, int64_t max_total,
                                  ctl_stream stream);
size_t ctl_conv_wpack_floats_x3(int32_t cin, int32_t cout, int32_t ks);
int ctl_pack_weights_x3_batched(const float* params, float* wpack, const int64_t* table, int32_t n_rec, int64_t max_total,
                                ctl_stream stream);

int ctl_bn_finalize(const float* partial, int32_t blocks, int32_t c, int64_t count, const float* gamma,
                    const float* beta, float eps, float momentum, int32_t update_running, float* running_mean,
                    float* running_var, int64_t* num_batches_tracked, float* scale, float* shift, float* save_mean,
                    float* save_invstd, int32_t groups, ctl_stream stream);
int ctl_bn_finalize_ex(const float* partial, int32_t blocks, int32_t c, int64_t count, const float* gamma,
                       const float* beta, float eps, float momentum, int32_t update_running, float* running_mean,
                       float* running_var, int64_t* num_batches_tracked, float* scale, float* shift, float* save_mean,
                       float* save_invstd, float* save_uvar, int32_t groups, ctl_stream stream);
int ctl_bn_replay_running(const void* act, float* buffers, int64_t* num_batches_tracked, const int64_t* table, int32_t n_rec,
                          float momentum, ctl_stream stream);
int ctl_bn_eval_coeffs(int32_t c, const float* gamma, const float* beta, const float* running_mean,
                       const float* running_var, float eps, float* scale, float* shift, int32_t groups, ctl_stream stream);
int ctl_bn_act(const float* x, const float* scale, const float* shift, float slope, float* y, int64_t pixels,
               int32_t c, int32_t groups, ctl_stream stream);

#ifndef CTL_RED_BLOCKS
#define CTL_RED_BLOCKS 512
#endif
int ctl_bwd_reduce(int32_t mode, const float* dy, const float* act_src, const float* bn_src, const float* scale,
                   const float* shift, float slope, int64_t pixels, int32_t c, float* partial, int32_t groups,
                   ctl_stream stream);
int ctl_bwd_reduce_rows(int32_t mode, int64_t pixels_per_group, int32_t c);
int ctl_red_blocks(void);
int ctl_bn_bwd_finalize(const float* partial, int32_t c, int64_t count, const float* gamma, const float* save_mean,
                        const float* save_invstd, float* coef, float* dgamma, float* dbeta, int32_t accumulate,
                        int32_t groups, int32_t blocks, ctl_stream stream);
int ctl_bn_bwd_finalize_ex(const float* partial, int32_t c, int64_t count, const float* gamma, const float* save_mean,
                           const float* save_invstd, float* coef, float* dgamma, float* dbeta, int32_t accumulate,
                           int32_t groups, int32_t blocks, uint32_t affine_groups, ctl_stream stream);
int ctl_bwd_apply(int32_t mode, const float* dy, const float* act_src, const float* bn_src, const float* scale,
                  const float* shift, float slope, const float* coef, int64_t pixels, int32_t c, float* ds,
                  float* dx, int32_t groups, ctl_stream stream);
int ctl_chan_sum_finalize(const float* partial, int32_t c, float* out, int32_t accumulate, ctl_stream stream);
int ctl_sumpool2(const float* dup, float* dx, int32_t n, int32_t h, int32_t w, int32_t c, int32_t accumulate,
                 ctl_stream stream);
int ctl_sigmoid_bwd(const float* dy, const float* y, float* dx, int64_t count, ctl_stream stream);

int ctl_softmax_t_fwd(const float* x, float inv_t, float* p, int64_t pixels, int32_t c, ctl_stream stream);
int ctl_softmax_t_bwd(const float* p, const float* dp, float inv_t, float* dx, int64_t pixels, int32_t c,
                      ctl_stream stream);
int ctl_onehot(const int64_t* label, float* y, int64_t pixels, int32_t c, ctl_stream stream);
int ctl_ce2d_fwd(const float* logit, const int64_t* label, int64_t pixels, int32_t c, double* partial, float* loss,
                 ctl_stream stream);
int ctl_ce2d_bwd(const float* logit, const int64_t* label, const float* gout, int64_t pixels, int32_t c,
                 float* dlogit, ctl_stream stream);
enum { CTL_LOSS_WCE = 0, CTL_LOSS_FOCAL = 1, CTL_LOSS_DICE = 2, CTL_LOSS_FG_DICE = 3 };
int32_t ctl_seg_loss_blocks(int32_t b, int64_t hw);
size_t ctl_seg_loss_ws_doubles(int32_t kind, int32_t b, int64_t hw, int32_t c);
int ctl_seg_loss_fwd(int32_t kind, const float* logit, const int64_t* label, const double* class_weights, float gamma, int32_t b,
                     int64_t hw, int32_t c, double* ws, float* loss, ctl_stream stream);
int ctl_seg_loss_bwd(int32_t kind, const float* logit, const int64_t* label, const double* class_weights, float gamma, const float* gout,
                     const double* ws, int32_t b, int64_t hw, int32_t c, float* dlogit, ctl_stream stream);
int ctl_mse_fwd(const float* a, const float* b, int64_t count, float scale, double* partial, float* loss,
                ctl_stream stream);
int ctl_mse_bwd(const float* a, const float* b, const float* gout, int64_t count, float scale, float* da,
                ctl_stream stream);
int ctl_argmax_c(const float* logit, uint8_t* out, int64_t pixels, int32_t c, ctl_stream stream);

int ctl_bn_act_dt(const float* x, const float* scale, const float* shift, float slope, float* y, int64_t pixels, int32_t c,
                  int32_t groups, uint32_t bf16_mask, ctl_stream stream);
int ctl_bwd_reduce_dt(int32_t mode, const float* dy, const float* act_src, const float* bn_src, const float* scale,
                      const float* shift, float slope, int64_t pixels, int32_t c, float* partial, int32_t groups,
                      uint32_t bf16_mask, float* ds, ctl_stream stream);
int ctl_bwd_apply_dt(int32_t mode, const float* dy, const float* act_src, const float* bn_src, const float* scale,
                     const float* shift, float slope, const float* coef, int64_t pixels, int32_t c, float* ds, float* dx,
                     int32_t groups, uint32_t bf16_mask, ctl_stream stream);
int ctl_sumpool2_dt(const float* dup, float* dx, int32_t n, int32_t h, int32_t w, int32_t c, int32_t accumulate,
                    uint32_t bf16_mask, ctl_stream stream);

size_t ctl_latent_score_ws_floats(int32_t mode, int32_t n, int32_t hw, int32_t c);
int ctl_latent_score(int32_t mode, const float* grad, float* score, float* scratch, int32_t n, int32_t hw, int32_t c,
                     ctl_stream stream);
size_t ctl_latent_mask_apply_ws_floats(int32_t mode, int32_t n, int32_t hw, int32_t c);
int ctl_latent_mask_apply(int32_t mode, const float* code, const float* score, const float* soft_noise,
                          int32_t k_host, const int32_t* k_dev, float* masked, float* mask_out, float* scratch, int32_t n,
                          int32_t hw, int32_t c, ctl_stream stream);
size_t ctl_latent_mask_fused_ws_floats(int32_t mode, int32_t n, int32_t hw, int32_t c);
int ctl_latent_mask_fused(int32_t mode, const float* grad, const float* code, const float* soft_noise, int32_t k_host,
                          const int32_t* k_dev, float* masked, float* mask_out, float* score_out, float* workspace, int32_t n,
                          int32_t hw, int32_t c, ctl_stream stream);
int ctl_dropout2d(const float* z, const float* keep, uint64_t seed, float p, float* out, float* keep_out, int32_t n,
                  int32_t hw, int32_t c, ctl_stream stream);
int ctl_uniform(float* out, int64_t count, uint64_t seed, ctl_stream stream);
int ctl_step_tick(int64_t* state, ctl_stream stream);
int ctl_spin(int32_t microseconds, ctl_stream stream);
int ctl_dropout2d_ex(const float* z, const float* keep, uint64_t seed_or_salt, const int64_t* state, float p, float* out,
                     float* keep_out, float* mask_full, int32_t n, int32_t hw, int32_t c, ctl_stream stream);
int ctl_uniform_dev(float* out, int64_t count, uint64_t salt, const int64_t* state, ctl_stream stream);
int ctl_dropout2d_dt(const void* z, const float* keep, uint64_t seed_or_salt, const int64_t* state, float p, void* out,
                     float* keep_out, int32_t n, int32_t hw, int32_t c, uint32_t bf16_mask, ctl_stream stream);

int ctl_confusion_hist(const int64_t* label_true, const uint8_t* label_pred, int64_t count, int32_t n_class, int64_t* hist,
                       ctl_stream stream);
size_t ctl_rescale_intensity_ws_floats(int32_t planes);
int ctl_rescale_intensity(const float* x, float* out, float* workspace, int32_t planes, int64_t plane_elems, float new_min,
                          float new_max, float eps, ctl_stream stream);
int ctl_noise_clamp(const float* x, const float* noise, uint64_t seed, float sigma, float lo, float hi, float* out,
                    int64_t count, ctl_stream stream);
int ctl_crop_or_pad(const void* src, void* dst, int32_t elem_bytes, int32_t n, int32_t h, int32_t w, int32_t new_h,
                    int32_t new_w, ctl_stream stream);

int32_t ctl_surface_stats_rows(int32_t d, int32_t n_class, int32_t foreground_only, int32_t mode);
size_t ctl_surface_stats_ws_bytes(int32_t d, int32_t h, int32_t w, int32_t n_class, int32_t foreground_only, int32_t mode);
int ctl_surface_stats(const uint8_t* pred, const int64_t* gt, int32_t d, int32_t h, int32_t w, int32_t n_class,
                      int32_t foreground_only, int32_t mode, int32_t connectivity, const double* sampling, double* table,
                      void* workspace, size_t workspace_bytes, ctl_stream stream);
size_t ctl_surface_quantiles_ws_bytes(int32_t d, int32_t h, int32_t w, int32_t n_class, int32_t foreground_only, int32_t mode,
                                      int32_t n_q);
int ctl_surface_quantiles(const uint8_t* pred, const int64_t* gt, int32_t d, int32_t h, int32_t w, int32_t n_class,
                          int32_t foreground_only, int32_t mode, int32_t connectivity, const double* sampling, const double* q,
                          int32_t n_q, double* stats_table, double* q_table, void* workspace, size_t workspace_bytes,
                          ctl_stream stream);
size_t ctl_surface_map_ws_bytes(int32_t d, int32_t h, int32_t w, int32_t mode);
int ctl_surface_map(const uint8_t* mask, int32_t d, int32_t h, int32_t w, int32_t mode, int32_t connectivity,
                    const double* sampling, double* d2_out, uint8_t* surface_out, void* workspace, size_t workspace_bytes,
                    ctl_stream stream);

size_t ctl_cc_ws_bytes(int32_t d, int32_t h, int32_t w, int32_t n_class, int32_t mode);
int ctl_cc_label(const uint8_t* labelmap, int32_t d, int32_t h, int32_t w, int32_t n_class, int32_t mode, int32_t connectivity,
                 int32_t* labels, ctl_stream stream);
int ctl_cc_keep_largest(const uint8_t* labelmap, int32_t d, int32_t h, int32_t w, int32_t n_class, int32_t mode, int32_t connectivity,
                        uint8_t* out, int64_t* table, void* workspace, size_t workspace_bytes, ctl_stream stream);

size_t ctl_aug_ws_bytes(int32_t n, int32_t hp, int32_t wp);
size_t ctl_aug_warp_ws_bytes(int32_t n, int32_t hp, int32_t wp, int32_t hc, int32_t wc);
int ctl_aug_field(const float* noise, const uint64_t* seeds, const float* alpha, const float* sigma, int32_t n, int32_t hp, int32_t wp,
                  float* field, void* workspace, size_t workspace_bytes, ctl_stream stream);
int ctl_aug_warp(const float* image, const int64_t* label, const float* matrix, const float* intensity, const float* field, int32_t n,
                 int32_t hp, int32_t wp, int32_t hc, int32_t wc, float* image_out, int64_t* label_out, void* workspace,
                 size_t workspace_bytes, ctl_stream stream);
size_t ctl_aug_spline_ws_bytes(int32_t n, int32_t hp, int32_t wp, int32_t n_class);
size_t ctl_aug_warp_cubic_ws_bytes(int32_t n, int32_t hp, int32_t wp, int32_t hc, int32_t wc, int32_t n_class);
int ctl_aug_spline_coeffs(const float* image, const int64_t* label, const float* intensity, int32_t n, int32_t hp, int32_t wp,
                          int32_t n_class, float* coeffs, void* workspace, size_t workspace_bytes, ctl_stream stream);
int ctl_aug_warp_cubic(const float* image, const int64_t* label, const float* matrix, const float* intensity, const float* field, int32_t n,
                       int32_t hp, int32_t wp, int32_t hc, int32_t wc, int32_t n_class, float* image_out, int64_t* label_out,
                       void* workspace, size_t workspace_bytes, ctl_stream stream);
size_t ctl_aug_bias_ws_bytes(int32_t n, int32_t hp, int32_t wp);
int ctl_aug_bias(const float* image, const float* bias, const float* noise, const uint64_t* seeds, int32_t n, int32_t hp, int32_t wp,
                 float* out, void* workspace, size_t workspace_bytes, ctl_stream stream);
int ctl_aug_coarse_field(const float* coarse, int32_t n, int32_t hp, int32_t wp, float* field, ctl_stream stream);

size_t ctl_order_stats_ws_bytes(int32_t segments, int32_t n_rank);
int ctl_order_stats(const float* x, int32_t segments, int64_t seg_elems, const int64_t* ranks, int32_t n_rank, float* out,
                    void* workspace, size_t workspace_bytes, ctl_stream stream);
int ctl_percentile_apply(const float* x, const float* table, int32_t segments, int64_t seg_elems, double g_lo, double g_hi,
                         int32_t form, float new_min, float new_max, float* out, float* bounds, ctl_stream stream);
int ctl_resample_inplane(const float* image, const void* label, int32_t label_bytes, int32_t n, int32_t h, int32_t w, int32_t new_h,
                         int32_t new_w, double r_h, double r_w, float* image_out, void* label_out, ctl_stream stream);

int ctl_restore_scores(const float* scores, int32_t n, int32_t c, int32_t win_h, int32_t win_w, int32_t h, int32_t w, int32_t res_h,
                       int32_t res_w, int32_t off_y, int32_t off_x, double q_h, double q_w, int32_t mode, uint8_t* label, float* soft,
                       ctl_stream stream);
int ctl_restore_labels(const uint8_t* labels, int32_t n, int32_t win_h, int32_t win_w, int32_t h, int32_t w, int32_t res_h, int32_t res_w,
                       int32_t off_y, int32_t off_x, double q_h, double q_w, uint8_t* out, ctl_stream stream);

#define CTL_CORRUPT_MAX_SPIKES 8
#define CTL_CORRUPT_MAX_COPIES 8
#define CTL_CORRUPT_RED_BLOCKS 256
int ctl_corrupt_bias(const float* x, const float* coefficients, int32_t d, int32_t h, int32_t w, float* out, ctl_stream stream);
size_t ctl_corrupt_spike_ws_bytes(int32_t d, int32_t h, int32_t w, int32_t n_spikes);
int ctl_corrupt_spike(const float* x, int32_t d, int32_t h, int32_t w, const int32_t* k, const int32_t* mult, int32_t n_spikes,
                      double intensity, float* out, void* workspace, size_t workspace_bytes, ctl_stream stream);
int ctl_corrupt_rigid3d(const float* x, int32_t d, int32_t h, int32_t w, const float* matrices, int32_t copies, float* out,
                        ctl_stream stream);
int ctl_axis_operator(const float* x0, const float* xs, int32_t n_volumes, int32_t d, int32_t h, int32_t w, int32_t axis,
                      const float* matrix, float* out, ctl_stream stream);

int ctl_slice_foreground(const uint8_t* label, const int64_t* table, int32_t n_slices, int64_t arena_elems, int32_t* counts,
                         ctl_stream stream);
int ctl_batch_gather(const float* image, const uint8_t* label, const int64_t* table, int32_t n_slices, int64_t arena_elems,
                     const int32_t* index, int32_t n, const uint8_t* lut, int32_t H, int32_t W, float* image_out, int64_t* label_out,
                     int32_t Hc, int32_t Wc, float* orig_image, int64_t* orig_label, ctl_stream stream);

int ctl_adam(float* p, const float* g, float* m, float* v, int64_t count, float lr, float beta1, float beta2,
             float eps, int32_t step, float grad_scale, ctl_stream stream);
int ctl_accumulate(float* dst, const float* const* srcs, int32_t k, int64_t count, ctl_stream stream);
int ctl_adam_dev(float* p, const float* g, float* m, float* v, int64_t count, float lr, float beta1, float beta2,
                 float eps, const int64_t* state, float grad_scale, ctl_stream stream);

enum ctl_op_kind {
    CTL_OP_CONV = 1, CTL_OP_WGRAD = 2, CTL_OP_WGRAD_REDUCE = 3, CTL_OP_PACK = 4, CTL_OP_BN_FINALIZE = 5,
    CTL_OP_BN_EVAL = 6, CTL_OP_BN_ACT = 7, CTL_OP_BWD_REDUCE = 8, CTL_OP_BN_BWD_FINALIZE = 9, CTL_OP_BWD_APPLY = 10,
    CTL_OP_CHAN_SUM_FINALIZE = 11, CTL_OP_SUMPOOL2 = 12, CTL_OP_SIGMOID_BWD = 13, CTL_OP_ZERO = 14, CTL_OP_COPY = 15, CTL_OP_PACK_BATCH = 16,
    CTL_OP_WGRAD_REDUCE_BATCH = 17, CTL_OP_DROPOUT2D = 18, CTL_OP_BN_REPLAY = 19,
    CTL_OP_WGRAD_GROUP = 20
};
#define CTL_OP_MAX_T 14
typedef struct ctl_op {
    int32_t kind;
    int32_t i[27];
    float   f[4];
    int32_t slot[CTL_OP_MAX_T];
    int64_t off[CTL_OP_MAX_T];
    int64_t l[4];
} ctl_op;
int ctl_plan_run(const ctl_op* ops, int32_t n_ops, void* const* bases, int32_t n_bases, ctl_stream stream);

int ctl_prof_start(const char* filter);
int ctl_prof_start_sampled(const char* filter, int32_t every);
int ctl_prof_stop(char* out, size_t cap);
unsigned long long ctl_launch_count(void);
size_t ctl_sizeof_op(void);
size_t ctl_sizeof_conv(void);

#ifdef __cplusplus
}
#endif
#endif
```

Before: 1100.

## Shrink conv grid via load-balance model and serpentine row-walk work distribution

Adds a host-side model of per-CU work when persistent conv blocks are spread across CUs, and picks a smaller persistent grid whenever the model predicts a lower maximum per-CU cost than the current rows grid by a set margin. When a smaller grid is chosen, a new rows-kernel variant has each block walk several virtual blocks in serpentine order (RowWalk), so tile shares even out across blocks. Results are memoized per shape, and debug entry points expose the chosen grids. This aims to cut tail imbalance in the implicit-GEMM conv launches, at the cost of a heuristic cost model that may misjudge real throughput and of extra kernel instantiations.

Result: no change. 1104, median of 6 (+0.4%).

```diff
diff --git a/cooperative_training_and_latent_space_data_augmentation_amd/_ffi.py b/cooperative_training_and_latent_space_data_augmentation_amd/_ffi.py
--- a/cooperative_training_and_latent_space_data_augmentation_amd/_ffi.py
+++ b/cooperative_training_and_latent_space_data_augmentation_amd/_ffi.py
@@ -24,7 +24,7 @@
     ("ks", "<i4"), ("stride", "<i4"), ("pad", "<i4"), ("in_mode", "<i4"), ("pro_affine", "<i4"), ("pro_slope", "<f4"),
     ("epi_flags", "<i4"), ("epi_act", "<i4"), ("epi_slope", "<f4"), ("out_h", "<i4"), ("out_w", "<i4"),
     ("out_sy", "<i4"), ("out_sx", "<i4"), ("nsub", "<i4"), ("out_sub", "<i4"), ("groups", "<i4"), ("dt", "<i4")])
-DT_BF16, DT_X16, DT_Y16, DT_RES16, DT_X3 = 1, 2, 4, 8, 16
+DT_BF16, DT_X16, DT_Y16, DT_RES16, DT_X3, DT_ROWS_GRID = 1, 2, 4, 8, 16, 32
 PACK_X3 = 16
 LOSS_WCE, LOSS_FOCAL, LOSS_DICE, LOSS_FG_DICE = 0, 1, 2, 3
 OP_DTYPE = np.dtype([("kind", "<i4"), ("i", "<i4", (27,)), ("f", "<f4", (4,)), ("slot", "<i4", (OP_MAX_T,)),
@@ -62,6 +62,7 @@
         sig = {
             "ctl_conv_wpack_floats": [i32, i32, i32],
             "ctl_conv_stats_floats": [p], "ctl_conv_stats_blocks": [p],
+            "ctl_conv_launch_grid": [p, i32, p], "ctl_conv_row_walk": [i32, i32, i32, p, p, p, p],
             "ctl_wgrad_splits": [p], "ctl_wgrad_partial_floats": [p], "ctl_wgrad_bias_partial_floats": [p],
             "ctl_pack_weights": [p, p, i32, i32, i32, i64, i64, i64, i64, i32, p],
             "ctl_conv_forward": [p] * 12, "ctl_conv_forward_ex": [p] * 16, "ctl_conv_pool_ok": [p],
@@ -184,7 +185,7 @@
             "ctl_percentile_apply", "ctl_resample_inplane", "ctl_corrupt_bias", "ctl_corrupt_spike_ws_bytes", "ctl_corrupt_spike",
             "ctl_corrupt_rigid3d", "ctl_axis_operator", "ctl_slice_foreground", "ctl_batch_gather", "ctl_surface_quantiles_ws_bytes",
             "ctl_surface_quantiles", "ctl_restore_scores", "ctl_restore_labels", "ctl_seg_loss_blocks", "ctl_seg_loss_ws_doubles",
-            "ctl_seg_loss_fwd", "ctl_seg_loss_bwd"]
+            "ctl_seg_loss_fwd", "ctl_seg_loss_bwd", "ctl_conv_launch_grid", "ctl_conv_row_walk"]
 
 
 def prof_start(kernel_filter: str = "", every: int = 1) -> None:
diff --git a/cooperative_training_and_latent_space_data_augmentation_amd/csrc/ctl_common.h b/cooperative_training_and_latent_space_data_augmentation_amd/csrc/ctl_common.h
--- a/cooperative_training_and_latent_space_data_augmentation_amd/csrc/ctl_common.h
+++ b/cooperative_training_and_latent_space_data_augmentation_amd/csrc/ctl_common.h
@@ -116,7 +116,10 @@
     int pc;
 };
 int ctl_conv_pick_cfg(const ctl_conv* d, ctl_conv_cfg* c, int for_wgrad);
+int ctl_conv_rows_grid_x(int ntiles, int other, int occ);
 int ctl_conv_grid_x(int ntiles, int other, int occ);
+struct ctl_conv_grids { int gc, gp, ntiles, other, occ, max_c, max_p, sum_tiles; };
+int ctl_conv_launch_grid_x(int ntiles, int other, int occ, int gc, bool rows_only, ctl_conv_grids* rec);
 static inline int ctl_num_cus() { static const int n = ctl_tune_int("CTL_NUM_CUS", 256); return n; }
 
 int ctl_conv_forward_bf16(const ctl_conv* d, const void* x, const void* x2, const void* wpack, const float* bias, const float* pro_scale,
@@ -135,6 +138,7 @@
 
 int ctl_conv_x3_ok(const ctl_conv* d);
 int ctl_conv_x3_stats_blocks(const ctl_conv* d);
+int ctl_conv_x3_launch_grid(const ctl_conv* d, int occ, ctl_conv_grids* g);
 int ctl_conv_forward_x3(const ctl_conv* d, const float* x, const float* wpack, const float* bias, const float* pro_scale, const float* pro_shift,
                         const float* res, const float* res_scale, const float* res_shift, const float* res2, const float* x2, float* y,
                         float* stats_partial, float* pool, float* xout, ctl_stream stream);
diff --git a/cooperative_training_and_latent_space_data_augmentation_amd/csrc/ctl_conv.hip b/cooperative_training_and_latent_space_data_augmentation_amd/csrc/ctl_conv.hip
--- a/cooperative_training_and_latent_space_data_augmentation_amd/csrc/ctl_conv.hip
+++ b/cooperative_training_and_latent_space_data_augmentation_amd/csrc/ctl_conv.hip
@@ -1,6 +1,10 @@
 #include <stdlib.h>
 
+#include <algorithm>
+#include <mutex>
 #include <type_traits>
+#include <unordered_map>
+#include <vector>
 
 #include "ctl_common.h"
 
@@ -798,7 +802,7 @@
     return CTL_OK;
 }
 
-int ctl_conv_grid_x(int ntiles, int other, int occ) {
+int ctl_conv_rows_grid_x(int ntiles, int other, int occ) {
     static int per_cu = -1;
     if (per_cu < 0) {
         per_cu = ctl_tune_int("CTL_PERSIST", 4);
@@ -809,6 +813,77 @@
     if (other > 1 && cap >= 8) cap -= cap % 8;
     if (cap < 1) cap = 1;
     return ntiles < cap ? ntiles : cap;
+}
+int ctl_conv_grid_x(int ntiles, int other, int occ) { return ctl_conv_rows_grid_x(ntiles, other, occ); }
+
+#ifndef CTL_BALANCE_INV1
+#define CTL_BALANCE_INV1 1800
+#endif
+#ifndef CTL_BALANCE_INV2
+#define CTL_BALANCE_INV2 1150
+#endif
+static void conv_grid_model(int ntiles, int other, int gc, int gp, int* max_tt, int* sum) {
+    static const int inv[3] = {0, ctl_tune_int("CTL_BALANCE_INV1", CTL_BALANCE_INV1), ctl_tune_int("CTL_BALANCE_INV2", CTL_BALANCE_INV2)};
+    const int ncu = ctl_num_cus();
+    std::vector<int> tiles((size_t)gp);
+    std::vector<std::vector<int>> on_cu((size_t)ncu);
+    for (int pb = 0; pb < gp; ++pb) {
+        RowWalk r;
+        int t = 0;
+        for (r.init(gc, gp, ntiles, pb); r.valid(); r.advance()) t += r.tiles();
+        tiles[(size_t)pb] = t;
+    }
+    for (int64_t L = 0; L < (int64_t)gp * other; ++L) on_cu[(size_t)(L % ncu)].push_back(tiles[(size_t)(L % gp)]);
+    int64_t m = 0;
+    for (auto& c : on_cu) {
+        std::sort(c.begin(), c.end(), [](int a, int b) { return a > b; });
+        int64_t cost = 0;
+        for (size_t j = 0; j < c.size(); ++j) {
+            const int rounds = c[j] - (j + 1 < c.size() ? c[j + 1] : 0), act = (int)j + 1;
+            cost += (int64_t)rounds * act * (act < 3 ? inv[act] : 1000);
+        }
+        m = std::max(m, cost);
+    }
+    *max_tt = (int)std::min<int64_t>(m, 0x7fffffff);
+    *sum = ntiles * other;
+}
+#ifndef CTL_BALANCE_PCT
+#define CTL_BALANCE_PCT 5
+#endif
+int ctl_conv_launch_grid_x(int ntiles, int other, int occ, int gc, bool rows_only, ctl_conv_grids* rec) {
+    static const int pct = ctl_tune_int("CTL_BALANCE_PCT", CTL_BALANCE_PCT);
+    const int force_res = ctl_tune_int("CTL_BALANCE_RES", 0);
+    struct entry { int gp, max_c, max_p; };
+    static std::mutex mu;
+    static std::unordered_map<uint64_t, entry> memo;
+    const uint64_t key = ((uint64_t)(uint32_t)ntiles << 32) | ((uint64_t)(uint32_t)other << 12) | ((uint64_t)(force_res & 0xf) << 8) | (uint64_t)(occ & 0xff);
+    entry e = {gc, 0, 0};
+    bool found = false;
+    {
+        std::lock_guard<std::mutex> lock(mu);
+        auto it = memo.find(key);
+        if (it != memo.end()) { e = it->second; found = true; }
+    }
+    int sum = ntiles * other;
+    if (!found) {
+        conv_grid_model(ntiles, other, gc, gc, &e.max_c, &sum);
+        e.gp = gc;
+        e.max_p = e.max_c;
+        const int resident = (int)(((int64_t)gc * other + ctl_num_cus() - 1) / ctl_num_cus());
+        for (int r = resident - 1; r >= 1 && (pct >= 0 || force_res); --r) {
+            if (force_res && r != force_res) continue;
+            int cand = (ctl_num_cus() * r) / other;
+            if (other > 1) cand -= cand % 8;
+            if (cand < 8 || cand >= gc) continue;
+            int m = 0;
+            conv_grid_model(ntiles, other, gc, cand, &m, &sum);
+            if (force_res || (m < e.max_p && (int64_t)(e.max_c - m) * 100 > (int64_t)pct * e.max_c)) { e.gp = cand; e.max_p = m; }
+        }
+        std::lock_guard<std::mutex> lock(mu);
+        memo[key] = e;
+    }
+    if (rec) *rec = ctl_conv_grids{gc, rows_only ? gc : e.gp, ntiles, other, occ, e.max_c, rows_only ? e.max_c : e.max_p, sum};
+    return rows_only ? gc : e.gp;
 }
 
 extern "C" int ctl_pack_weights(const float* src, float* dst, int32_t cout, int32_t cin, int32_t ks, int64_t s_co,
@@ -828,6 +903,8 @@
     hipStream_t stream;
     bool query;
     int grid_x;
+    int occ_override;
+    ctl_conv_grids grids;
 };
 
 template <int KS, int S, int MODE, int MT, int TW, int NT, int EPI, bool X2 = false>
@@ -845,13 +922,20 @@
         occ = n;
     }
     const ctl_conv* d = a.d;
-    const int ntiles = d->n * a.c.tiles_h * a.c.tiles_w;
-    a.grid_x = ctl_conv_grid_x(ntiles, (a.c.cot / NT) * d->nsub, occ);
+    const int ntiles = d->n * a.c.tiles_h * a.c.tiles_w, other = (a.c.cot / NT) * d->nsub;
+    const int occ_used = (a.query && a.occ_override > 0) ? a.occ_override : occ;
+    a.grid_x = ctl_conv_rows_grid_x(ntiles, other, occ_used);
+    const int gp = ctl_conv_launch_grid_x(ntiles, other, occ_used, a.grid_x, (d->dt & CTL_DT_ROWS_GRID) != 0, &a.grids);
     if (a.query) return;
-    const dim3 grid((unsigned)a.grid_x, (unsigned)(a.c.cot / NT), (unsigned)d->nsub);
-    conv_igemm_kernel<KS, S, MODE, MT, TW, NT, EPI, X2><<<grid, dim3(256), 0, a.stream>>>(
-        *d, a.x, a.wpack, a.bias, a.pro_scale, a.pro_shift, a.res, a.res_scale, a.res_shift, a.y, a.stats_partial, a.c.tiles_h,
-        a.c.tiles_w, a.c.g, (int64_t)ctl_conv_wpack_floats(d->cin, d->cout, d->ks), ntiles, a.res2, a.x2, a.pool, a.xout);
+    const dim3 grid((unsigned)gp, (unsigned)(a.c.cot / NT), (unsigned)d->nsub);
+    if (gp == a.grid_x)
+        conv_igemm_kernel<KS, S, MODE, MT, TW, NT, EPI, X2><<<grid, dim3(256), 0, a.stream>>>(
+            *d, a.x, a.wpack, a.bias, a.pro_scale, a.pro_shift, a.res, a.res_scale, a.res_shift, a.y, a.stats_partial, a.c.tiles_h,
+            a.c.tiles_w, a.c.g, (int64_t)ctl_conv_wpack_floats(d->cin, d->cout, d->ks), ntiles, a.res2, a.x2, a.pool, a.xout);
+    else
+        conv_igemm_rows_kernel<KS, S, MODE, MT, TW, NT, EPI, X2><<<grid, dim3(256), 0, a.stream>>>(
+            *d, a.x, a.wpack, a.bias, a.pro_scale, a.pro_shift, a.res, a.res_scale, a.res_shift, a.y, a.stats_partial, a.c.tiles_h,
+            a.c.tiles_w, a.c.g, (int64_t)ctl_conv_wpack_floats(d->cin, d->cout, d->ks), ntiles, a.res2, a.x2, a.pool, a.xout, a.grid_x);
 }
 template <int KS, int S, int MODE>
 constexpr bool conv_tail_ok() { return (KS == 1 && MODE == CTL_IN_PLAIN) || KS == 2 || (KS == 3 && S == 1 && MODE == CTL_IN_ZINS2); }
@@ -909,6 +993,42 @@
     a.query = true;
     if (conv_dispatch(a) != CTL_OK) return -1;
     return a.grid_x * d->nsub;
+}
+extern "C" int ctl_conv_launch_grid(const ctl_conv* d, int32_t occ, int32_t* out8) {
+    CTL_REQUIRE(d && out8 && occ >= 0 && occ <= 8, "conv_launch_grid: bad arguments");
+    ctl_conv_grids g = {};
+    if (d->dt & CTL_DT_BF16) {
+        CTL_FAIL(CTL_EUNSUPPORTED, "conv_launch_grid: the bf16 family launches its rows grid");
+    } else if (d->dt & CTL_DT_X3) {
+        const int rc = ctl_conv_x3_launch_grid(d, occ, &g);
+        if (rc != CTL_OK) return rc;
+    } else {
+        conv_call a = {};
+        a.d = d;
+        const int rc = ctl_conv_pick_cfg(d, &a.c, 0);
+        if (rc != CTL_OK) return rc;
+        a.query = true;
+        a.occ_override = occ;
+        if (conv_dispatch(a) != CTL_OK) return CTL_EUNSUPPORTED;
+        g = a.grids;
+    }
+    const int v[8] = {g.gc, g.gp, g.ntiles, g.other, g.occ, g.max_c, g.max_p, g.sum_tiles};
+    for (int i = 0; i < 8; ++i) out8[i] = v[i];
+    return CTL_OK;
+}
+extern "C" int ctl_conv_row_walk(int32_t gc, int32_t gp, int32_t ntiles, int32_t* owner, int32_t* walks, int32_t* tiles, int32_t* place) {
+    if (gc < 1 || gp < (gc < 8 ? gc : 8) || gp > gc || ntiles < gc || !owner || !walks || !tiles || !place) return -1;
+    for (int v = 0; v < gc; ++v) { owner[v] = -1; walks[v] = 0; tiles[v] = 0; place[v] = -1; }
+    for (int pb = 0; pb < gp; ++pb) {
+        RowWalk r;
+        int n = 0;
+        for (r.init(gc, gp, ntiles, pb); r.valid(); r.advance(), ++n) {
+            const int v = r.vblock();
+            if (v < 0 || v >= gc) return -2;
+            owner[v] = pb; walks[v] += 1; tiles[v] = r.tiles(); place[v] = n;
+        }
+    }
+    return 0;
 }
 extern "C" size_t ctl_conv_stats_floats(const ctl_conv* d) {
     const int b = ctl_conv_stats_blocks(d);
diff --git a/cooperative_training_and_latent_space_data_augmentation_amd/csrc/ctl_conv_igemm.h b/cooperative_training_and_latent_space_data_augmentation_amd/csrc/ctl_conv_igemm.h
--- a/cooperative_training_and_latent_space_data_augmentation_amd/csrc/ctl_conv_igemm.h
+++ b/cooperative_training_and_latent_space_data_augmentation_amd/csrc/ctl_conv_igemm.h
@@ -158,6 +158,41 @@
     }
 };
 
+struct RowWalk {
+    int P, cls, nbv, nbp, t_lo;
+    int q, r;
+    int j, step;
+    __host__ __device__ __forceinline__ void init(int Gc, int Gp, int ntiles, int pb) {
+        int k, t_hi;
+        if (Gc >= 8) {
+            P = 8;
+            cls = pb & 7;
+            k = pb >> 3;
+            nbv = (Gc - cls + 7) >> 3;
+            nbp = (Gp - cls + 7) >> 3;
+            t_lo = (int)(((int64_t)ntiles * cls) >> 3);
+            t_hi = (int)(((int64_t)ntiles * (cls + 1)) >> 3);
+        } else {
+            P = Gc;
+            cls = pb;
+            k = 0;
+            nbv = nbp = 1;
+            t_lo = (int)(((int64_t)ntiles * cls) / P);
+            t_hi = (int)(((int64_t)ntiles * (cls + 1)) / P);
+        }
+        const int t = t_hi - t_lo;
+        q = t / nbv;
+        r = t - q * nbv;
+        j = k;
+        step = 2 * (nbp - k) - 1;
+    }
+    __host__ __device__ __forceinline__ bool valid() const { return j < nbv; }
+    __host__ __device__ __forceinline__ void advance() { j += step; step = 2 * nbp - step; }
+    __host__ __device__ __forceinline__ int vblock() const { return cls + P * j; }
+    __host__ __device__ __forceinline__ int first_tile() const { return t_lo + j; }
+    __host__ __device__ __forceinline__ int tiles() const { return q + (j < r ? 1 : 0); }
+};
+
 
 #ifndef CTL_LB_MID
 #define CTL_LB_MID 3
@@ -171,7 +206,7 @@
 #ifndef CTL_PC_SETS_X2
 #define CTL_PC_SETS_X2 2
 #endif
-template <int KS, int S, int MODE, int MT, int TW, int NT, int EPI, bool X2 = false, bool X3 = false, bool PC = false>
+template <int KS, int S, int MODE, int MT, int TW, int NT, int EPI, bool X2 = false, bool X3 = false, bool PC = false, bool ROWS = false>
 #ifndef CTL_LB_X2EPI
 #define CTL_LB_X2EPI 2
 #endif
@@ -184,8 +219,9 @@
 #ifndef CTL_LB_X3
 #define CTL_LB_X3(MT, NT, X2) (((NT) == 1 && (MT) >= 2 && !(X2)) ? 3 : 2)
 #endif
-__global__ __launch_bounds__(PC ? 512 : 256, PC ? 2 : X3 ? CTL_LB_X3(MT, NT, X2) : (MT * NT >= 8 || KS == 4) ? 2 : ((MT * NT >= 4) ? (X2 ? (EPI ? CTL_LB_X2EPI : CTL_LB_X2) : CTL_LB_MID)
-                                                                                    : ((X2 && EPI) ? CTL_LB_SMALL_X2EPI : CTL_LB_SMALL))) void conv_igemm_kernel(const ctl_conv d, const float* __restrict__ x,
+#define CTL_CONV_LB __launch_bounds__(PC ? 512 : 256, PC ? 2 : X3 ? CTL_LB_X3(MT, NT, X2) : (MT * NT >= 8 || KS == 4) ? 2 : ((MT * NT >= 4) ? (X2 ? (EPI ? CTL_LB_X2EPI : CTL_LB_X2) : CTL_LB_MID) \
+                                                                                    : ((X2 && EPI) ? CTL_LB_SMALL_X2EPI : CTL_LB_SMALL)))
+__device__ __forceinline__ void conv_igemm_body(const ctl_conv& d, const float* __restrict__ x,
                                                           const float* __restrict__ wpack,
                                                           const float* __restrict__ bias,
                                                           const float* __restrict__ pro_scale,
@@ -196,13 +232,14 @@
                                                           float* __restrict__ stats_partial, int tiles_h, int tiles_w,
                                                           int G_chunks, int64_t wpack_sub_stride, int ntiles,
                                                           const float* __restrict__ res2, const float* __restrict__ x2,
-                                                          float* __restrict__ pool, float* __restrict__ xout) {
+                                                          float* __restrict__ pool, float* __restrict__ xout, int Gc) {
     using G = Geom<KS, S, MT, TW>;
     constexpr int TAPS = KS * KS;
     constexpr bool C4 = (MODE == CTL_IN_C4);
     static_assert(!C4 || (KS == 3 && S == 1), "K-packed taps: 3x3 stride-1 only");
     static_assert(!X3 || !C4, "X3: whole 16-channel chunks");
     static_assert(!PC || X3, "the producer / consumer form exists for the X3 launches");
+    static_assert(!(PC && ROWS), "the producer / consumer form launches its rows grid (equal shares by its gate)");
     constexpr int NIMG = PC ? 2 : 1;
     using XS3 = XStage3<KS, S, C4 ? CTL_IN_PLAIN : MODE, MT, TW, X2>;
     constexpr int NFRAG = X3 ? (TAPS + 1) / 2 : (C4 ? 3 : TAPS);
@@ -225,15 +262,24 @@
     const int wave = PC ? (wave_all & 3) : wave_all;
     const bool consumer = PC && wave_all >= 4;
     const int p = lane & 15, q = lane >> 4;
-    const int P = gridDim.x < 8 ? (int)gridDim.x : 8;
-    const int xcd = blockIdx.x % P, jblk = blockIdx.x / P;
-    const int nb = ((int)gridDim.x - xcd + P - 1) / P;
-    const int t_lo = (int)(((int64_t)ntiles * xcd) / P), t_hi = (int)(((int64_t)ntiles * (xcd + 1)) / P);
-    const int bid0 = t_lo + jblk;
+    RowWalk rows = {};
+    int nb, bid0 = 0, my_tiles;
+    if constexpr (ROWS) {
+        rows.init(Gc, (int)gridDim.x, ntiles, (int)blockIdx.x);
+        nb = rows.nbv;
+        my_tiles = 0;
+        for (RowWalk r = rows; r.valid(); r.advance()) my_tiles += r.tiles();
+    } else {
+        const int P = gridDim.x < 8 ? (int)gridDim.x : 8;
+        const int xcd = blockIdx.x % P, jblk = blockIdx.x / P;
+        nb = ((int)gridDim.x - xcd + P - 1) / P;
+        const int t_lo = (int)(((int64_t)ntiles * xcd) / P), t_hi = (int)(((int64_t)ntiles * (xcd + 1)) / P);
+        bid0 = t_lo + jblk;
+        my_tiles = (bid0 < t_hi) ? (t_hi - bid0 + nb - 1) / nb : 0;
+    }
     const int z = blockIdx.z;
     const int cot0 = blockIdx.y * NT;
     const float* wp = wpack + (int64_t)z * wpack_sub_stride;
-    const int my_tiles = (bid0 < t_hi) ? (t_hi - bid0 + nb - 1) / nb : 0;
     const int total_it = my_tiles * G_chunks;
     const int flags = d.epi_flags;
     const int ngroups = d.groups > 1 ? d.groups : 1;
@@ -313,9 +359,37 @@
         }
     };
 
+    RowWalk nrow = rows;
     TileWalk cur, nxt;
-    cur.init(bid0, nb, tiles_h, tiles_w);
+    int nxt_left = 0, nxt_v = (int)blockIdx.x;
+    if constexpr (ROWS) {
+        while (nrow.tiles() == 0) {
+            RowWalk r = nrow;
+            r.advance();
+            if (!r.valid()) break;
+            nrow = r;
+        }
+        cur.init(nrow.first_tile(), nb, tiles_h, tiles_w);
+        nxt_left = nrow.tiles() - 1;
+        nxt_v = nrow.vblock();
+    } else {
+        cur.init(bid0, nb, tiles_h, tiles_w);
+    }
     nxt = cur;
+    int cur_v = nxt_v;
+    auto advance_nxt = [&]() {
+        if constexpr (!ROWS) { nxt.next(); return; }
+        if (nxt_left > 0) { nxt.next(); --nxt_left; return; }
+        do nrow.advance(); while (nrow.valid() && nrow.tiles() == 0);
+        if (!nrow.valid()) return;
+        const int b0 = nrow.first_tile();
+        nxt.tw = b0 % tiles_w;
+        const int b1 = b0 / tiles_w;
+        nxt.th = b1 % tiles_h;
+        nxt.n = b1 / tiles_h;
+        nxt_left = nrow.tiles() - 1;
+        nxt_v = nrow.vblock();
+    };
     TM_DECL
     if (!PC && total_it > 0) {
         xs.load(rx, rx2, d, cur.n, cur.th * G::TH, cur.tw * TW, 0);
@@ -391,8 +465,11 @@
         }
     }
 
-    const int srows = gridDim.x * gridDim.z * (PC ? 4 : 1), srow = (z * gridDim.x + blockIdx.x) * (PC ? 4 : 1) + (PC ? wave : 0);
-    auto flush_stats = [&](int grp) {
+    const int srows = (ROWS ? Gc : (int)gridDim.x) * gridDim.z * (PC ? 4 : 1);
+    const int srow_one = (z * gridDim.x + blockIdx.x) * (PC ? 4 : 1) + (PC ? wave : 0);
+    auto srow_of = [&](int v) { return ROWS ? (z * Gc + v) : srow_one; };
+    auto flush_stats = [&](int grp, int v) {
+        const int srow = srow_of(v);
 #pragma unroll
         for (int t = 0; t < NT; ++t) {
             float a[8] = {ssum[t].x, ssum[t].y, ssum[t].z, ssum[t].w, ssq[t].x, ssq[t].y, ssq[t].z, ssq[t].w};
@@ -438,8 +515,10 @@
         __syncthreads();
     };
     int cur_grp = (my_tiles > 0) ? cur.n / group_n : 0;
+    int acc_v = cur_v;
     if constexpr (PC) {
         if ((flags & CTL_EPI_STATS) && ngroups > 1 && consumer && p == 0) {
+            const int srow = srow_of(cur_v);
             for (int gi = 0; gi < ngroups; ++gi)
 #pragma unroll
                 for (int t = 0; t < NT; ++t)
@@ -452,10 +531,20 @@
                         }
                     }
         }
-    } else if ((flags & CTL_EPI_STATS) && ngroups > 1 && tid < NT * 16 * 2) {
+    } else if constexpr (!ROWS) {
+        if ((flags & CTL_EPI_STATS) && ngroups > 1 && tid < NT * 16 * 2) {
+            const int stat = tid / (NT * 16), co = cot0 * 16 + tid % (NT * 16), srow = srow_of(cur_v);
+            if (co < d.cout)
+                for (int gi = 0; gi < ngroups; ++gi) stats_partial[(((int64_t)gi * srows + srow) * 2 + stat) * d.cout + co] = 0.f;
+        }
+    } else if ((flags & CTL_EPI_STATS) && tid < NT * 16 * 2) {
         const int stat = tid / (NT * 16), co = cot0 * 16 + tid % (NT * 16);
         if (co < d.cout)
-            for (int gi = 0; gi < ngroups; ++gi) stats_partial[(((int64_t)gi * srows + srow) * 2 + stat) * d.cout + co] = 0.f;
+            for (RowWalk r = rows; r.valid(); r.advance()) {
+                if (ngroups <= 1 && r.tiles() > 0) continue;
+                const int srow = srow_of(r.vblock());
+                for (int gi = 0; gi < ngroups; ++gi) stats_partial[(((int64_t)gi * srows + srow) * 2 + stat) * d.cout + co] = 0.f;
+            }
     }
 
     TM(7)
@@ -728,7 +817,7 @@
             const bool full = tile_full(ho0, wo0);
             if (last) {
                 const int grp = n / group_n;
-                if ((flags & CTL_EPI_STATS) && grp != cur_grp) { flush_stats(cur_grp); cur_grp = grp; }
+                if ((flags & CTL_EPI_STATS) && grp != cur_grp) { flush_stats(cur_grp, acc_v); cur_grp = grp; }
                 if (full) epi_load(std::true_type{}, n, ho0, wo0); else epi_load(std::false_type{}, n, ho0, wo0);
             }
             TM(7)
@@ -750,7 +839,7 @@
             TM(5)
             if (++g == G_chunks) { g = 0; cw.next(); }
         }
-        if (flags & CTL_EPI_STATS) flush_stats(cur_grp);
+        if (flags & CTL_EPI_STATS) flush_stats(cur_grp, acc_v);
         TM_FLUSH
         return;
     } else {
@@ -760,7 +849,7 @@
         const bool has_next = it + 1 < total_it;
         const int g2 = (g + 1 == G_chunks) ? 0 : g + 1;
         const bool new_w = has_next && G_chunks > 1;
-        if (g2 == 0) nxt.next();
+        if (g2 == 0) advance_nxt();
         if (has_next && !(X3 && (CTL_X3_ABLATE & 2))) {
             xs.load(rx, rx2, d, nxt.n, nxt.th * G::TH, nxt.tw * TW, g2);
             if (new_w) wload(g2);
@@ -835,15 +924,19 @@
 
         if (g == G_chunks - 1 && !(X3 && (CTL_X3_ABLATE & 8))) {
             const int grp = n / group_n;
-            if ((flags & CTL_EPI_STATS) && grp != cur_grp) {
-                flush_stats(cur_grp);
+            if ((flags & CTL_EPI_STATS) && (grp != cur_grp || (ROWS && cur_v != acc_v))) {
+                flush_stats(cur_grp, acc_v);
                 cur_grp = grp;
+                if constexpr (ROWS) acc_v = cur_v;
             }
             if (tile_full(ho0, wo0)) { epi_load(std::true_type{}, n, ho0, wo0); epi_finish(std::true_type{}, n, ho0, wo0); }
             else { epi_load(std::false_type{}, n, ho0, wo0); epi_finish(std::false_type{}, n, ho0, wo0); }
         }
         TM(5)
-        if (g2 == 0) cur = nxt;
+        if (g2 == 0) {
+            cur = nxt;
+            if constexpr (ROWS) cur_v = nxt_v;
+        }
         g = g2;
     }
     }
@@ -854,5 +947,37 @@
     TM_FLUSH
 #endif
 
-    if (flags & CTL_EPI_STATS) flush_stats(cur_grp);
+    if ((flags & CTL_EPI_STATS) && (!ROWS || total_it > 0)) flush_stats(cur_grp, acc_v);
 }
+
+template <int KS, int S, int MODE, int MT, int TW, int NT, int EPI, bool X2 = false, bool X3 = false, bool PC = false>
+__global__ CTL_CONV_LB void conv_igemm_kernel(const ctl_conv d, const float* __restrict__ x,
+                                                          const float* __restrict__ wpack,
+                                                          const float* __restrict__ bias,
+                                                          const float* __restrict__ pro_scale,
+                                                          const float* __restrict__ pro_shift,
+                                                          const float* __restrict__ res,
+                                                          const float* __restrict__ res_scale,
+                                                          const float* __restrict__ res_shift, float* __restrict__ y,
+                                                          float* __restrict__ stats_partial, int tiles_h, int tiles_w,
+                                                          int G_chunks, int64_t wpack_sub_stride, int ntiles,
+                                                          const float* __restrict__ res2, const float* __restrict__ x2,
+                                                          float* __restrict__ pool, float* __restrict__ xout) {
+    conv_igemm_body<KS, S, MODE, MT, TW, NT, EPI, X2, X3, PC, false>(d, x, wpack, bias, pro_scale, pro_shift, res, res_scale, res_shift, y, stats_partial, tiles_h, tiles_w, G_chunks, wpack_sub_stride, ntiles, res2, x2, pool, xout, (int)gridDim.x);
+}
+template <int KS, int S, int MODE, int MT, int TW, int NT, int EPI, bool X2 = false, bool X3 = false, bool PC = false>
+__global__ CTL_CONV_LB void conv_igemm_rows_kernel(const ctl_conv d, const float* __restrict__ x,
+                                                          const float* __restrict__ wpack,
+                                                          const float* __restrict__ bias,
+                                                          const float* __restrict__ pro_scale,
+                                                          const float* __restrict__ pro_shift,
+                                                          const float* __restrict__ res,
+                                                          const float* __restrict__ res_scale,
+                                                          const float* __restrict__ res_shift, float* __restrict__ y,
+                                                          float* __restrict__ stats_partial, int tiles_h, int tiles_w,
+                                                          int G_chunks, int64_t wpack_sub_stride, int ntiles,
+                                                          const float* __restrict__ res2, const float* __restrict__ x2,
+                                                          float* __restrict__ pool, float* __restrict__ xout, int Gc) {
+    static_assert(!PC, "the producer / consumer form launches its rows grid");
+    conv_igemm_body<KS, S, MODE, MT, TW, NT, EPI, X2, X3, PC, true>(d, x, wpack, bias, pro_scale, pro_shift, res, res_scale, res_shift, y, stats_partial, tiles_h, tiles_w, G_chunks, wpack_sub_stride, ntiles, res2, x2, pool, xout, Gc);
+}
diff --git a/cooperative_training_and_latent_space_data_augmentation_amd/csrc/ctl_conv_x3.hip b/cooperative_training_and_latent_space_data_augmentation_amd/csrc/ctl_conv_x3.hip
--- a/cooperative_training_and_latent_space_data_augmentation_amd/csrc/ctl_conv_x3.hip
+++ b/cooperative_training_and_latent_space_data_augmentation_amd/csrc/ctl_conv_x3.hip
@@ -106,6 +106,8 @@
     hipStream_t stream;
     bool query;
     int grid_x;
+    int occ_override;
+    ctl_conv_grids grids;
     int stat_rows_per_block;
 };
 
@@ -128,8 +130,9 @@
         if (!a.c.pc) return false;
         const ctl_conv* d = a.d;
         const int ntiles = d->n * a.c.tiles_h * a.c.tiles_w;
-        const int grid_x = ctl_conv_grid_x(ntiles, (a.c.cot / NT) * d->nsub, 1);
+        const int grid_x = ctl_conv_rows_grid_x(ntiles, (a.c.cot / NT) * d->nsub, 1);
         a.grid_x = grid_x;
+        a.grids = ctl_conv_grids{grid_x, grid_x, ntiles, (a.c.cot / NT) * d->nsub, 1, 0, 0, ntiles * (a.c.cot / NT) * d->nsub};
         a.stat_rows_per_block = 4;
         if (a.query) return true;
         const dim3 grid((unsigned)grid_x, (unsigned)(a.c.cot / NT), (unsigned)d->nsub);
@@ -157,13 +160,20 @@
         occ = n;
     }
     const ctl_conv* d = a.d;
-    const int ntiles = d->n * a.c.tiles_h * a.c.tiles_w;
-    a.grid_x = ctl_conv_grid_x(ntiles, (a.c.cot / NT) * d->nsub, occ);
+    const int ntiles = d->n * a.c.tiles_h * a.c.tiles_w, other = (a.c.cot / NT) * d->nsub;
+    const int occ_used = (a.query && a.occ_override > 0) ? a.occ_override : occ;
+    a.grid_x = ctl_conv_rows_grid_x(ntiles, other, occ_used);
+    const int gp = ctl_conv_launch_grid_x(ntiles, other, occ_used, a.grid_x, (d->dt & CTL_DT_ROWS_GRID) != 0, &a.grids);
     if (a.query) return;
-    const dim3 grid((unsigned)a.grid_x, (unsigned)(a.c.cot / NT), (unsigned)d->nsub);
-    conv_igemm_kernel<KS, S, MODE, MT, TW, NT, EPI, X2, true><<<grid, dim3(256), 0, a.stream>>>(
-        *d, a.x, a.wpack, a.bias, a.pro_scale, a.pro_shift, a.res, a.res_scale, a.res_shift, a.y, a.stats_partial, a.c.tiles_h,
-        a.c.tiles_w, a.c.g, (int64_t)ctl_conv_wpack_floats_x3(d->cin, d->cout, d->ks), ntiles, a.res2, a.x2, a.pool, a.xout);
+    const dim3 grid((unsigned)gp, (unsigned)(a.c.cot / NT), (unsigned)d->nsub);
+    if (gp == a.grid_x)
+        conv_igemm_kernel<KS, S, MODE, MT, TW, NT, EPI, X2, true><<<grid, dim3(256), 0, a.stream>>>(
+            *d, a.x, a.wpack, a.bias, a.pro_scale, a.pro_shift, a.res, a.res_scale, a.res_shift, a.y, a.stats_partial, a.c.tiles_h,
+            a.c.tiles_w, a.c.g, (int64_t)ctl_conv_wpack_floats_x3(d->cin, d->cout, d->ks), ntiles, a.res2, a.x2, a.pool, a.xout);
+    else
+        conv_igemm_rows_kernel<KS, S, MODE, MT, TW, NT, EPI, X2, true><<<grid, dim3(256), 0, a.stream>>>(
+            *d, a.x, a.wpack, a.bias, a.pro_scale, a.pro_shift, a.res, a.res_scale, a.res_shift, a.y, a.stats_partial, a.c.tiles_h,
+            a.c.tiles_w, a.c.g, (int64_t)ctl_conv_wpack_floats_x3(d->cin, d->cout, d->ks), ntiles, a.res2, a.x2, a.pool, a.xout, a.grid_x);
 }
 template <int KS, int S, int MODE>
 constexpr bool conv3_tail_ok() { return KS == 2 || (KS == 3 && S == 1 && MODE == CTL_IN_ZINS2); }
@@ -220,7 +230,7 @@
             if (tw == 32 && d->wout < 32) continue;
             const int64_t ntiles = (int64_t)d->n * ctl_cdiv(d->hout, th) * ctl_cdiv(d->wout, tw);
             if (ntiles * other < ctl_num_cus() && i < 2) continue;
-            const int grid_x = ctl_conv_grid_x((int)ntiles, other, 1);
+            const int grid_x = ctl_conv_rows_grid_x((int)ntiles, other, 1);
             static const int gate = ctl_tune_int("CTL_X3_PC_GATE", 1);
             const bool shares_ok = !gate || ntiles <= grid_x || ntiles % grid_x == 0;
             if (shares_ok && ntiles * c->g >= (int64_t)min_steps * grid_x) {
@@ -251,6 +261,18 @@
     a.query = true;
     if (conv3_dispatch(a) != CTL_OK) return -1;
     return a.grid_x * d->nsub * a.stat_rows_per_block;
+}
+int ctl_conv_x3_launch_grid(const ctl_conv* d, int occ, ctl_conv_grids* g) {
+    conv3_call a = {};
+    a.d = d;
+    CTL_REQUIRE(ctl_conv_x3_ok(d), "conv_launch_grid(x3): not an X3 launch");
+    const int rc = conv3_pick_cfg(d, &a.c);
+    if (rc != CTL_OK) return rc;
+    a.query = true;
+    a.occ_override = occ;
+    if (conv3_dispatch(a) != CTL_OK) return CTL_EUNSUPPORTED;
+    *g = a.grids;
+    return CTL_OK;
 }
 int ctl_conv_forward_x3(const ctl_conv* d, const float* x, const float* wpack, const float* bias, const float* pro_scale, const float* pro_shift,
                         const float* res, const float* res_scale, const float* res_shift, const float* res2, const float* x2, float* y,
diff --git a/include/ctl_hip.h b/include/ctl_hip.h
--- a/include/ctl_hip.h
+++ b/include/ctl_hip.h
@@ -36,12 +36,15 @@
     int32_t groups;
     int32_t dt;
 } ctl_conv;
-enum { CTL_DT_BF16 = 1, CTL_DT_X16 = 2, CTL_DT_Y16 = 4, CTL_DT_RES16 = 8, CTL_DT_X3 = 16 };
+enum { CTL_DT_BF16 = 1, CTL_DT_X16 = 2, CTL_DT_Y16 = 4, CTL_DT_RES16 = 8, CTL_DT_X3 = 16,
+       CTL_DT_ROWS_GRID = 32  };
 enum { CTL_PACK_X3 = 16 };
 
 size_t ctl_conv_wpack_floats(int32_t cin, int32_t cout, int32_t ks);
 size_t ctl_conv_stats_floats(const ctl_conv* d);
 int    ctl_conv_stats_blocks(const ctl_conv* d);
+int    ctl_conv_launch_grid(const ctl_conv* d, int32_t occ, int32_t* out8);
+int    ctl_conv_row_walk(int32_t gc, int32_t gp, int32_t ntiles, int32_t* owner, int32_t* walks, int32_t* tiles, int32_t* place);
 
 int ctl_pack_weights(const float* src, float* dst, int32_t cout, int32_t cin, int32_t ks,
                      int64_t s_co, int64_t s_ci, int64_t s_kh, int64_t s_kw, int32_t flip, ctl_stream stream);
```
